# ctu-vras/depth_correction

Hardware: AMD Instinct MI355X
Metric: points/sec through min_eigval_loss fwd+bwd (200k pts, k=10); HBM GB/s vs peak (higher is better)
Workload: dtype f64

## Files before the change

### depth_correction_amd/_native.py

```python
from __future__ import annotations

import ctypes
import functools
import os

import torch

__all__ = ['lib', 'lib_path', 'on_device', 'DC_F32', 'DC_F64', 'DC_Q32', 'LOSS_KINDS', 'MODEL_KINDS']

DC_F32, DC_F64, DC_Q32 = 0, 1, 2
DC_TABLE_SLOTS, DC_TABLE_RUNS = 0, 1
LOSS_KINDS = {'min_eigval_loss': 0, 'trace_loss': 1}
DC_LOSS_RAW_POINTWISE, DC_LOSS_SKIP_NANS, DC_LOSS_ONLY_FINITE = 0x100, 0x200, 0x400
LOSS_RAW_POINTWISE = 0x100
DC_ERR_ARG, DC_ERR_DTYPE, DC_ERR_WORKSPACE, DC_ERR_UNSUPPORTED = -1, -2, -3, -4
DC_ERR_BACKWARD_TABLES = -5
MODEL_KINDS = {None: 0, 'BaseModel': 0, 'Polynomial': 1, 'ScaledPolynomial': 2, 'Linear': 3, 'InvCos': 4, 'ScaledInvCos': 5}
MAX_MODEL_TERMS = 8
DC_ICP_STATE_COUNT, DC_ICP_STATE_POSE, DC_ICP_STATE_PRIOR, DC_ICP_STATE_PAIRS, DC_ICP_STATE_SSE, DC_ICP_STATE_OVERLAP = 64, 0, 16, 48, 49, 50
DC_ICP_MAX_SMOOTH, DC_ICP_PARTIALS = 8, 30
DC_ICP_CT_STATE_COUNT, DC_ICP_CT_STATE_TWIST, DC_ICP_CT_STATE_PRIOR_TWIST, DC_ICP_CT_PARTIALS = 16, 0, 6, 93
DC_BIAS_MAX_BINS, DC_BIAS_MAX_TERMS, DC_BIAS_TOTALS, DC_BIAS_BIN_COLS = 256, 4, 5, 9
DC_BEAM_MAX_SAMPLES = 64
BEAM_DETECTIONS = {'mean': 0, 'quantile': 1}
BEAM_WEIGHTS = {'uniform': 0, 'lambert': 1}
DC_ALIGN_STATE_COUNT, DC_ALIGN_STATE_POSE, DC_ALIGN_STATE_PRIOR, DC_ALIGN_STATE_THRESHOLD = 64, 0, 16, 32
DC_ALIGN_STATE_PAIRS, DC_ALIGN_STATE_RMS, DC_ALIGN_STATE_D_ROT, DC_ALIGN_STATE_D_TRANS = 33, 34, 35, 36
DC_ALIGN_PARTIALS, DC_ALIGN_HISTORY_COLS = 17, 5
DC_GREG_BINS, DC_GREG_FEAT = 11, 33
DC_PLANEREG_MIN_PLANES, DC_PLANEREG_MAX_PLANES = 3, 64
ALIGN_STATUS = {0: 'running', 1: 'converged', 2: 'max_iterations', -1: 'too_few_pairs', -2: 'degenerate', -3: 'not_finite'}
ICP_STATUS = {0: 'running', 1: 'converged', 2: 'max_iterations', -1: 'too_few_pairs', -2: 'singular', -3: 'not_finite', -4: 'bound'}

_LIB = None
_vp, _i32, _i64, _f64, _sz = ctypes.c_void_p, ctypes.c_int, ctypes.c_int64, ctypes.c_double, ctypes.c_size_t

_SIGNATURES = {
    'dc_version': (ctypes.c_int, []),
    'dc_knn_workspace_bytes': (_sz, [_i64, _i64]),
    'dc_knn_set_shell_budget': (_i32, [_i32]),
    'dc_knn_set_fine_cell_count': (_i32, [_i32]),
    'dc_knn_build': (_i32, [_vp, _i32, _i32, _i64, _vp, _i32, _i64, _i32, _f64, _f64, _vp, _vp, _vp, _sz, _vp]),
    'dc_knn_build_i64': (_i32, [_vp, _i32, _i32, _i64, _vp, _i32, _i64, _i32, _f64, _f64, _vp, _vp, _vp, _vp, _sz, _vp]),
    'dc_radius_count': (_i32, [_vp, _i32, _i32, _i64, _f64, _vp, _vp, _vp, _sz, _vp]),
    'dc_radius_fill': (_i32, [_i64, _f64, _i32, _vp, _vp, _sz, _vp]),
    'dc_radius_count_query': (_i32, [_vp, _i32, _i32, _i64, _vp, _i32, _i64, _f64, _vp, _vp, _vp, _sz, _vp]),
    'dc_radius_fill_query': (_i32, [_i64, _i64, _f64, _i32, _vp, _vp, _sz, _vp]),
    'dc_knn_transpose_workspace_bytes': (_sz, [_i64, _i32]),
    'dc_knn_transpose': (_i32, [_vp, _i64, _i32, _i64, _vp, _vp, _vp, _sz, _vp]),
    'dc_spatial_order_workspace_bytes': (_sz, [_i64]),
    'dc_spatial_order': (_i32, [_vp, _i32, _i32, _i64, _vp, _vp, _sz, _vp]),
    'dc_points_fwd': (_i32, [_vp, _vp, _vp, _vp, _vp, _vp, _vp, _i32, _i32, _i32, _vp, _vp, _i64, _i32, _i32, _vp, _i32,
                             _vp, _vp, _vp, _vp, _vp, _vp]),
    'dc_consistency_gate': (_i32, [_vp, _i32, _i32, _vp, _i64, _vp, _i32, _vp, _vp, _vp, _vp]),
    'dc_points_basis': (_i32, [_vp, _vp, _vp, _vp, _vp, _vp, _vp, _i32, _i32, _i32, _vp, _i64, _i32, _vp, _vp, _vp, _vp]),
    'dc_partial_rows': (_i64, [_i64]),
    'dc_param_grad_count': (_i32, [_i32, _i32]),
    'dc_sequence_partials_count': (_i64, [_i64, _i32, _i32]),
    'dc_points_bwd': (_i32, [_vp, _vp, _i32, _i32, _i64, _vp, _vp, _vp, _vp, _vp, _vp, _vp, _i32, _i32, _i32, _vp, _vp, _i32,
                             _i32, _vp, _vp, _vp]),
    'dc_features_fwd': (_i32, [_vp, _i32, _i32, _vp, _i64, _i32, _vp, _f64, _vp, _vp, _vp, _vp, _vp, _vp, _vp, _vp, _vp,
                               _vp, _vp, _vp]),
    'dc_features_set_tiled': (_i32, [_i32]),
    'dc_features_bwd': (_i32, [_vp, _i32, _i32, _vp, _vp, _i64, _vp, _vp, _vp, _vp, _vp, _vp, _vp, _vp, _vp, _vp]),
    'dc_block_table_slots': (_i32, [_vp, _i64, _i32, _vp, _vp, _vp]),
    'dc_block_table_workspace_bytes': (_sz, [_i64]),
    'dc_block_table_build': (_i32, [_vp, _vp, _i64, _i32, _i64, _vp, _i64, _vp, _vp, _vp, _vp, _vp, _sz, _vp]),
    'dc_step_header_build': (_i32, [_vp, _i64, _vp, _vp, _vp, _vp]),
    'dc_step_rows_build': (_i32, [_vp, _i64, _vp, _i32, _vp, _vp]),
    'dc_block_group': (_i32, [_vp, _vp, _vp, _i64, _i32, _vp, _vp, _vp, _vp, _vp]),
    'dc_pose_table_build': (_i32, [_vp, _vp, _i64, _i32, _i32, _vp, _vp, _vp, _vp, _vp, _vp, _vp]),
    'dc_points_local_basis': (_i32, [_vp, _vp, _vp, _vp, _vp, _i32, _i32, _vp, _i64, _i32, _vp, _vp, _vp]),
    'dc_pose_train_finish': (_i32, [_vp, _i32, _i32, _i32, _vp, _vp, _vp, _vp, _vp, _vp, _vp, _i32, _i32, _vp, _f64, _f64, _f64, _f64, _f64,
                                    _vp, _vp, _i32, _vp, _vp, _vp, _vp, _i32, _vp]),
    'dc_pose_train_combine': (_i32, [_vp, _i32, _i32, _i32, _vp, _vp]),
    'dc_pose_train_combine2': (_i32, [_vp, _i32, _vp, _i32, _i32, _i32, _vp, _vp]),
    'dc_table_permute': (_i32, [_vp, _i64, _i32, _vp, _vp, _vp, _vp]),
    'dc_gather_rows': (_i32, [_vp, _i32, _vp, _i64, _vp, _vp]),
    'dc_points_extent_workspace_bytes': (_sz, []),
    'dc_points_extent': (_i32, [_vp, _i32, _i32, _i64, _vp, _vp, _sz, _vp]),
    'dc_scan_ids': (_i32, [_vp, _i32, _i64, _vp, _vp]),
    'dc_scan_lattice_workspace_bytes': (_sz, [_i32]),
    'dc_scan_lattice_shift': (_i32, [_vp, _i32, _i64, _vp, _i32, _vp, _vp, _vp, _sz, _vp]),
    'dc_scan_lattice_localize': (_i32, [_vp, _i64, _i32, _vp, _i32, _vp, _vp]),
    'dc_block_table_set_lds_build': (_i32, [_i32]),
    'dc_block_table_slots_workspace_bytes': (_sz, [_i64, _i32]),
    'dc_block_table_own_base': (_i32, [_vp, _vp, _i64, _vp, _vp]),
    'dc_block_table_run_capacity': (_i64, [_i64, _i64]),
    'dc_block_table_build_runs': (_i32, [_vp, _vp, _i64, _i64, _vp, _vp, _vp, _vp, _vp, _vp, _sz, _vp]),
    'dc_consistency_fwd': (_i32, [_vp, _i32, _i32, _i32, _vp, _vp, _vp, _vp, _i64, _i32, _vp, _vp, _i32, _i32, _i32, _vp, _vp,
                                  _vp, _vp, _vp, _vp]),
    'dc_consistency_bwd': (_i32, [_vp, _i32, _i32, _i32, _vp, _vp, _vp, _vp, _vp, _vp, _i64, _vp, _vp, _vp, _vp, _vp, _vp, _vp,
                                  _i32, _i32, _i32, _vp, _vp, _i32, _i32, _vp, _vp, _vp, _vp]),
    'dc_mask_bounds': (_i32, [_vp, _i32, _i32, _vp, _i32, _i32, _i32, _i64, _f64, _f64, _vp, _vp]),
    'dc_valid_count': (_i32, [_vp, _i64, _i32, _vp, _vp]),
    'dc_mask_bounds_multi': (_i32, [_vp, _i32, _i32, _i64, _i32, _vp, _vp, _vp, _vp, _i32, _vp, _vp]),
    'dc_compact_rows_workspace_bytes': (_sz, [_i64]),
    'dc_compact_rows': (_i32, [_vp, _i64, _i32, _vp, _vp, _vp, _vp, _vp, _vp, _sz, _vp]),
    'dc_to_points': (_i32, [_vp, _i32, _vp, _vp, _i32, _i64, _vp, _vp]),
    'dc_valid_weights': (_i32, [_vp, _i64, _vp, _vp]),
    'dc_scan_prefilter_workspace_bytes': (_sz, [_i64]),
    'dc_scan_prefilter': (_i32, [_vp, _i32, _i32, _vp, _i64, _i32, _f64, _f64, _f64, _vp, _vp, _vp, _vp, _vp, _vp, _sz, _vp]),
    'dc_nn1_corr_workspace_bytes': (_sz, [_i64]),
    'dc_nn1_corr': (_i32, [_vp, _vp, _i64, _f64, _vp, _vp, _vp, _vp, _vp, _sz, _vp]),
    'dc_dispersion': (_i32, [_vp, _i32, _vp, _vp, _i64, _i32, _vp, _vp]),
    'dc_sequence_eval': (_i32, [_vp, _vp, _vp, _vp, _i32, _i32, _i32, _vp, _vp]),
    'dc_sequence_step': (_i32, [_vp, _vp, _vp, _vp, _vp, _vp, _i64, _f64, _f64, _f64, _f64, _f64, _f64, _vp, _vp]),
    'dc_sequence_step_chained': (_i32, [_vp, _vp, _vp, _vp, _vp, _vp, _i64, _i32, _f64, _f64, _f64, _f64, _f64, _f64, _vp, _vp, _vp]),
    'dc_sequence_step_chained_rec': (_i32, [_vp, _vp, _vp, _vp, _vp, _vp, _i64, _i32, _f64, _f64, _f64, _f64, _f64, _f64, _vp, _vp, _vp, _vp]),
    'dc_sequence_eval_after_update': (_i32, [_vp, _vp, _vp, _vp, _vp, _vp, _i64, _vp, _f64, _f64, _f64, _f64, _f64, _f64, _vp, _vp, _vp, _vp]),
    'dc_sequence_step_linked': (_i32, [_vp, _vp, _i32, _i32, _vp, _vp, _vp, _vp, _vp, _vp, _i64, _i64, _f64, _f64, _f64, _f64, _f64, _f64, _vp, _vp,
                                       _vp, _vp]),
    'dc_sequence_chain_flush_linked': (_i32, [_vp, _i32, _vp, _vp, _vp, _vp, _i64, _i64, _f64, _f64, _f64, _f64, _f64, _f64, _vp, _vp, _vp]),
    'dc_sequence_chain_flush': (_i32, [_vp, _vp, _vp, _vp, _i64, _f64, _f64, _f64, _f64, _f64, _f64, _vp, _vp]),
    'dc_adam_step': (_i32, [_vp, _vp, _vp, _vp, _i64, _i64, _f64, _f64, _f64, _f64, _f64, _f64, _vp]),
    'dc_adam_step_device': (_i32, [_vp, _vp, _vp, _vp, _i64, _vp, _f64, _f64, _f64, _f64, _f64, _f64, _vp]),
    'dc_voxel_filter_workspace_bytes': (_sz, [_i64]),
    'dc_voxel_filter': (_i32, [_vp, _i32, _i32, _i64, _f64, _vp, _i32, _vp, _vp, _vp, _vp, _sz, _vp]),
    'dc_cloud_from_points_workspace_bytes': (_sz, [_i64]),
    'dc_cloud_from_points': (_i32, [_vp, _i32, _i32, _vp, _i64, _f64, _f64, _f64, _i32, _vp, _vp, _vp, _vp, _vp, _vp, _sz, _vp]),
    'dc_set_option': (_i32, [_i32, _i32]),
    'dc_profiler_enable': (_i32, [_i32]),
    'dc_profiler_reset': (_i32, []),
    'dc_profiler_read': (_i32, [_i32, _vp, _vp]),
    'dc_profiler_kernel': (_i32, [_i32, _vp, _i32]),
    'dc_p2plane_partial_count': (_i64, [_i64]),
    'dc_p2plane_pair': (_i32, [_vp, _vp, _vp, _vp, _vp, _vp, _vp, _vp, _vp, _vp, _vp, _vp, _i32, _vp, _vp, _i32, _i32,
                               _vp, _vp, _vp, _vp, _i64, _i32, _i32, _vp, _vp, _vp]),
    'dc_p2plane_sequence_partial_count': (_i64, [_vp, _i32]),
    'dc_p2plane_sequence': (_i32, [_vp, _i32, _vp, _i32, _i32, _vp, _i32, _i32, _vp, _vp, _vp, _vp, _vp]),
    'dc_p2point_pair': (_i32, [_vp, _vp, _vp, _vp, _vp, _vp, _vp, _vp, _vp, _vp, _i32, _vp, _vp, _i32, _i32, _vp, _vp, _vp, _vp,
                               _i64, _vp, _vp, _vp]),
    'dc_p2point_sequence': (_i32, [_vp, _i32, _vp, _i32, _i32, _vp, _i32, _i32, _vp, _vp, _vp, _vp, _vp]),
    'dc_icp_sequence_step': (_i32, [_i32, _vp, _i32, _vp, _i32, _i32, _vp, _i32, _i32, _vp, _vp, _vp, _vp, _vp, _vp, _vp]),
    'dc_pose_correct_fwd': (_i32, [_vp, _vp, _i32, _i32, _vp, _vp]),
    'dc_pose_correct_bwd': (_i32, [_vp, _vp, _i32, _i32, _vp, _vp, _vp]),
    'dc_shadow_mask': (_i32, [_vp, _vp, _i32, _i32, _vp, _i64, _i32, _f64, _f64, _f64, _vp, _vp]),
    'dc_correct_depth': (_i32, [_vp, _vp, _vp, _vp, _vp, _i32, _i32, _i32, _i64, _vp, _vp]),
    'dc_shadow_filter': (_i32, [_vp, _vp, _i32, _vp, _i32, _i64, _f64, _f64, _f64, _vp, _vp, _sz, _vp]),
    'dc_ransac_score': (_i32, [_vp, _i32, _vp, _i64, _i64, _i64, _i32, _f64, _vp, _vp, _vp, _vp, _vp, _vp]),
    'dc_ransac_refit_partial_count': (_i32, [_i64]),
    'dc_ransac_refit': (_i32, [_vp, _i32, _vp, _i64, _vp, _vp, _vp, _f64, _vp, _i32, _vp, _vp, _vp]),
    'dc_dbscan': (_i32, [_vp, _i64, _i32, _i32, _vp, _vp, _vp, _vp, _vp, _vp, _vp]),
    'dc_plane_moments_fwd': (_i32, [_vp, _vp, _vp, _i32, _vp, _vp, _vp, _i32, _vp, _vp, _vp, _i32, _i32, _i32, _i32, _vp, _vp, _vp,
                                    _vp, _vp, _vp]),
    'dc_plane_moments_bwd': (_i32, [_vp, _vp, _vp, _i32, _vp, _vp, _vp, _i32, _vp, _vp, _i32, _i32, _i32, _i32, _vp, _vp, _vp, _vp,
                                    _vp, _vp, _vp, _vp, _vp, _vp]),
    'dc_sequence_landscape_workspace_count': (_i64, [_i64]),
    'dc_sequence_landscape': (_i32, [_vp, _i32, _f64, _i32, _vp, _i64, _i32, _vp, _vp, _i64, _i32, _i32, _i32, _i32, _vp, _vp, _i64,
                                     _vp, _vp]),
    'dc_plane_landscape_partials_count': (_i32, [_i32, _i32]),
    'dc_plane_landscape': (_i32, [_vp, _vp, _vp, _i32, _vp, _vp, _vp, _i32, _vp, _vp, _vp, _i32, _i32, _i32, _i32, _vp, _vp, _vp,
# ... 47 lines not shown
    'dc_image_features_fwd': (_i32, [_vp, _vp, _i32, _vp, _vp, _i64, _vp, _i32, _i32, _i32, _i32, _i32, _f64, _vp, _vp, _vp, _vp, _vp, _vp, _vp,
                                     _vp, _vp]),
    'dc_image_shadow_mask': (_i32, [_vp, _vp, _i32, _vp, _i32, _vp, _vp, _i64, _vp, _i32, _i32, _i32, _i32, _i32, _f64, _f64, _f64, _vp, _vp]),
    'dc_align_blocks': (_i32, [_i64]),
    'dc_align_init': (_i32, [_vp, _vp, _vp, _vp, _i32, _vp]),
    'dc_align_accumulate': (_i32, [_vp, _i64, _vp, _i64, _vp, _vp, _vp, _vp, _vp, _vp, _i32, _vp, _vp]),
    'dc_align_finish': (_i32, [_vp, _i32, _vp, _f64, _f64, _i32, _i32, _vp, _vp, _vp, _i32, _vp]),
    'dc_survey_align_workspace_bytes': (_sz, [_i64]),
    'dc_survey_align': (_i32, [_vp, _sz, _i64, _vp, _i64, _vp, _i64, _vp, _f64, _f64, _i32, _f64, _f64, _i32, _vp, _vp, _vp, _vp, _vp, _sz,
                               _vp]),
    'dc_pair_spfh': (_i32, [_vp, _vp, _i64, _vp, _i32, _vp, _vp, _vp]),
    'dc_pair_fpfh': (_i32, [_vp, _vp, _i64, _vp, _i32, _vp, _vp, _vp, _vp]),
    'dc_feature_nn': (_i32, [_vp, _vp, _i64, _vp, _vp, _i64, _vp, _vp, _vp]),
    'dc_feature_nn_tile': (_i32, []),
    'dc_greg_fit': (_i32, [_vp, _vp, _i64, _i64, _i64, _f64, _f64, _vp, _vp, _vp, _vp]),
    'dc_greg_score': (_i32, [_vp, _i64, _vp, _i64, _vp, _vp, _i64, _f64, _vp, _vp]),
    'dc_planereg_blocks': (_i64, [_i64]),
    'dc_planereg_count': (_i32, [_vp, _vp, _i32, _vp, _i32, _vp, _i64, _i64, _i64, _f64, _f64, _f64, _f64, _vp, _vp]),
    'dc_planereg_fill': (_i32, [_vp, _vp, _i32, _vp, _i32, _vp, _i64, _i64, _i64, _f64, _f64, _f64, _f64, _vp, _i64, _vp, _vp, _vp, _vp]),
    'dc_tsdf_integrate': (_i32, [_vp, _vp, _vp, _i32, _i64, _vp, _vp, _f64, _f64, _f64, _f64, _i32, _i32, _i32, _f64, _i32, _f64, _f64, _f64,
                                 _vp, _vp, _vp, _vp]),
    'dc_tsdf_extract_workspace_bytes': (_sz, [_i32, _i32, _i32]),
    'dc_tsdf_extract_count': (_i32, [_vp, _vp, _i32, _i32, _i32, _i32, _vp, _vp, _sz, _vp]),
    'dc_tsdf_extract_fill': (_i32, [_vp, _vp, _f64, _f64, _f64, _f64, _i32, _i32, _i32, _i32, _vp, _sz, _i64, _i64, _vp, _vp, _vp]),
    'dc_tsdf_sparse_workspace_bytes': (_sz, [_i64, _i32, _i64]),
    'dc_tsdf_sparse_allocate': (_i32, [_vp, _vp, _vp, _i32, _i64, _vp, _vp, _f64, _f64, _f64, _f64, _f64, _i32, _f64, _f64, _i64, _vp, _vp, _vp,
                                       _vp, _vp, _sz, _vp]),
    'dc_tsdf_sparse_integrate': (_i32, [_vp, _vp, _vp, _i32, _i64, _vp, _vp, _f64, _f64, _f64, _f64, _f64, _i32, _f64, _f64, _i64, _vp, _vp, _vp,
                                        _vp, _vp, _vp, _vp]),
    'dc_tsdf_sparse_extract_workspace_bytes': (_sz, [_i64]),
    'dc_tsdf_sparse_extract_count': (_i32, [_vp, _vp, _i64, _vp, _vp, _i32, _vp, _vp, _sz, _vp]),
    'dc_tsdf_sparse_extract_fill': (_i32, [_vp, _vp, _i64, _vp, _vp, _f64, _f64, _f64, _f64, _i32, _vp, _sz, _i64, _i64, _vp, _vp, _vp]),
    'dc_tsdf_sparse_sample': (_i32, [_vp, _vp, _vp, _i64, _vp, _vp, _f64, _f64, _f64, _f64, _f64, _i32, _vp, _i64, _vp, _vp, _vp, _vp, _vp, _vp,
                                     _vp, _vp]),
    'dc_tsdf_icp_accumulate': (_i32, [_vp, _vp, _vp, _vp, _vp, _i64, _vp, _f64, _vp, _vp, _vp, _i32, _vp, _vp]),
    'dc_tsdf_loss_workspace_bytes': (_sz, [_i64, _i32, _i32]),
    'dc_tsdf_loss': (_i32, [_vp, _vp, _vp, _i64, _vp, _vp, _vp, _vp, _vp, _i64, _i64, _vp, _vp, _f64, _f64, _f64, _f64, _f64, _i32, _vp, _vp,
                            _vp, _vp, _vp, _vp, _i32, _i64, _vp, _vp, _i32, _i32, _i32, _vp, _vp, _i32, _i32, _f64, _vp, _vp, _vp, _vp, _vp,
                            _sz, _vp]),
    'dc_tsdf_sparse_cast_rays': (_i32, [_vp, _vp, _vp, _i64, _vp, _vp, _vp, _vp, _vp, _i64, _i64, _vp, _vp, _f64, _f64, _f64, _f64, _f64, _i32,
                                        _vp, _vp, _vp, _i32, _i64, _vp, _vp, _i32, _f64, _f64, _f64, _i32, _i32, _vp, _vp, _vp, _vp, _vp, _vp,
                                        _vp, _vp]),
}


class BlockTableDesc(ctypes.Structure):
    _fields_ = [('blk_ptr', _vp), ('blk_ids', _vp), ('slot_ptr', _vp), ('loc', _vp), ('max_rows', ctypes.c_int32),
                ('layout', ctypes.c_int32), ('run_ptr', _vp), ('own_base', _vp), ('packed', ctypes.c_int32),
                ('reserved', ctypes.c_int32), ('row_ptr', _vp)]


class PoseTableDesc(ctypes.Structure):
    _fields_ = [('blk_ptr', _vp), ('ids', _vp), ('loc', _vp), ('own_pos', _vp), ('row_seg', _vp), ('row_scan', _vp)]


class IcpScan(ctypes.Structure):
    _fields_ = [('vps', _vp), ('dirs', _vp), ('depth', _vp), ('inc', _vp), ('lmask', _vp), ('normals', _vp)]


class IcpPair(ctypes.Structure):
    _fields_ = [('scan_a', ctypes.c_int32), ('scan_b', ctypes.c_int32), ('idx_a', _vp), ('idx_b', _vp),
                ('m', ctypes.c_int64), ('weight', ctypes.c_double)]


class PoseTrainStepDesc(ctypes.Structure):
    _fields_ = [('w', _vp), ('w_m', _vp), ('w_v', _vp), ('poses0', _vp), ('deltas', _vp), ('d_m', _vp), ('d_v', _vp),
                ('n_deltas', ctypes.c_int32), ('zero_first', ctypes.c_int32), ('step', _vp), ('lr_w', _f64), ('lr_d', _f64),
                ('beta1', _f64), ('beta2', _f64), ('eps', _f64), ('poses_used', _vp), ('record', _vp), ('ring_rows', ctypes.c_int32),
                ('n_record_extra', ctypes.c_int32), ('record_extra', _vp), ('poses_next', _vp), ('poses12_next', _vp)]


class SequenceDesc(ctypes.Structure):
    _fields_ = [('n', ctypes.c_int64), ('k', ctypes.c_int32), ('n_scans', ctypes.c_int32), ('dtype', ctypes.c_int32),
                ('point_fmt', ctypes.c_int32), ('qparams', ctypes.c_double * 4),
                ('vps', _vp), ('dirs', _vp), ('depth', _vp), ('inc', _vp), ('lmask', _vp), ('scan_id', _vp),
                ('nbr', _vp), ('csr_ptr', _vp), ('csr_src', _vp), ('mask', _vp), ('lane_perm', _vp), ('centre_idx', _vp),
                ('n_centres', ctypes.c_int64), ('x', _vp), ('rec', _vp),
                ('partials', _vp), ('model_kind', ctypes.c_int32), ('n_terms', ctypes.c_int32),
                ('loss_kind', ctypes.c_int32), ('normalization', ctypes.c_int32), ('sqrt_', ctypes.c_int32),
                ('reserved', ctypes.c_int32), ('fwd_table', _vp), ('bwd_table', _vp), ('status', _vp), ('basis', _vp),
                ('partials_count', ctypes.c_int64), ('scan_seg', _vp), ('blk_skip', _vp), ('fwd_rows_active', ctypes.c_int32),
                ('reserved2', ctypes.c_int32), ('pose_table', _vp), ('local_basis', _vp), ('fwd_table_loss', _vp),
                ('fwd_rows_active_loss', ctypes.c_int32), ('reserved3', ctypes.c_int32), ('step_hdr', _vp),
                ('step_rows', _vp)]


def lib_path():
    return os.path.join(os.path.dirname(os.path.abspath(__file__)), 'lib', 'libdc_hip.so')


def lib():
    global _LIB
    if _LIB is None:
        path = lib_path()
        if not os.path.exists(path):
            raise RuntimeError('depth_correction_amd: %s is missing -- build it with `python -c "import '
                               '__graft_entry__ as g; g.build()"` (hipcc, gfx950). There is no CPU fallback.' % path)
        handle = ctypes.CDLL(path)
        for name, (res, args) in _SIGNATURES.items():
            fn = getattr(handle, name)
            fn.restype, fn.argtypes = res, args
        _LIB = handle
    return _LIB


def check(status, what):
    if status != 0:
        kind = {-1: 'invalid argument', -2: 'unsupported dtype', -3: 'workspace too small',
                -4: 'unsupported size', -5: 'backward tables missing'}.get(status, 'HIP error %d' % status)
        raise RuntimeError('%s failed: %s' % (what, kind))


def stream_ptr():
    raw = getattr(torch._C, '_cuda_getCurrentRawStream', None)
    if raw is not None:
        return ctypes.c_void_p(raw(torch.cuda.current_device()))
    return ctypes.c_void_p(torch.cuda.current_stream().cuda_stream)


def _device_of(args, kwargs):
    for a in tuple(args) + tuple(kwargs.values()):
        dev = a.device if isinstance(a, torch.Tensor) else getattr(a, 'device', None)
        if callable(dev):
            dev = dev()
        if isinstance(dev, torch.device) and dev.type == 'cuda':
            return dev
        if isinstance(a, dict):
            a = list(a.values())
        if isinstance(a, (list, tuple)) and a and not isinstance(a[0], (int, float, str)):
            dev = _device_of(a[:1], {})
            if dev is not None:
                return dev
    return None


def on_device(fn):
    @functools.wraps(fn)
    def guarded(*args, **kwargs):
        dev = _device_of(args, kwargs)
        if dev is None or dev.index is None or dev.index == torch.cuda.current_device():
            return fn(*args, **kwargs)
        with torch.cuda.device(dev):
            return fn(*args, **kwargs)
    return guarded


def dtype_code(t):
    if t.dtype == torch.float32:
        return DC_F32
    if t.dtype == torch.float64:
        return DC_F64
    raise TypeError('depth_correction_amd kernels take float32 or float64 tensors, got %s' % t.dtype)


def ptr(t):
    return None if t is None else ctypes.c_void_p(t.data_ptr())


def need(t, shape=None, dtype=None, name='tensor', device=None):
    if not isinstance(t, torch.Tensor):
        raise TypeError('%s must be a torch.Tensor' % name)
    if not t.is_cuda:
        raise RuntimeError('%s must live on the GPU (depth_correction_amd has no CPU path)' % name)
    if device is not None and t.device != device:
        raise RuntimeError('%s is on %s, expected %s' % (name, t.device, device))
    if not t.is_contiguous():
        raise RuntimeError('%s must be contiguous' % name)
# ... 7 lines not shown
```

### depth_correction_amd/csrc/dc_cons_basis.h

```cpp
#pragma once

namespace dc {

struct PointBasis {
  const void* __restrict__ rows;
  const double* __restrict__ w;
  int n_terms;
  double w_scale;
};

__host__ __device__ constexpr int step_rows_piece_words(int row_words, int piece) {
  return row_words - 4 * piece < 4 ? row_words - 4 * piece : 4;
}

__device__ __forceinline__ void stage_weights(const PointBasis& pb, double* s_w, bool coherent = false) {
  if ((int)threadIdx.x < pb.n_terms) {
    const double w = coherent ? __hip_atomic_load(pb.w + threadIdx.x, __ATOMIC_RELAXED, __HIP_MEMORY_SCOPE_AGENT) : pb.w[threadIdx.x];
    s_w[threadIdx.x] = w * pb.w_scale;
  }
}

template <typename PT> struct Basis;
template <> struct Basis<q32> {
  using T = float;
// ... 67 lines not shown
  static __device__ __forceinline__ void stage(int4* tile, int cap, int t, const Pt<double>::Raw& r) {
    tile[t] = make_int4(__double2loint(r.v[0]), __double2hiint(r.v[0]), __double2loint(r.v[1]), __double2hiint(r.v[1]));
    tile[cap + t] = make_int4(__double2loint(r.v[2]), __double2hiint(r.v[2]), 0, 0);
  }
  template <int NP>
  static __device__ __forceinline__ void chain(const PointBasis& pb, int np, int64_t j, const double* g, double* gw) {
    const double* r = static_cast<const double*>(pb.rows) + j * (6 + np);
    const double gu = g[0] * r[3] + g[1] * r[4] + g[2] * r[5];
#pragma unroll
    for (int k = 0; k < NP; ++k)
      if (k < np) gw[k] = gu * r[6 + k];
  }
  static __device__ __forceinline__ void write(void* rows, int64_t i, int nt, const double* x0, const double* u, const QParams&) {
    double* r = static_cast<double*>(rows) + i * (6 + nt);
#pragma unroll
    for (int a = 0; a < 3; ++a) { r[a] = x0[a]; r[3 + a] = u[a]; }
  }
  static __device__ __forceinline__ void write_term(void* rows, int64_t i, int nt, int k, double c) {
    static_cast<double*>(rows)[i * (6 + nt) + 6 + k] = c;
  }
};

template <typename PT>
__device__ __forceinline__ typename Pt<PT>::Raw staged_point(const int4* tile, int cap, int t) {
  int4 piece[Pt<PT>::kRow16];
  read_row<Pt<PT>::kRow16>(tile, cap, (uint32_t)t * 16u, piece);
  return Pt<PT>::from_row(piece);
}

template <typename PT>
__global__ __launch_bounds__(kBlock) void points_basis_kernel(PointInputs in, int64_t n, QParams qp, void* __restrict__ rows) {
  using T = typename Basis<PT>::T;
  __shared__ double s_pose[kLdsScans * 12];
  const PoseTile poses = stage_poses(in, s_pose);
  __syncthreads();
  const int64_t i = (int64_t)blockIdx.x * kBlock + threadIdx.x;
  if (i >= n) return;
  ModelParams mp;
  load_model(in, mp);
  double vp[3], dr[3], T12[12];
  if (in.vps) Row3<T, 3>::load((const T*)in.vps, i, vp, qp);
  else { vp[0] = vp[1] = vp[2] = 0.0; }
  Row3<T, 3>::load((const T*)in.dirs, i, dr, qp);
  const double d = (double)((const T*)in.depth)[i];
  const bool lm = in.lmask ? in.lmask[i] != 0 : true;
  const double inc = (mp.kind != DC_MODEL_NONE && lm) ? (double)((const T*)in.inc)[i] : 0.0;
  load_pose(in, poses, in.scan_id ? in.scan_id[i] : 0, T12);
  double vr[3], drr[3], x0[3];
  rot3(T12, vp, vr);
  vr[0] += T12[3]; vr[1] += T12[7]; vr[2] += T12[11];
  rot3(T12, dr, drr);
  const bool on = mp.kind != DC_MODEL_NONE && lm;
  const double d0 = (on && mp.kind == DC_MODEL_LINEAR) ? 0.0 : d;
#pragma unroll
  for (int a = 0; a < 3; ++a) x0[a] = vr[a] + d0 * drr[a];
  Basis<PT>::write(rows, i, mp.n_terms, x0, drr, qp);
#pragma unroll
  for (int k = 0; k < DC_MAX_MODEL_TERMS; ++k) {
    if (k < mp.n_terms) {
      double dk = 0.0;
      if (on) {
        if (mp.kind > DC_MODEL_SCALED_POLYNOMIAL) dk = model_dw_other(mp, k, d, inc);
        else dk = (mp.kind == DC_MODEL_SCALED_POLYNOMIAL ? -d : -1.0) * pow_term(inc, mp.e[k]);
      }
      Basis<PT>::write_term(rows, i, mp.n_terms, k, dk);
    }
  }
}

__global__ __launch_bounds__(kBlock) void step_rows_kernel(const int32_t* __restrict__ blk_ptr, const int32_t* __restrict__ blk_ids,
                                                           const int32_t* __restrict__ basis, int W, int32_t* __restrict__ out) {
  const int32_t base = blk_ptr[blockIdx.x], nd = blk_ptr[blockIdx.x + 1] - base;
  const int32_t* ids = blk_ids + base;
  int32_t* stretch = out + (int64_t)base * W;
  const int full = (W / 4) * 4 * nd;
  for (int j = threadIdx.x; j < W * nd; j += kBlock) {
    const int g = j < full ? j / (4 * nd) : W / 4;
    const int gw = step_rows_piece_words(W, g);
    const int r = j - 4 * g * nd, t = r / gw, c = r - t * gw;
    stretch[j] = basis[(int64_t)ids[t] * W + 4 * g + c];
  }
}

template <typename PT, bool FULL_EIG, int NS, int P>
__global__ __launch_bounds__(kBlock) void consistency_fwd_basis_kernel(
    PointBasis pb, BlockTab tab, const int32_t* __restrict__ own_base, int cap, const int32_t* __restrict__ centre_idx, int64_t n,
    const uint8_t* __restrict__ mask, const typename Basis<PT>::T* __restrict__ offset, LossParams lp, QParams qp, PT* __restrict__ rec,
    typename Basis<PT>::T* __restrict__ pointwise, typename Basis<PT>::T* __restrict__ eigvals, double* __restrict__ partials) {
  using T = typename Basis<PT>::T;
  extern __shared__ int4 tile[];
  __shared__ double s_w[DC_MAX_MODEL_TERMS];
  const int64_t nblocks = (n + kBlock - 1) / kBlock;
  const int64_t blk = xcd_block(nblocks);
  double acc2[2] = {0.0, 0.0};
  const int32_t s0 = blk >= 0 ? tab.slot_ptr[blk] : 0;
  const bool bad = blk >= 0 && tab.slot_ptr[blk + 1] - s0 != NS;
  if (blk >= 0 && !bad) {
    const int64_t i = blk * kBlock + threadIdx.x;
    const bool live = i < n;
    const uint16_t* lrow = tab.loc + (int64_t)s0 * kBlock + threadIdx.x;
    uint32_t pre[NS];
#pragma unroll
    for (int q = 0; q < NS; ++q) pre[q] = (uint32_t)lrow[q * kBlock];
    stage_weights(pb, s_w);
    const int32_t base = tab.blk_ptr[blk], nd = tab.blk_ptr[blk + 1] - base;
    const int32_t own = (own_base && !centre_idx) ? own_base[blk] : -1;
    __syncthreads();
    double wq[P > 0 ? P : DC_MAX_MODEL_TERMS];
#pragma unroll
    for (int k = 0; k < (P > 0 ? P : DC_MAX_MODEL_TERMS); ++k) wq[k] = (P > 0 || k < pb.n_terms) ? s_w[k] : 0.0;
    for (int t = threadIdx.x; t < nd; t += kBlock)
      Basis<PT>::stage(tile, cap, t, Basis<PT>::template point<P>(pb, wq, tab.blk_ids[base + t]));
    typename Pt<PT>::Raw ci;
    if (own < 0) ci = Basis<PT>::template point<P>(pb, wq, live ? (centre_idx ? (int64_t)centre_idx[i] : i) : 0);
    __syncthreads();
    if (own >= 0) ci = staged_point<PT>(tile, cap, own + (live ? (int)threadIdx.x : 0));
    if (live) {
      CovAcc acc;
      cov_init(acc);
      uint32_t mx = pre[0];
#pragma unroll
      for (int q = 1; q < NS; ++q) mx = max(mx, pre[q]);
      int n_have;
      if (__any((int)(mx == kNoLoc))) n_have = gather_fixed<PT, NS, true>(tile, cap, ci, pre, acc);
      else n_have = gather_fixed<PT, NS, false>(tile, cap, ci, pre, acc);
      acc.W = (double)n_have;
      consistency_point<T, PT, FULL_EIG>(acc, ci, i, mask, offset, lp, qp, rec, pointwise, eigvals, acc2);
    }
  } else {
    __syncthreads();
    __syncthreads();
  }
  if (bad) acc2[0] = acc2[1] = __longlong_as_double(0x7ff8000000000000ll);
  wave_partials<2>(acc2, partials);
}

template <typename PT, bool FULL_EIG, int P>
__global__ __launch_bounds__(kBlock) void consistency_fwd_basis_slots_kernel(
    PointBasis pb, BlockTab tab, const int32_t* __restrict__ own_base, int cap, const int32_t* __restrict__ centre_idx, int64_t n,
    const uint8_t* __restrict__ mask, const typename Basis<PT>::T* __restrict__ offset, LossParams lp, QParams qp, PT* __restrict__ rec,
    typename Basis<PT>::T* __restrict__ pointwise, typename Basis<PT>::T* __restrict__ eigvals, double* __restrict__ partials) {
  using T = typename Basis<PT>::T;
  extern __shared__ int4 tile[];
  __shared__ double s_w[DC_MAX_MODEL_TERMS];
  const int64_t nblocks = (n + kBlock - 1) / kBlock;
  const int64_t blk = xcd_block(nblocks);
  double acc2[2] = {0.0, 0.0};
  const int64_t i = blk * kBlock + threadIdx.x;
  const bool live = blk >= 0 && i < n;
  int32_t nslots = 0, own = -1;
  const uint16_t* lrow = tab.loc;
  uint32_t pre[kPreSlots];
  stage_weights(pb, s_w);
  if (blk >= 0) {
    const int32_t s0 = tab.slot_ptr[blk];
    nslots = tab.slot_ptr[blk + 1] - s0;
    lrow = tab.loc + (int64_t)s0 * kBlock + threadIdx.x;
#pragma unroll
    for (int q = 0; q < kPreSlots; ++q) pre[q] = (live && q < nslots) ? (uint32_t)lrow[q * kBlock] : kNoLoc;
    own = (own_base && !centre_idx) ? own_base[blk] : -1;
  }
  __syncthreads();
  double wq[P > 0 ? P : DC_MAX_MODEL_TERMS];
#pragma unroll
  for (int k = 0; k < (P > 0 ? P : DC_MAX_MODEL_TERMS); ++k) wq[k] = (P > 0 || k < pb.n_terms) ? s_w[k] : 0.0;
  typename Pt<PT>::Raw ci;
// ... 94 lines not shown
```

### depth_correction_amd/csrc/dc_cons_pose.h

```cpp
#pragma once

namespace dc {

struct PoseTab {
  const int32_t* __restrict__ blk_ptr;
  const int32_t* __restrict__ ids;
  const uint16_t* __restrict__ loc;
  const uint16_t* __restrict__ own_pos;
  const uint16_t* __restrict__ row_seg;
  const uint8_t* __restrict__ row_scan;
};
constexpr int kPoseCap = 512;

template <int K>
__global__ __launch_bounds__(kBlock) void pose_table_kernel(BlockTab tab, const int32_t* __restrict__ own_base,
                                                            const int32_t* __restrict__ scan_id, int64_t n, int n_scans,
                                                            int32_t* __restrict__ ids_out, uint16_t* __restrict__ loc_out,
                                                            uint16_t* __restrict__ own_pos, uint16_t* __restrict__ row_seg,
                                                            uint8_t* __restrict__ row_scan, int32_t* __restrict__ info) {
  __shared__ int32_t s_id[kPoseCap];
  __shared__ uint8_t s_scan[kPoseCap];
  __shared__ uint16_t s_new[kPoseCap];
  __shared__ int s_start[kMaxBlockScans + 1];
  const int64_t b = blockIdx.x;
// ... 99 lines not shown
  }
}

template <int NS, int P>
__global__ __launch_bounds__(kBlock, 4) void consistency_step_pose_kernel(
    const int32_t* __restrict__ lrows, PoseTab tab, const double* __restrict__ poses, int n_scans, const double* __restrict__ w,
    int64_t n, const uint8_t* __restrict__ mask, LossParams lp, QParams qp, double* __restrict__ p_fwd, double* __restrict__ p_bwd) {
  constexpr int CAP = kPoseCap;
  __shared__ int4 tile[2 * CAP];
  __shared__ unsigned long long s_g[3 * CAP];
  __shared__ double s_pose[kLdsScans * 12];
  __shared__ float s_bound[kWavesPerBlock];
  const int tid = threadIdx.x;
  const int64_t nblocks = (n + kBlock - 1) / kBlock;
  const int64_t blk = xcd_block(nblocks);
  const int64_t rs = (int64_t)gridDim.x;
  double* pcol = p_bwd + 2 * P * rs + (int64_t)(blockIdx.x & 7) * (gridDim.x >> 3) + (blockIdx.x >> 3);
  double acc2[2] = {0.0, 0.0}, gw[P];
#pragma unroll
  for (int k = 0; k < P; ++k) gw[k] = 0.0;
  if (blk < 0) {
    for (int item = tid; item < 12 * n_scans; item += kBlock) pcol[item * rs] = 0.0;
  } else {
    for (int t = tid; t < n_scans * 12; t += kBlock) s_pose[t] = poses[t];
    double wq[P];
#pragma unroll
    for (int k = 0; k < P; ++k) wq[k] = w[k];
    const int64_t i = blk * kBlock + tid;
    const bool live = i < n;
    const bool in_mask = live && (mask ? mask[i] != 0 : true);
    const uint16_t* lrow = tab.loc + (blk * NS) * kBlock + tid;
    uint32_t pre[NS];
#pragma unroll
    for (int q = 0; q < NS; ++q) pre[q] = live ? (uint32_t)lrow[q * kBlock] : kNoLoc;
    const uint32_t own = live ? (uint32_t)tab.own_pos[i] : 0u;
    const int32_t base = tab.blk_ptr[blk], nd = tab.blk_ptr[blk + 1] - base;
    static_assert(CAP == 2 * kBlock, "two staged rows per thread");
    int2 rw[2][3];
    int rsc[2];
#pragma unroll
    for (int j = 0; j < 2; ++j) {
      const int t = tid + j * kBlock < nd ? tid + j * kBlock : 0;
      const int2* src = reinterpret_cast<const int2*>(lrows) + 3 * (int64_t)(base + t);
      rw[j][0] = src[0]; rw[j][1] = src[1]; rw[j][2] = src[2];
      rsc[j] = tab.row_scan[base + t];
    }
    for (int t = tid; t < 3 * CAP; t += kBlock) s_g[t] = 0ull;
    __syncthreads();
#pragma unroll
    for (int j = 0; j < 2; ++j) {
      const int t = tid + j * kBlock;
      if (t >= nd) continue;
      const float c0 = __int_as_float(rw[j][2].x), c1f = __int_as_float(rw[j][2].y);
      const int sc = rsc[j];
      double dp = (double)__int_as_float(rw[j][0].x) + wq[0] * (double)c0;
      if constexpr (P > 1) dp += wq[1] * (double)c1f;
      const double dl[3] = {(double)__int_as_float(rw[j][0].y), (double)__int_as_float(rw[j][1].x), (double)__int_as_float(rw[j][1].y)};
      const double* Tp = s_pose + sc * 12;
      double u[3], x[3];
#pragma unroll
      for (int a = 0; a < 3; ++a) {
        u[a] = Tp[4 * a] * dl[0] + Tp[4 * a + 1] * dl[1] + Tp[4 * a + 2] * dl[2];
        x[a] = Tp[4 * a + 3] + dp * u[a];
      }
      tile[t] = make_int4(quantize(x[0], qp.origin[0], qp.inv_scale, qp.flag), quantize(x[1], qp.origin[1], qp.inv_scale, qp.flag),
                          quantize(x[2], qp.origin[2], qp.inv_scale, qp.flag), __float_as_int((float)u[0]));
      tile[CAP + t] = make_int4(__float_as_int((float)u[1]), __float_as_int((float)u[2]), rw[j][2].x, rw[j][2].y);
    }
    __syncthreads();
    const bool work = live && (!mask || __any((int)in_mask));
    Pt<q32>::Raw ci;
    double cm[3] = {0.0, 0.0, 0.0}, v0[3] = {0.0, 0.0, 0.0}, c1 = 0.0, c2 = 0.0;
    float bound = 0.0f;
    if (work) {
      const char* tb = reinterpret_cast<const char*>(tile);
      ci = Pt<q32>::from_row(reinterpret_cast<const int4*>(tb + own));
      CovAcc acc;
      cov_init(acc);
      uint32_t mo = pre[0];
#pragma unroll
      for (int q = 1; q < NS; ++q) mo |= pre[q];
      const bool any_miss = __any((int)(mo & 1u)) != 0;
      int n_have;
      if (any_miss) n_have = gather_fixed<q32, NS, true>(tile, CAP, ci, pre, acc);
      else n_have = gather_fixed<q32, NS, false>(tile, CAP, ci, pre, acc);
      acc.W = (double)n_have;
      double se2;
      step_point2<q32, NS>(acc, n_have, !any_miss, in_mask, lp, qp, acc2, cm, v0, &c1, &c2, &se2);
      const float r = sqrtf((float)se2);
      bound = (float)(fabs(c1) + fabs(c2)) * (r > 1.0f ? r : 1.0f);
    }
    bound = bound == bound ? bound : INFINITY;
#pragma unroll
    for (int o = kWave / 2; o > 0; o >>= 1) bound = fmaxf(bound, __shfl_xor(bound, o, kWave));
    if ((tid & (kWave - 1)) == 0) s_bound[tid / kWave] = bound;
    __syncthreads();
    bound = s_bound[0];
#pragma unroll
    for (int q = 1; q < kWavesPerBlock; ++q) bound = fmaxf(bound, s_bound[q]);
    const bool poisoned = !(bound < INFINITY);
    int sh = 0;
    if (bound > 0.0f && !poisoned) {
      int ex;
      (void)frexpf(bound, &ex);
      sh = 50 - ex;
      sh = sh > 100 ? 100 : sh;
    }
    const double S = ldexp(1.0, sh), invS = ldexp(1.0, -sh);
    if (work && !poisoned) {
      float cmf[3], vs[3], vu[3], gwf[P];
      const double c1s = c1 * S;
#pragma unroll
      for (int a = 0; a < 3; ++a) { cmf[a] = (float)cm[a]; vs[a] = (float)(c1s * v0[a]); vu[a] = (float)v0[a]; }
      const float c2f = (float)(c2 * S);
#pragma unroll
      for (int k = 0; k < P; ++k) gwf[k] = 0.0f;
      if (__any((int)(c1 != 0.0 || c2 != 0.0))) {
#pragma unroll
        for (int q = 0; q < NS; ++q) {
          if (q % 4 == 0 && q > 0) __builtin_amdgcn_sched_barrier(0);
          chain_term_pose<P, CAP>(tile, s_g, pre[q], pre[q] != kNoLoc && (c1 != 0.0 || c2 != 0.0), ci, cmf, vs, vu, c2f, gwf);
        }
      }
#pragma unroll
      for (int k = 0; k < P; ++k) gw[k] = (double)gwf[k] * (qp.scale * invS);
    }
    __syncthreads();
    {
      const uint16_t* seg = tab.row_seg + blk * (n_scans + 1);
      const int sc = tid >> 3, part = tid & 7;
      const bool mine = sc < n_scans;
      const int end = mine ? (int)seg[sc + 1] : 0;
      double sacc[12];
#pragma unroll
      for (int q = 0; q < 12; ++q) sacc[q] = 0.0;
      for (int p = mine ? (int)seg[sc] + part : 0; p < end; p += 8) {
        const int4 xr = tile[p];
        const double qd[3] = {(double)xr.x, (double)xr.y, (double)xr.z};
#pragma unroll
        for (int a = 0; a < 3; ++a) {
          const unsigned long long bits = s_g[a * CAP + p];
          const double g = fma((double)(int)(uint32_t)(bits >> 32), 4294967296.0, (double)(uint32_t)bits);
#pragma unroll
          for (int c = 0; c < 3; ++c) sacc[(a & 1) * 6 + (a >> 1) * 3 + c] = fma(g, qd[c], sacc[(a & 1) * 6 + (a >> 1) * 3 + c]);
          sacc[9 + a] += g;
        }
      }
      const bool up1 = (part & 1) != 0, up2 = (part & 2) != 0;
      double h[6], r3[3], gs[3];
#pragma unroll
      for (int q = 0; q < 6; ++q) h[q] = (up1 ? sacc[6 + q] : sacc[q]) + dpp_f64<kDppXor1>(up1 ? sacc[q] : sacc[6 + q]);
#pragma unroll
      for (int q = 0; q < 3; ++q) {
        r3[q] = (up2 ? h[3 + q] : h[q]) + dpp_f64<kDppXor2>(up2 ? h[q] : h[3 + q]);
        r3[q] += dpp_f64<kDppShl4>(r3[q]);
        gs[q] = dpp_f64<kDppQuad3>(r3[q]);
      }
      if (mine && part < 3) {
        const double unscale = qp.scale * invS;
        const double* Tp = s_pose + sc * 12;
        const double ga = (part == 0 ? gs[0] : (part == 1 ? gs[1] : gs[2])) * unscale;
        double m[3];
#pragma unroll
        for (int c = 0; c < 3; ++c) m[c] = fma(r3[c] * unscale, qp.scale, ga * (qp.origin[c] - Tp[4 * c + 3]));
        double* dst = pcol + (sc * 12 + part * 4) * rs;
#pragma unroll
        for (int b2 = 0; b2 < 3; ++b2) {
          const double v = fma(m[2], Tp[8 + b2], fma(m[1], Tp[4 + b2], m[0] * Tp[b2]));
// ... 12 lines not shown
```

### depth_correction_amd/csrc/dc_cons_step.h

```cpp
#pragma once

namespace dc {

template <typename PT, int P> struct StepRow;
template <int P> struct StepRow<q32, P> {
  static constexpr int kPieces = (6 + P + 3) / 4;
  struct Raw { int32_t q[6 + P]; };
  static __device__ __forceinline__ Raw fetch(const PointBasis& pb, int64_t row) {
    const int32_t* r = static_cast<const int32_t*>(pb.rows) + row * (6 + P);
    Raw o;
#pragma unroll
    for (int c = 0; c < 6 + P; ++c) o.q[c] = r[c];
    return o;
  }
  static __device__ __forceinline__ void stage(const PointBasis& pb, const double* wq, int64_t row, int4* tile, int cap, int t) {
    place(fetch(pb, row), wq, tile, cap, t);
  }
  static __device__ __forceinline__ Raw fetch_copy(const int32_t* crow, int nd, int t) {
    constexpr int W = 6 + P;
    Raw o;
#pragma unroll
    for (int g = 0; g < kPieces; ++g) {
      const int gw = step_rows_piece_words(W, g);
      const int32_t* r = crow + (uint32_t)(4 * g * nd + gw * t);
// ... 368 lines not shown
  {
    const double* h = hand + lane;
    v[0] = (v[0] + h[0]) + (h[kWave] + h[2 * kWave]);
#pragma unroll
    for (int k = 0; k < P; ++k) {
      const double* hk = h + (1 + k) * kOthers * kWave;
      v[2 + k] = (v[2 + k] + hk[0]) + (hk[kWave] + hk[2 * kWave]);
    }
    const double* hc = hand + NL * kOthers * kWave;
    cnt = (cnt + hc[1]) + (hc[2] + hc[3]);
  }
  double tot;
  if constexpr (NP2 == 4) tot = DPP ? wave_sum4_dpp<true>(v) : wave_sum_packed<4>(v);
  else tot = DPP ? wave_sum8_regs(v) : wave_sum_packed<8>(v);
  if (q == 1) tot = cnt;
  if (lane < NP2) {
    if (q < 2) *reinterpret_cast<double*>(fwd + off_f) = tot;
    else if (q < NV) *reinterpret_cast<double*>(bwd + off_b) = tot;
  }
}

template <typename PT, int NS, int P, int VAR = 0>
__global__ __launch_bounds__(kBlock) void consistency_step_basis_kernel(
    PointBasis pb, BlockTab tab, const int32_t* __restrict__ own_base, int cap, const int32_t* __restrict__ centre_idx, int64_t n,
    const uint8_t* __restrict__ mask, LossParams lp, QParams qp, double* __restrict__ p_fwd, double* __restrict__ p_bwd,
    StepChain ch) {
  extern __shared__ int4 tile[];
  __shared__ double s_w[DC_MAX_MODEL_TERMS];
  __shared__ int s_ok;
  __shared__ double s_front[kBlock / kWave];
  const bool chained = ch.ready != nullptr;
  if (chained && (int)blockIdx.x < ch.n_front) { chain_front_block<P>(ch, s_front); return; }
  const int64_t nblocks = (n + kBlock - 1) / kBlock;
  int64_t blk = chain_block_of(ch, chained, nblocks);
  if (blk >= 0 && ch.blk_skip && ch.blk_skip[blk]) blk = -1;
  double acc2[2] = {0.0, 0.0}, gw[P];
#pragma unroll
  for (int k = 0; k < P; ++k) gw[k] = 0.0;
  const int32_t s0 = blk >= 0 ? tab.slot_ptr[blk] : 0;
  bool bad = blk >= 0 && tab.slot_ptr[blk + 1] - s0 != NS;
  if (blk >= 0 && !bad) {
    const int64_t i = blk * kBlock + threadIdx.x;
    const bool live = i < n;
    const bool in_mask = live && (mask ? mask[i] != 0 : true);
    const uint16_t* lrow = tab.loc + (int64_t)s0 * kBlock + threadIdx.x;
    uint32_t pre[NS];
#pragma unroll
    for (int q = 0; q < NS; ++q) pre[q] = (uint32_t)lrow[q * kBlock];
    const int32_t base = tab.blk_ptr[blk], nd = tab.blk_ptr[blk + 1] - base;
    const int32_t own = (own_base && !centre_idx) ? own_base[blk] : -1;
    double wq[P];
    if (chained) {
      typename StepRow<PT, P>::Raw r0, r1;
      const int t0 = threadIdx.x, t1 = threadIdx.x + kBlock;
      if (t0 < nd) r0 = StepRow<PT, P>::fetch(pb, tab.blk_ids[base + t0]);
      if (t1 < nd) r1 = StepRow<PT, P>::fetch(pb, tab.blk_ids[base + t1]);
      chain_weights<P>(ch, pb.w_scale, s_w, &s_ok);
      __syncthreads();
      if (!s_ok) bad = true;
#pragma unroll
      for (int k = 0; k < P; ++k) wq[k] = s_w[k];
      if (t0 < nd) StepRow<PT, P>::place(r0, wq, tile, cap, t0);
      if (t1 < nd) StepRow<PT, P>::place(r1, wq, tile, cap, t1);
      for (int t = threadIdx.x + 2 * kBlock; t < nd; t += kBlock) StepRow<PT, P>::stage(pb, wq, tab.blk_ids[base + t], tile, cap, t);
    } else {
      stage_weights(pb, s_w);
      __syncthreads();
#pragma unroll
      for (int k = 0; k < P; ++k) wq[k] = s_w[k];
      for (int t = threadIdx.x; t < nd; t += kBlock) StepRow<PT, P>::stage(pb, wq, tab.blk_ids[base + t], tile, cap, t);
    }
    typename Pt<PT>::Raw ci;
    if (own < 0) ci = Basis<PT>::template point<P>(pb, wq, live ? (centre_idx ? (int64_t)centre_idx[i] : i) : 0);
    __syncthreads();
    if (own >= 0) ci = staged_point<PT>(tile, cap, own + (live ? (int)threadIdx.x : 0));
    if (live && (!mask || __any((int)in_mask))) {
      CovAcc acc;
      cov_init(acc);
      uint32_t mx = pre[0];
#pragma unroll
      for (int q = 1; q < NS; ++q) mx = max(mx, pre[q]);
      const bool any_miss = __any((int)(mx == kNoLoc)) != 0;
      int n_have;
      if (any_miss) n_have = gather_fixed<PT, NS, true>(tile, cap, ci, pre, acc);
      else n_have = gather_fixed<PT, NS, false>(tile, cap, ci, pre, acc);
      acc.W = (double)n_have;
      double cm[3], v0[3], c1, c2;
      if constexpr ((VAR & kVarSlimTail) != 0) step_point2<PT, NS>(acc, n_have, !any_miss, in_mask, lp, qp, acc2, cm, v0, &c1, &c2);
      else step_point<PT>(acc, in_mask, lp, qp, acc2, cm, v0, &c1, &c2);
      const double u = Pt<PT>::unit(qp);
      if constexpr ((VAR & kVarF32Sweep) != 0 && std::is_same<PT, q32>::value) {
        float cmf[3], vs[3], vu[3], gwf[P];
#pragma unroll
        for (int a = 0; a < 3; ++a) { cmf[a] = (float)cm[a]; vs[a] = (float)(c1 * v0[a]); vu[a] = (float)v0[a]; }
        const float c2f = (float)c2;
#pragma unroll
        for (int k = 0; k < P; ++k) gwf[k] = 0.0f;
        if (any_miss) {
#pragma unroll
          for (int q = 0; q < NS; ++q) {
            if (q % 4 == 0 && q > 0) __builtin_amdgcn_sched_barrier(0);
            chain_term_f32<P>(tile, cap, pre[q], pre[q] != kNoLoc, ci, cmf, vs, vu, c2f, gwf);
          }
        } else {
#pragma unroll
          for (int q = 0; q < NS; ++q) {
            if (q % 4 == 0 && q > 0) __builtin_amdgcn_sched_barrier(0);
            chain_term_f32<P>(tile, cap, pre[q], true, ci, cmf, vs, vu, c2f, gwf);
          }
        }
#pragma unroll
        for (int k = 0; k < P; ++k) gw[k] = (double)gwf[k] * u;
      } else {
        double mean[3];
        StepRow<PT, P>::mean_of(ci, cm, mean);
        if (any_miss) {
#pragma unroll
          for (int q = 0; q < NS; ++q) chain_term<PT, P>(tile, cap, pre[q], pre[q] != kNoLoc, mean, v0, c1, c2, gw);
        } else {
#pragma unroll
          for (int q = 0; q < NS; ++q) chain_term<PT, P>(tile, cap, pre[q], true, mean, v0, c1, c2, gw);
        }
#pragma unroll
        for (int k = 0; k < P; ++k) gw[k] *= u;
      }
    }
  }
  if (chained) {
    step_block_row<P, (VAR & kVarDppSums) != 0>(acc2[0], acc2[1] != 0.0, gw, bad, blk < 0, reinterpret_cast<double*>(tile), p_fwd, p_bwd, ch.n_front);
    return;
  }
  if (bad) acc2[0] = acc2[1] = __longlong_as_double(0x7ff8000000000000ll);
  step_partials<P, (VAR & kVarDppSums) != 0>(acc2, gw, p_fwd, p_bwd);
}

constexpr int kStepQ32Cap = 512;

typedef float float2v __attribute__((ext_vector_type(2)));
template <int P, int CAP>
__device__ __forceinline__ void chain_term_q32(const int4* tile, uint32_t off, bool have, const Pt<q32>::Raw& ci, const float* cmf, const float* vs,
                                               const float* vu, float c2f, float* gw) {
  const char* row = reinterpret_cast<const char*>(tile) + (have ? off : 0u);
  const int4 p0 = *reinterpret_cast<const int4*>(row);
  const int4 p1 = *reinterpret_cast<const int4*>(row + (size_t)CAP * 16);
  const float2v e01 = float2v{(float)(p0.x - ci.v[0]), (float)(p0.y - ci.v[1])} - float2v{cmf[0], cmf[1]};
  const float e0 = e01.x, e1 = e01.y, e2 = (float)(p0.z - ci.v[2]) - cmf[2];
  const float u0 = __int_as_float(p0.w), u1 = __int_as_float(p1.x), u2 = __int_as_float(p1.y);
  const float al = fmaf(vs[2], e2, fmaf(vs[1], e1, vs[0] * e0));
  const float be = fmaf(vu[2], u2, fmaf(vu[1], u1, vu[0] * u0));
  const float ga = fmaf(e2, u2, fmaf(e1, u1, e0 * u0));
  float tj = fmaf(al, be, -(c2f * ga));
  if (!have) tj = 0.0f;
  if constexpr (P == 2) {
    float2v g = float2v{gw[0], gw[1]};
    g = __builtin_elementwise_fma(float2v{tj, tj}, float2v{__int_as_float(p1.z), __int_as_float(p1.w)}, g);
    gw[0] = g.x; gw[1] = g.y;
  } else {
    gw[0] = fmaf(tj, __int_as_float(p1.z), gw[0]);
    if constexpr (P > 1) gw[1] = fmaf(tj, __int_as_float(p1.w), gw[1]);
    if constexpr (P > 2) gw[2] = fmaf(tj, __int_as_float(reinterpret_cast<const int4*>(row + (size_t)CAP * 32)->x), gw[2]);
  }
}

template <int P, int CAP> constexpr int step_q32_blocks() {
  constexpr int lds = StepRow<q32, P>::kPieces * CAP * 16 + 512;
  return 7 * lds <= 160 * 1024 ? 7 : 6 * lds <= 160 * 1024 ? 6 : 4;
}
template <int Q> __device__ __forceinline__ uint32_t pre_at(const uint32_t* pk) { return (Q & 1) ? pk[Q >> 1] >> 16 : pk[Q >> 1] & 0xFFFFu; }
template <int NS, bool MISS, int Q0 = 0>
__device__ __forceinline__ int gather_fixed_pk(const int4* tile, const Pt<q32>::Raw& ci, const uint32_t* pk, CovAcc& acc) {
  if constexpr (Q0 >= NS) return 0;
  else {
    constexpr int NQ = NS - Q0 < 4 ? NS - Q0 : 4;
    uint32_t off[NQ];
    off[0] = pre_at<Q0>(pk);
    if constexpr (NQ > 1) off[1] = pre_at<Q0 + (NQ > 1 ? 1 : 0)>(pk);
    if constexpr (NQ > 2) off[2] = pre_at<Q0 + (NQ > 2 ? 2 : 0)>(pk);
    if constexpr (NQ > 3) off[3] = pre_at<Q0 + (NQ > 3 ? 3 : 0)>(pk);
    Pt<q32>::Raw cj[NQ];
    bool have[NQ];
    int n_have = 0;
#pragma unroll
    for (int u_ = 0; u_ < NQ; ++u_) {
      have[u_] = !MISS || off[u_] != kNoLoc;
      int4 piece[1];
      read_row<1>(tile, 0, have[u_] ? off[u_] : 0u, piece);
      cj[u_] = Pt<q32>::from_row(piece);
    }
#pragma unroll
    for (int u_ = 0; u_ < NQ; ++u_) {
      double d[3];
      Pt<q32>::delta(have[u_] ? cj[u_] : ci, ci, d);
      cov_add_d(acc, d[0], d[1], d[2]);
      n_have += have[u_] ? 1 : 0;
    }
    return n_have + gather_fixed_pk<NS, MISS, Q0 + 4>(tile, ci, pk, acc);
  }
}
template <int NS, int P, int CAP, bool MISS, int Q = 0>
__device__ __forceinline__ void chain_sweep_pk(const int4* tile, const uint32_t* pk, const Pt<q32>::Raw& ci, const float* cmf, const float* vs,
                                               const float* vu, float c2f, float* gwf) {
  if constexpr (Q < NS) {
    if constexpr (Q % 4 == 0 && Q > 0) __builtin_amdgcn_sched_barrier(0);
    const uint32_t off = pre_at<Q>(pk);
    chain_term_q32<P, CAP>(tile, off, !MISS || off != kNoLoc, ci, cmf, vs, vu, c2f, gwf);
    chain_sweep_pk<NS, P, CAP, MISS, Q + 1>(tile, pk, ci, cmf, vs, vu, c2f, gwf);
  }
}
#ifdef DC_BLOCK_TRACE
__device__ unsigned long long* g_block_trace = nullptr;
#define DC_TRACE_BEGIN() const unsigned long long trace_t0 = __builtin_amdgcn_s_memrealtime()
#define DC_TRACE_END() do { if (threadIdx.x == 0 && g_block_trace) { \
    unsigned long long* tr_ = g_block_trace + 4 * (size_t)blockIdx.x; \
    tr_[0] = ((unsigned long long)__builtin_amdgcn_s_getreg((31 << 11) | 20) << 32) | (unsigned)__builtin_amdgcn_s_getreg((31 << 11) | 4); \
    tr_[1] = trace_t0; tr_[2] = __builtin_amdgcn_s_memrealtime(); tr_[3] = 1; } } while (0)
#else
#define DC_TRACE_BEGIN() do {} while (0)
#define DC_TRACE_END() do {} while (0)
#endif

template <int NS, int P, int CAP, int BLOCKS = step_q32_blocks<P, CAP>()>
__global__ __launch_bounds__(kBlock, BLOCKS) void consistency_step_q32_kernel(
    PointBasis pb, BlockTab tab, const StepHdr* __restrict__ hdr, const int32_t* __restrict__ step_rows, const int32_t* __restrict__ centre_idx,
    int64_t n, LossParams lp, QParams qp, double* __restrict__ p_fwd, double* __restrict__ p_bwd, StepChain ch) {
  constexpr int NV = 2 + P, NP2 = NV <= 4 ? 4 : 8;
  constexpr int cap = CAP;
  __shared__ int4 tile[StepRow<q32, P>::kPieces * CAP];
  __shared__ double s_w[DC_MAX_MODEL_TERMS];
  __shared__ double s_front[kWavesPerBlock];
  __shared__ int s_ok[2];
  DC_TRACE_BEGIN();
  const bool chained = ch.ready != nullptr;
  if (chained && (int)blockIdx.x < ch.n_front) { chain_front_block<P>(ch, s_front); return; }
  const int64_t nblocks = (n + kBlock - 1) / kBlock;
  const int64_t blk = chain_block_of(ch, chained, nblocks);
  double loss = 0.0, gw[P];
  bool cnt_lane = false;
#pragma unroll
  for (int k = 0; k < P; ++k) gw[k] = 0.0;
  typedef int32_t int16v __attribute__((ext_vector_type(16)));
  int16v hw = {0, 0, 0, 0, 0, kStepHdrSkip, 0, 0, 0, 0, 0, 0, 0, 0, 0, 0};
  if (blk >= 0) hw = *reinterpret_cast<const int16v*>(hdr + blk);
  const int wave_s = __builtin_amdgcn_readfirstlane((int)(threadIdx.x / kWave));
  const uint32_t in_lo = (uint32_t)(wave_s == 0 ? hw[8] : wave_s == 1 ? hw[10] : wave_s == 2 ? hw[12] : hw[14]);
  const uint32_t in_hi = (uint32_t)(wave_s == 0 ? hw[9] : wave_s == 1 ? hw[11] : wave_s == 2 ? hw[13] : hw[15]);
  const uint64_t in_word = ((uint64_t)in_hi << 32) | in_lo;
  const int32_t s0 = hw[0], base = hw[2], nd = hw[3], own = hw[4];
  const bool skip = (hw[5] & kStepHdrSkip) != 0;
  bool bad = !skip && hw[1] != NS;
  if (!skip && !bad) {
    const uint32_t tid = threadIdx.x;
    const int64_t i0 = blk * kBlock;
    const bool live = tid < (uint32_t)hw[6];
    const bool in_mask = ((in_word >> (tid & (kWave - 1))) & 1ull) != 0;
    const uint16_t* lrow = tab.loc + (int64_t)s0 * kBlock;
    constexpr int NW = (NS + 1) / 2;
    uint32_t pk[NW];
#pragma unroll
    for (int j = 0; j < NW; ++j)
      pk[j] = (uint32_t)lrow[(uint32_t)(2 * j * kBlock) + tid] |
              (2 * j + 1 < NS ? (uint32_t)lrow[(uint32_t)((2 * j + 1 < NS ? 2 * j + 1 : 0) * kBlock) + tid] << 16 : 0u);
    const int32_t* ids = tab.blk_ids + base;
    const int32_t* crow = step_rows ? step_rows + (int64_t)base * (6 + P) : nullptr;
    double wq[P];
    if (chained) {
      typename StepRow<q32, P>::Raw r0, r1;
      const int t0 = (int)tid, t1 = (int)tid + kBlock;
      if (crow) {
        if (t0 < nd) r0 = StepRow<q32, P>::fetch_copy(crow, nd, t0);
        if (t1 < nd) r1 = StepRow<q32, P>::fetch_copy(crow, nd, t1);
      } else {
        if (t0 < nd) r0 = StepRow<q32, P>::fetch(pb, ids[t0]);
        if (t1 < nd) r1 = StepRow<q32, P>::fetch(pb, ids[t1]);
      }
      chain_weights<P>(ch, pb.w_scale, s_w, s_ok);
      __syncthreads();
      if (!s_ok[0]) bad = true;
#pragma unroll
      for (int k = 0; k < P; ++k) wq[k] = s_w[k];
      if (t0 < nd) StepRow<q32, P>::place(r0, wq, tile, cap, t0);
      if (t1 < nd) StepRow<q32, P>::place(r1, wq, tile, cap, t1);
      if (crow) for (int t = (int)tid + 2 * kBlock; t < nd; t += kBlock) StepRow<q32, P>::place(StepRow<q32, P>::fetch_copy(crow, nd, t), wq, tile, cap, t);
      else for (int t = (int)tid + 2 * kBlock; t < nd; t += kBlock) StepRow<q32, P>::stage(pb, wq, ids[t], tile, cap, t);
    } else {
      stage_weights(pb, s_w);
      __syncthreads();
#pragma unroll
      for (int k = 0; k < P; ++k) wq[k] = s_w[k];
      if (crow) for (int t = (int)tid; t < nd; t += kBlock) StepRow<q32, P>::place(StepRow<q32, P>::fetch_copy(crow, nd, t), wq, tile, cap, t);
      else for (int t = (int)tid; t < nd; t += kBlock) StepRow<q32, P>::stage(pb, wq, ids[t], tile, cap, t);
    }
    Pt<q32>::Raw ci;
    if (own < 0) ci = Basis<q32>::template point<P>(pb, wq, live ? (centre_idx ? (int64_t)(centre_idx + i0)[tid] : i0 + tid) : 0);
    __syncthreads();
    if (own >= 0) ci = staged_point<q32>(tile, cap, own + (live ? (int)tid : 0));
    if (live && in_word != 0) {
      CovAcc acc;
      cov_init(acc);
      uint32_t mo = pk[0];
#pragma unroll
      for (int j = 1; j < NW; ++j) mo |= pk[j];
      const bool any_miss = __any((int)(mo & 0x00010001u)) != 0;
      int n_have;
      if (any_miss) n_have = gather_fixed_pk<NS, true>(tile, ci, pk, acc);
      else n_have = gather_fixed_pk<NS, false>(tile, ci, pk, acc);
      acc.W = (double)n_have;
      double cm[3], v0[3], c1, c2, acc2[2] = {0.0, 0.0};
      step_point2<q32, NS>(acc, n_have, !any_miss, in_mask, lp, qp, acc2, cm, v0, &c1, &c2);
      loss = acc2[0];
      cnt_lane = acc2[1] != 0.0;
      float cmf[3], vs[3], vu[3], gwf[P];
#pragma unroll
      for (int a = 0; a < 3; ++a) { cmf[a] = (float)cm[a]; vs[a] = (float)(c1 * v0[a]); vu[a] = (float)v0[a]; }
      const float c2f = (float)c2;
#pragma unroll
      for (int k = 0; k < P; ++k) gwf[k] = 0.0f;
      asm volatile("" ::: "memory");
      Pt<q32>::Raw cs;
      if (own >= 0) {
        cs = staged_point<q32>(tile, cap, own + (int)tid);
      } else {
        double w2[P];
#pragma unroll
        for (int k = 0; k < P; ++k) w2[k] = s_w[k];
        cs = Basis<q32>::template point<P>(pb, w2, centre_idx ? (int64_t)(centre_idx + i0)[tid] : i0 + tid);
      }
      if (any_miss) chain_sweep_pk<NS, P, CAP, true>(tile, pk, cs, cmf, vs, vu, c2f, gwf);
      else chain_sweep_pk<NS, P, CAP, false>(tile, pk, cs, cmf, vs, vu, c2f, gwf);
      const double u = qp.scale;
#pragma unroll
      for (int k = 0; k < P; ++k) gw[k] = (double)gwf[k] * u;
    }
  }
  if (chained) {
    static_assert(sizeof(tile) >= step_hand_bytes<P>(), "the hand-over of step_block_row lives in the tile");
    step_block_row<P>(loss, cnt_lane, gw, bad, skip, reinterpret_cast<double*>(tile), p_fwd, p_bwd, ch.n_front);
    DC_TRACE_END();
    return;
  }
  const double nan_ = __longlong_as_double(0x7ff8000000000000ll);
  if (bad) loss = nan_;
  const double cnt = bad ? nan_ : (double)__popcll(__ballot((int)cnt_lane));
  double v[NP2];
  v[0] = loss; v[1] = 0.0;
#pragma unroll
  for (int k = 0; k < NP2 - 2; ++k) v[2 + k] = k < P ? gw[k] : 0.0;
  double tot;
  if constexpr (NP2 == 4) tot = wave_sum4_dpp(v);
  else tot = wave_sum8_regs(v);
  const int lane = threadIdx.x & (kWave - 1), wave = threadIdx.x / kWave;
  if (packed_value_of_lane<NP2>(lane & (NP2 - 1)) == 1) tot = cnt;
  const int64_t rs = (int64_t)gridDim.x * kWavesPerBlock, row = (int64_t)blockIdx.x * kWavesPerBlock + wave;
  if (lane < NP2) {
    const int q = packed_value_of_lane<NP2>(lane);
    if (q < 2) p_fwd[q * rs + row] = tot;
    else if (q < NV) p_bwd[(q - 2) * rs + row] = tot;
  }
  DC_TRACE_END();
}

template <typename PT, int P>
__global__ __launch_bounds__(kBlock) void consistency_step_basis_slots_kernel(
    PointBasis pb, BlockTab tab, const int32_t* __restrict__ own_base, int cap, const int32_t* __restrict__ centre_idx, int64_t n,
    const uint8_t* __restrict__ mask, LossParams lp, QParams qp, double* __restrict__ p_fwd, double* __restrict__ p_bwd,
    StepChain ch, int packed) {
  extern __shared__ int4 tile[];
  __shared__ double s_w[DC_MAX_MODEL_TERMS];
  __shared__ int s_ok;
  __shared__ double s_front[kBlock / kWave];
  const bool chained = ch.ready != nullptr;
  if (chained && (int)blockIdx.x < ch.n_front) { chain_front_block<P>(ch, s_front); return; }
  const int64_t nblocks = (n + kBlock - 1) / kBlock;
  int64_t blk = xcd_block_of((int64_t)blockIdx.x - (chained ? ch.n_front : 0), nblocks);
  if (blk >= 0 && ch.blk_skip && ch.blk_skip[blk]) blk = -1;
  double acc2[2] = {0.0, 0.0}, gw[P];
#pragma unroll
  for (int k = 0; k < P; ++k) gw[k] = 0.0;
  const int64_t i = blk * kBlock + threadIdx.x;
  const bool live = blk >= 0 && i < n;
  int32_t nslots = 0, own = -1, base = 0, nd = 0;
  const uint16_t* lrow = tab.loc;
  uint32_t pre[kPreSlots];
  if (blk >= 0) {
    const int32_t s0 = tab.slot_ptr[blk];
    nslots = tab.slot_ptr[blk + 1] - s0;
    lrow = tab.loc + (int64_t)s0 * kBlock + threadIdx.x;
#pragma unroll
    for (int q = 0; q < kPreSlots; ++q) pre[q] = (live && q < nslots) ? (uint32_t)lrow[q * kBlock] : kNoLoc;
    own = (own_base && !centre_idx) ? own_base[blk] : -1;
    base = tab.blk_ptr[blk];
    nd = tab.blk_ptr[blk + 1] - base;
  }
  double wq[P];
  bool timed_out = false;
  typename Pt<PT>::Raw ci;
  if (chained) {
    typename StepRow<PT, P>::Raw r0, r1;
    const int t0 = threadIdx.x, t1 = threadIdx.x + kBlock;
    if (t0 < nd) r0 = StepRow<PT, P>::fetch(pb, tab.blk_ids[base + t0]);
    if (t1 < nd) r1 = StepRow<PT, P>::fetch(pb, tab.blk_ids[base + t1]);
    chain_weights<P>(ch, pb.w_scale, s_w, &s_ok);
    __syncthreads();
    timed_out = !s_ok;
#pragma unroll
    for (int k = 0; k < P; ++k) wq[k] = s_w[k];
    if (t0 < nd) StepRow<PT, P>::place(r0, wq, tile, cap, t0);
    if (t1 < nd) StepRow<PT, P>::place(r1, wq, tile, cap, t1);
    for (int t = threadIdx.x + 2 * kBlock; t < nd; t += kBlock) StepRow<PT, P>::stage(pb, wq, tab.blk_ids[base + t], tile, cap, t);
  } else {
    stage_weights(pb, s_w);
    __syncthreads();
#pragma unroll
    for (int k = 0; k < P; ++k) wq[k] = s_w[k];
    for (int t = threadIdx.x; t < nd; t += kBlock) StepRow<PT, P>::stage(pb, wq, tab.blk_ids[base + t], tile, cap, t);
  }
  if (blk >= 0 && own < 0) ci = Basis<PT>::template point<P>(pb, wq, live ? (centre_idx ? (int64_t)centre_idx[i] : i) : 0);
  __syncthreads();
  if (live) {
    if (own >= 0) ci = staged_point<PT>(tile, cap, own + (int)threadIdx.x);
    CovAcc acc;
    cov_init(acc);
    bool miss = false;
#pragma unroll
    for (int q = 0; q < kPreSlots; ++q) miss |= (q < nslots) && pre[q] == kNoLoc;
    int n_have = 0;
    if (__any((int)miss)) n_have = gather_slots<PT, true>(tile, cap, ci, pre, nslots, acc);
    else n_have = gather_slots<PT, false>(tile, cap, ci, pre, nslots, acc);
    if (nslots > kPreSlots) n_have += gather_tail<PT>(tile, cap, ci, lrow, nslots, packed != 0, acc);
    acc.W = (double)n_have;
    double cm[3], v0[3], c1, c2;
    const bool full = nslots >= 2 && !__any((int)(n_have != nslots));
    step_point2<PT, 2>(acc, n_have, full, mask ? mask[i] != 0 : true, lp, qp, acc2, cm, v0, &c1, &c2, nullptr, nslots);
    const double u = Pt<PT>::unit(qp);
    if constexpr (std::is_same<PT, q32>::value) {
      float cmf[3], vs[3], vu[3], gwf[P];
#pragma unroll
      for (int a = 0; a < 3; ++a) { cmf[a] = (float)cm[a]; vs[a] = (float)(c1 * v0[a]); vu[a] = (float)v0[a]; }
      const float c2f = (float)c2;
#pragma unroll
      for (int k = 0; k < P; ++k) gwf[k] = 0.0f;
#pragma unroll
      for (int q = 0; q < kPreSlots; ++q)
        if (q < nslots) chain_term_f32<P>(tile, cap, pre[q], pre[q] != kNoLoc, ci, cmf, vs, vu, c2f, gwf);
#pragma unroll
      for (int k = 0; k < P; ++k) gw[k] = (double)gwf[k];
      if (nslots > kPreSlots) chain_tail_f32<P>(tile, cap, lrow, nslots, packed != 0, ci, cmf, vs, vu, c2f, gw);
#pragma unroll
      for (int k = 0; k < P; ++k) gw[k] *= u;
    } else {
      double mean[3];
      StepRow<PT, P>::mean_of(ci, cm, mean);
#pragma unroll
      for (int q = 0; q < kPreSlots; ++q)
        if (q < nslots) chain_term<PT, P>(tile, cap, pre[q], pre[q] != kNoLoc, mean, v0, c1, c2, gw);
      if (nslots > kPreSlots) chain_tail<PT, P>(tile, cap, lrow, nslots, packed != 0, mean, v0, c1, c2, gw);
#pragma unroll
      for (int k = 0; k < P; ++k) gw[k] *= u;
    }
  }
  if (chained) {
    step_block_row<P>(acc2[0], acc2[1] != 0.0, gw, timed_out, blk < 0, reinterpret_cast<double*>(tile), p_fwd, p_bwd, ch.n_front);
    return;
  }
  step_partials<P, true>(acc2, gw, p_fwd, p_bwd);
}

template <int P, int CAP>
__global__ __launch_bounds__(kBlock, (CAP <= 1024 ? 5 : 4)) void consistency_step_ragged_q32_kernel(
    PointBasis pb, BlockTab tab, const int32_t* __restrict__ own_base, const int32_t* __restrict__ row_ptr, int64_t n,
    const uint8_t* __restrict__ mask, LossParams lp, QParams qp, double* __restrict__ p_fwd, double* __restrict__ p_bwd,
    StepChain ch) {
  using Row = StepRow<q32, P>;
  extern __shared__ int4 tile[];
  __shared__ double s_w[DC_MAX_MODEL_TERMS];
  __shared__ int s_ok;
  __shared__ double s_front[kBlock / kWave];
  DC_TRACE_BEGIN();
  const bool chained = ch.ready != nullptr;
  if (chained && (int)blockIdx.x < ch.n_front) { chain_front_block<P>(ch, s_front); return; }
  const int64_t nblocks = (n + kBlock - 1) / kBlock;
  int64_t blk = xcd_block_of((int64_t)blockIdx.x - (chained ? ch.n_front : 0), nblocks);
  if (blk >= 0 && ch.blk_skip && ch.blk_skip[blk]) blk = -1;
  double acc2[2] = {0.0, 0.0}, gw[P];
#pragma unroll
  for (int k = 0; k < P; ++k) gw[k] = 0.0;
  const int64_t i = blk * kBlock + threadIdx.x;
  const bool live = blk >= 0 && i < n;
  int32_t nslots = 0, own = 0, base = 0, nd = 0, deg = 0;
  const uint16_t* lrow = tab.loc;
  uint32_t first[kTrip];
  if (blk >= 0) {
    const int32_t s0 = tab.slot_ptr[blk];
    nslots = tab.slot_ptr[blk + 1] - s0;
    lrow = tab.loc + (int64_t)s0 * kBlock + threadIdx.x;
    if (live) deg = row_ptr[i + 1] - row_ptr[i];
    own = own_base[blk];
    base = tab.blk_ptr[blk];
    nd = tab.blk_ptr[blk + 1] - base;
  }
  const uint32_t own_off = (uint32_t)(own + (int)threadIdx.x) * 16u;
#pragma unroll
  for (int u_ = 0; u_ < kTrip; ++u_) first[u_] = (live && nslots > 0) ? (uint32_t)lrow[u_ * kBlock] : kNoLoc;
  double wq[P];
  bool timed_out = false;
  if (chained) {
    typename Row::Raw r0, r1;
    const int t0 = threadIdx.x, t1 = threadIdx.x + kBlock;
    if (t0 < nd) r0 = Row::fetch(pb, tab.blk_ids[base + t0]);
    if (t1 < nd) r1 = Row::fetch(pb, tab.blk_ids[base + t1]);
    chain_weights<P>(ch, pb.w_scale, s_w, &s_ok);
    __syncthreads();
    timed_out = !s_ok;
#pragma unroll
    for (int k = 0; k < P; ++k) wq[k] = s_w[k];
    if (t0 < nd) Row::place(r0, wq, tile, CAP, t0);
    if (t1 < nd) Row::place(r1, wq, tile, CAP, t1);
    for (int t = threadIdx.x + 2 * kBlock; t < nd; t += kBlock) Row::stage(pb, wq, tab.blk_ids[base + t], tile, CAP, t);
  } else {
    stage_weights(pb, s_w);
    __syncthreads();
#pragma unroll
    for (int k = 0; k < P; ++k) wq[k] = s_w[k];
    for (int t = threadIdx.x; t < nd; t += kBlock) Row::stage(pb, wq, tab.blk_ids[base + t], tile, CAP, t);
  }
  __syncthreads();
  const bool in_mask = live && (mask ? mask[i] != 0 : true);
  if (live && (!mask || __any((int)in_mask))) {
    const char* tb = reinterpret_cast<const char*>(tile);
    const Pt<q32>::Raw ci = Pt<q32>::from_row(reinterpret_cast<const int4*>(tb + own_off));
    int wmax = deg;
#pragma unroll
    for (int off = kWave / 2; off > 0; off >>= 1) wmax = max(wmax, __shfl_xor(wmax, off, kWave));
    wmax = __builtin_amdgcn_readfirstlane(min(wmax, nslots));
    CovAcc acc;
    cov_init(acc);
    auto sweep1 = [&](const uint32_t* l, uint32_t* nx, const uint16_t* pn) {
#pragma unroll
      for (int u_ = 0; u_ < kTrip; ++u_) nx[u_] = (uint32_t)pn[u_ * kBlock];
      int4 r[kTrip];
#pragma unroll
      for (int u_ = 0; u_ < kTrip; ++u_) r[u_] = *reinterpret_cast<const int4*>(tb + (l[u_] == kNoLoc ? own_off : l[u_]));
#pragma unroll
      for (int u_ = 0; u_ < kTrip; ++u_)
        cov_add_d(acc, (double)(r[u_].x - ci.v[0]), (double)(r[u_].y - ci.v[1]), (double)(r[u_].z - ci.v[2]));
    };
    {
      uint32_t la[kTrip], lb[kTrip];
#pragma unroll
      for (int u_ = 0; u_ < kTrip; ++u_) la[u_] = first[u_];
      const uint16_t* pn = lrow + kTrip * kBlock;
      for (int q0 = 0; q0 < wmax; q0 += 2 * kTrip) {
        sweep1(la, lb, pn);
        pn += kTrip * kBlock;
        if (q0 + kTrip >= wmax) break;
        sweep1(lb, la, pn);
        pn += kTrip * kBlock;
      }
    }
    acc.W = (double)deg;
    double cm[3], v0[3], c1, c2;
    step_point2<q32, 2>(acc, deg, false, in_mask, lp, qp, acc2, cm, v0, &c1, &c2);
    const double u = Pt<q32>::unit(qp);
    float cmf[3], vs[3], vu[3];
#pragma unroll
    for (int a = 0; a < 3; ++a) { cmf[a] = (float)cm[a]; vs[a] = (float)(c1 * v0[a]); vu[a] = (float)v0[a]; }
    const float c2f = (float)c2;
    auto sweep2 = [&](const uint32_t* l, uint32_t* nx, const uint16_t* pn) {
#pragma unroll
      for (int u_ = 0; u_ < kTrip; ++u_) nx[u_] = (uint32_t)pn[u_ * kBlock];
      float2v g[P];
#pragma unroll
      for (int k = 0; k < P; ++k) g[k] = float2v{0.0f, 0.0f};
#pragma unroll
      for (int u_ = 0; u_ < kTrip; u_ += 2) {
        const bool ha = l[u_] != kNoLoc, hb = l[u_ + 1] != kNoLoc;
        const char* ra = tb + (ha ? l[u_] : own_off);
        const char* rb = tb + (hb ? l[u_ + 1] : own_off);
        const int4 a0 = *reinterpret_cast<const int4*>(ra), a1 = *reinterpret_cast<const int4*>(ra + CAP * 16);
        const int4 b0 = *reinterpret_cast<const int4*>(rb), b1 = *reinterpret_cast<const int4*>(rb + CAP * 16);
        const float2v e0 = float2v{(float)(a0.x - ci.v[0]), (float)(b0.x - ci.v[0])} - float2v{cmf[0], cmf[0]};
        const float2v e1 = float2v{(float)(a0.y - ci.v[1]), (float)(b0.y - ci.v[1])} - float2v{cmf[1], cmf[1]};
        const float2v e2 = float2v{(float)(a0.z - ci.v[2]), (float)(b0.z - ci.v[2])} - float2v{cmf[2], cmf[2]};
        const float2v u0 = float2v{__int_as_float(a0.w), __int_as_float(b0.w)};
        const float2v u1 = float2v{__int_as_float(a1.x), __int_as_float(b1.x)};
        const float2v u2 = float2v{__int_as_float(a1.y), __int_as_float(b1.y)};
        const float2v al = __builtin_elementwise_fma(float2v{vs[2], vs[2]}, e2, __builtin_elementwise_fma(float2v{vs[1], vs[1]}, e1, float2v{vs[0], vs[0]} * e0));
        const float2v be = __builtin_elementwise_fma(float2v{vu[2], vu[2]}, u2, __builtin_elementwise_fma(float2v{vu[1], vu[1]}, u1, float2v{vu[0], vu[0]} * u0));
        const float2v ga = __builtin_elementwise_fma(e2, u2, __builtin_elementwise_fma(e1, u1, e0 * u0));
        float2v tj = __builtin_elementwise_fma(al, be, -(float2v{c2f, c2f} * ga));
        tj = float2v{ha ? tj.x : 0.0f, hb ? tj.y : 0.0f};
        g[0] = __builtin_elementwise_fma(tj, float2v{__int_as_float(a1.z), __int_as_float(b1.z)}, g[0]);
        if constexpr (P > 1) g[1] = __builtin_elementwise_fma(tj, float2v{__int_as_float(a1.w), __int_as_float(b1.w)}, g[1]);
        if constexpr (P > 2)
          g[2] = __builtin_elementwise_fma(tj, float2v{__int_as_float(reinterpret_cast<const int4*>(ra + CAP * 32)->x),
                                                       __int_as_float(reinterpret_cast<const int4*>(rb + CAP * 32)->x)}, g[2]);
      }
#pragma unroll
      for (int k = 0; k < P; ++k) gw[k] += (double)(g[k].x + g[k].y);
    };
    {
      uint32_t la[kTrip], lb[kTrip];
#pragma unroll
      for (int u_ = 0; u_ < kTrip; ++u_) la[u_] = first[u_];
      const uint16_t* pn = lrow + kTrip * kBlock;
      for (int q0 = 0; q0 < wmax; q0 += 2 * kTrip) {
        sweep2(la, lb, pn);
        pn += kTrip * kBlock;
        if (q0 + kTrip >= wmax) break;
        sweep2(lb, la, pn);
        pn += kTrip * kBlock;
      }
    }
#pragma unroll
    for (int k = 0; k < P; ++k) gw[k] *= u;
  }
  if (chained) step_block_row<P>(acc2[0], acc2[1] != 0.0, gw, timed_out, blk < 0, reinterpret_cast<double*>(tile), p_fwd, p_bwd, ch.n_front);
  else step_partials<P, true>(acc2, gw, p_fwd, p_bwd);
  DC_TRACE_END();
}

}
```

### depth_correction_amd/csrc/dc_consistency.hip

```cpp
#include <type_traits>
#include <atomic>
#include <mutex>
#include <cstdio>
#include <hip/hip_ext.h>
#include "dc_common.h"
#include "dc_device.h"
#include "dc_pointmath.h"
#include "dc_prof.h"
#include "dc_points_dev.h"
#include "dc_cons_route.h"
#include "../../include/dc_hip.h"

namespace dc {

template <typename T, typename PT, int STRIDE>
__global__ __launch_bounds__(kBlock) void points_fwd_kernel(PointInputs in, int64_t n, QParams qp, PT* __restrict__ x_out,
                                                            T* __restrict__ vps_out, T* __restrict__ dirs_out,
                                                            T* __restrict__ depth_out) {
  __shared__ double s_pose[kLdsScans * 12];
  const int64_t i = (int64_t)blockIdx.x * kBlock + threadIdx.x;
  const int64_t ic = i < n ? i : n - 1;
  ModelParams mp;
  load_model(in, mp);
  T vp_r[3] = {T(0), T(0), T(0)}, dr_r[3];
// ... 356 lines not shown
    const PT* __restrict__ x, const PT* __restrict__ rec, const int32_t* __restrict__ csr_ptr,
    const int32_t* __restrict__ csr_src, const uint8_t* __restrict__ lane_perm, int64_t n, PointInputs in, QParams qp,
    T* __restrict__ grad_points, double* __restrict__ partials, int n_acc, uint32_t rec_bytes) {
#pragma clang fp contract(off)
  constexpr int want_e = WANT_E, want_pose = WANT_POSE;
  __shared__ double lds[(kBlock / kWave) * 2 * DC_MAX_MODEL_TERMS];
  __shared__ double s_pose[kLdsScans * 12];
  const PoseTile poses = in.dirs ? stage_poses(in, s_pose) : PoseTile{nullptr};
  if (WANT_POSE) pose_ticket_init();
  __syncthreads();
  const int64_t nblocks = (n + kBlock - 1) / kBlock;
  const int64_t blk = xcd_block(nblocks);
  ModelParams mp;
  load_model(in, mp);
  double gw[DC_MAX_MODEL_TERMS], ge[DC_MAX_MODEL_TERMS], gT[6];
#pragma unroll
  for (int k = 0; k < DC_MAX_MODEL_TERMS; ++k) gw[k] = ge[k] = 0.0;
#pragma unroll
  for (int k = 0; k < 6; ++k) gT[k] = 0.0;
  int scan = -1;
  bool active = false;
  if (blk >= 0) {
    const int64_t base = blk * kBlock;
    const int64_t j = base + (lane_perm ? (int64_t)lane_perm[base + threadIdx.x] : (int64_t)threadIdx.x);
    if (j < n) {
      active = true;
      double g[3] = {0.0, 0.0, 0.0};
      const typename Pt<PT>::Raw cj = Pt<PT>::template load<STRIDE>(x, j, qp);
      const double u = Pt<PT>::unit(qp);
      const int32_t beg = csr_ptr[j], end = csr_ptr[j + 1];
      const BufRsrc rrec = make_rsrc(rec, rec_bytes);
      int32_t nxt[4];
#pragma unroll
      for (int u_ = 0; u_ < 4; ++u_) nxt[u_] = (beg + u_ < end) ? csr_src[beg + u_] : -1;
      for (int32_t e0 = beg; e0 < end; e0 += 4) {
        int32_t src[4];
        int4 q[4][RecRaw<PT>::kRow16];
#pragma unroll
        for (int u_ = 0; u_ < 4; ++u_) src[u_] = nxt[u_];
#pragma unroll
        for (int u_ = 0; u_ < 4; ++u_) {
#pragma unroll
          for (int a = 0; a < RecRaw<PT>::kRow16; ++a) q[u_][a] = buf_load16(rrec, (uint32_t)src[u_] * RowBytes<PT>::rec + 16u * a);
        }
#pragma unroll
        for (int u_ = 0; u_ < 4; ++u_) nxt[u_] = (e0 + 4 + u_ < end) ? csr_src[e0 + 4 + u_] : -1;
        edge_terms4<PT>(cj, q, g);
      }
      g[0] *= u; g[1] *= u; g[2] *= u;
      if (grad_points) Row3<T, STRIDE>::store(grad_points, j, g, QParams{});
      if (in.dirs) points_bwd_point<T>(in, poses, mp, j, g, gw, ge, gT, want_e != 0, want_pose != 0, &scan);
    }
  }
  if (in.dirs) reduce_param_grads<T>(in, active, want_e, want_pose, gw, ge, gT, scan, lds, partials, lane_perm ? -2 : blk);
}

struct BlockTab {
  const int32_t* __restrict__ blk_ptr;
  const int32_t* __restrict__ blk_ids;
  const int32_t* __restrict__ slot_ptr;
  const uint16_t* __restrict__ loc;
};
constexpr uint32_t kNoLoc = 0xFFFFu;

template <int ROW16>
__device__ __forceinline__ int stage_rows(const int32_t* __restrict__ blk_ptr, const int32_t* __restrict__ blk_ids, int64_t blk,
                                          const int4* __restrict__ src, int4* tile, int cap) {
  const int32_t base = blk_ptr[blk], nd = blk_ptr[blk + 1] - base;
  for (int t = threadIdx.x; t < nd; t += kBlock) {
    const int64_t id = blk_ids[base + t];
#pragma unroll
    for (int a = 0; a < ROW16; ++a) tile[a * cap + t] = src[id * ROW16 + a];
  }
  return nd;
}

template <int ROW16>
__device__ __forceinline__ void read_row(const int4* tile, int cap, uint32_t off, int4* q) {
  const char* p = reinterpret_cast<const char*>(tile) + off;
#pragma unroll
  for (int a = 0; a < ROW16; ++a) q[a] = *reinterpret_cast<const int4*>(p + (size_t)a * cap * 16);
}

constexpr int kPreSlots = 16;

template <typename PT, bool MISS>
__device__ __forceinline__ int slot_add(const int4* tile, int cap, const typename Pt<PT>::Raw& ci, uint32_t l, CovAcc& acc) {
  constexpr int XR = Pt<PT>::kRow16;
  const bool have = !MISS || l != kNoLoc;
  int4 piece[XR];
  read_row<XR>(tile, cap, have ? l : 0u, piece);
  const typename Pt<PT>::Raw cj = Pt<PT>::from_row(piece);
  double d[3];
  Pt<PT>::delta(have ? cj : ci, ci, d);
  cov_add_d(acc, d[0], d[1], d[2]);
  return have ? 1 : 0;
}

template <typename PT, bool MISS>
__device__ __forceinline__ int gather_slots(const int4* tile, int cap, const typename Pt<PT>::Raw& ci, const uint32_t* pre,
                                            int nslots, CovAcc& acc) {
  constexpr int XR = Pt<PT>::kRow16;
  int n_have = 0;
#pragma unroll
  for (int t = 0; t < kPreSlots / 4; ++t) {
    if (4 * t + 4 <= nslots) {
      typename Pt<PT>::Raw cj[4];
      bool have[4];
#pragma unroll
      for (int u_ = 0; u_ < 4; ++u_) {
        have[u_] = !MISS || pre[4 * t + u_] != kNoLoc;
        int4 piece[XR];
        read_row<XR>(tile, cap, have[u_] ? pre[4 * t + u_] : 0u, piece);
        cj[u_] = Pt<PT>::from_row(piece);
      }
#pragma unroll
      for (int u_ = 0; u_ < 4; ++u_) {
        double d[3];
        Pt<PT>::delta(have[u_] ? cj[u_] : ci, ci, d);
        cov_add_d(acc, d[0], d[1], d[2]);
        n_have += have[u_] ? 1 : 0;
      }
    } else {
#pragma unroll
      for (int u_ = 0; u_ < 4; ++u_)
        if (4 * t + u_ < nslots) n_have += slot_add<PT, MISS>(tile, cap, ci, pre[4 * t + u_], acc);
    }
  }
  return n_have;
}

constexpr int kTrip = 8;
template <typename PT>
__device__ __forceinline__ int gather_tail(const int4* tile, int cap, const typename Pt<PT>::Raw& ci, const uint16_t* lrow,
                                           int nslots, bool packed, CovAcc& acc) {
  constexpr int XR = Pt<PT>::kRow16;
  int n_have = 0;
  uint32_t nxt[kTrip];
#pragma unroll
  for (int u_ = 0; u_ < kTrip; ++u_) nxt[u_] = (kPreSlots + u_ < nslots) ? (uint32_t)lrow[(kPreSlots + u_) * kBlock] : kNoLoc;
  for (int q0 = kPreSlots; q0 < nslots; q0 += kTrip) {
    uint32_t l[kTrip];
#pragma unroll
    for (int u_ = 0; u_ < kTrip; ++u_) l[u_] = nxt[u_];
    if (packed && __all((int)(l[0] == kNoLoc))) break;
#pragma unroll
    for (int u_ = 0; u_ < kTrip; ++u_) nxt[u_] = (q0 + kTrip + u_ < nslots) ? (uint32_t)lrow[(q0 + kTrip + u_) * kBlock] : kNoLoc;
    typename Pt<PT>::Raw cj[kTrip];
#pragma unroll
    for (int u_ = 0; u_ < kTrip; ++u_) {
      int4 piece[XR];
      read_row<XR>(tile, cap, l[u_] != kNoLoc ? l[u_] : 0u, piece);
      cj[u_] = Pt<PT>::from_row(piece);
    }
#pragma unroll
    for (int u_ = 0; u_ < kTrip; ++u_) {
      const bool have = l[u_] != kNoLoc;
      double d[3];
      Pt<PT>::delta(have ? cj[u_] : ci, ci, d);
      cov_add_d(acc, d[0], d[1], d[2]);
      n_have += have ? 1 : 0;
    }
  }
  return n_have;
}

template <typename T, typename PT, bool FULL_EIG>
__global__ __launch_bounds__(kBlock) void consistency_fwd_staged_kernel(
    const PT* __restrict__ x, BlockTab tab, int cap, const int32_t* __restrict__ centre_idx, int64_t n,
    const uint8_t* __restrict__ mask, const T* __restrict__ offset, LossParams lp, QParams qp, PT* __restrict__ rec,
    T* __restrict__ pointwise, T* __restrict__ eigvals, double* __restrict__ partials) {
  constexpr int XR = Pt<PT>::kRow16;
  extern __shared__ int4 tile[];
  const int64_t nblocks = (n + kBlock - 1) / kBlock;
  const int64_t blk = xcd_block(nblocks);
  double acc2[2] = {0.0, 0.0};
  const int4* xg = reinterpret_cast<const int4*>(x);
  const int64_t i = blk * kBlock + threadIdx.x;
  const bool live = blk >= 0 && i < n;
  typename Pt<PT>::Raw ci;
  int32_t nslots = 0;
  const uint16_t* lrow = tab.loc;
  uint32_t pre[kPreSlots];
  if (blk >= 0) {
    const int32_t s0 = tab.slot_ptr[blk];
    nslots = tab.slot_ptr[blk + 1] - s0;
    lrow = tab.loc + (int64_t)s0 * kBlock + threadIdx.x;
    if (live) ci = Pt<PT>::from_row(xg + (centre_idx ? (int64_t)centre_idx[i] : i) * XR);
#pragma unroll
    for (int q = 0; q < kPreSlots; ++q) pre[q] = (live && q < nslots) ? (uint32_t)lrow[q * kBlock] : kNoLoc;
    stage_rows<XR>(tab.blk_ptr, tab.blk_ids, blk, xg, tile, cap);
  }
  __syncthreads();
  if (live) {
    CovAcc acc;
    cov_init(acc);
    bool miss = false;
#pragma unroll
    for (int q = 0; q < kPreSlots; ++q) miss |= (q < nslots) && pre[q] == kNoLoc;
    int n_have = 0;
    if (__any((int)miss)) n_have = gather_slots<PT, true>(tile, cap, ci, pre, nslots, acc);
    else n_have = gather_slots<PT, false>(tile, cap, ci, pre, nslots, acc);
    for (int q = kPreSlots; q < nslots; ++q) {
      const uint32_t l = lrow[q * kBlock];
      n_have += slot_add<PT, true>(tile, cap, ci, l, acc);
    }
    acc.W = (double)n_have;
    consistency_point<T, PT, FULL_EIG>(acc, ci, i, mask, offset, lp, qp, rec, pointwise, eigvals, acc2);
  }
  wave_partials<2>(acc2, partials);
}

template <typename PT, int NS, bool MISS>
__device__ __forceinline__ int gather_fixed(const int4* tile, int cap, const typename Pt<PT>::Raw& ci, const uint32_t* pre,
                                            CovAcc& acc) {
  constexpr int XR = Pt<PT>::kRow16;
  int n_have = 0;
#pragma unroll
  for (int q0 = 0; q0 < NS; q0 += 4) {
    typename Pt<PT>::Raw cj[4];
    bool have[4];
#pragma unroll
    for (int u_ = 0; u_ < 4; ++u_) {
      if (q0 + u_ < NS) {
        have[u_] = !MISS || pre[q0 + u_] != kNoLoc;
        int4 piece[XR];
        read_row<XR>(tile, cap, have[u_] ? pre[q0 + u_] : 0u, piece);
        cj[u_] = Pt<PT>::from_row(piece);
      }
    }
#pragma unroll
    for (int u_ = 0; u_ < 4; ++u_) {
      if (q0 + u_ < NS) {
        double d[3];
        Pt<PT>::delta(have[u_] ? cj[u_] : ci, ci, d);
        cov_add_d(acc, d[0], d[1], d[2]);
        n_have += have[u_] ? 1 : 0;
      }
    }
  }
  return n_have;
}

template <typename T, typename PT, bool FULL_EIG, int NS>
__global__ __launch_bounds__(kBlock) void consistency_fwd_fixed_kernel(
    const PT* __restrict__ x, BlockTab tab, int cap, const int32_t* __restrict__ centre_idx, int64_t n,
    const uint8_t* __restrict__ mask, const T* __restrict__ offset, LossParams lp, QParams qp, PT* __restrict__ rec,
    T* __restrict__ pointwise, T* __restrict__ eigvals, double* __restrict__ partials) {
  constexpr int XR = Pt<PT>::kRow16;
  extern __shared__ int4 tile[];
  const int64_t nblocks = (n + kBlock - 1) / kBlock;
  const int64_t blk = xcd_block(nblocks);
  double acc2[2] = {0.0, 0.0};
  const int32_t s0 = blk >= 0 ? tab.slot_ptr[blk] : 0;
  const bool bad = blk >= 0 && tab.slot_ptr[blk + 1] - s0 != NS;
  if (blk >= 0 && !bad) {
    const int4* xg = reinterpret_cast<const int4*>(x);
    const int64_t i = blk * kBlock + threadIdx.x;
    const bool live = i < n;
    const uint16_t* lrow = tab.loc + (int64_t)s0 * kBlock + threadIdx.x;
    uint32_t pre[NS];
#pragma unroll
    for (int q = 0; q < NS; ++q) pre[q] = (uint32_t)lrow[q * kBlock];
    typename Pt<PT>::Raw ci = Pt<PT>::from_row(xg + (live ? (centre_idx ? (int64_t)centre_idx[i] : i) : 0) * XR);
    stage_rows<XR>(tab.blk_ptr, tab.blk_ids, blk, xg, tile, cap);
    __syncthreads();
    if (live) {
      CovAcc acc;
      cov_init(acc);
      uint32_t mx = pre[0];
#pragma unroll
      for (int q = 1; q < NS; ++q) mx = max(mx, pre[q]);
      int n_have;
      if (__any((int)(mx == kNoLoc))) n_have = gather_fixed<PT, NS, true>(tile, cap, ci, pre, acc);
      else n_have = gather_fixed<PT, NS, false>(tile, cap, ci, pre, acc);
      acc.W = (double)n_have;
      consistency_point<T, PT, FULL_EIG>(acc, ci, i, mask, offset, lp, qp, rec, pointwise, eigvals, acc2);
    }
  } else {
    __syncthreads();
  }
  if (bad) acc2[0] = acc2[1] = __longlong_as_double(0x7ff8000000000000ll);
  wave_partials<2>(acc2, partials);
}

template <typename T, typename PT, bool WANT_E, bool WANT_POSE>
__global__ __launch_bounds__(kBlock) void consistency_bwd_staged_kernel(
    const PT* __restrict__ x, const PT* __restrict__ rec, BlockTab tab, int cap, int64_t n, PointInputs in, QParams qp,
    T* __restrict__ grad_points, double* __restrict__ partials, int n_acc) {
  constexpr int want_e = WANT_E, want_pose = WANT_POSE;
  constexpr int RR = RecRaw<PT>::kRow16, XR = Pt<PT>::kRow16;
  extern __shared__ int4 tile[];
  __shared__ double lds[(kBlock / kWave) * 2 * DC_MAX_MODEL_TERMS];
  __shared__ double s_pose[kLdsScans * 12];
  const PoseTile poses = in.dirs ? stage_poses(in, s_pose) : PoseTile{nullptr};
  const int64_t nblocks = (n + kBlock - 1) / kBlock;
  const int64_t blk = xcd_block(nblocks);
  ModelParams mp;
  load_model(in, mp);
  double gw[DC_MAX_MODEL_TERMS], ge[DC_MAX_MODEL_TERMS], gT[6];
#pragma unroll
  for (int k = 0; k < DC_MAX_MODEL_TERMS; ++k) gw[k] = ge[k] = 0.0;
#pragma unroll
  for (int k = 0; k < 6; ++k) gT[k] = 0.0;
  int scan = -1;
  const int64_t j = blk * kBlock + threadIdx.x;
  const bool active = blk >= 0 && j < n;
  typename Pt<PT>::Raw cj;
  PointRaw<T> raw;
  uint32_t pre[kPreSlots];
  int32_t nslots = 0;
  uint32_t nd = 0;
  const uint16_t* lrow = tab.loc;
  if (blk >= 0) {
    const int32_t s0 = tab.slot_ptr[blk];
    nslots = tab.slot_ptr[blk + 1] - s0;
// ... 244 lines not shown
                                                                int64_t rows_fwd, int64_t rows_bwd, int n_red, int n_out,
                                                                double* __restrict__ out, AdamArgs adam,
                                                                const int32_t* __restrict__ status, int pose_first = -1,
                                                                int pose_cols = 0) {
  __shared__ double lds[kRedBlock / kWave * kPoseRedCols];
  const int a = blockIdx.x;
  if (a == 0)
    for (int z = 2 + n_red + threadIdx.x; z < n_out; z += kRedBlock) out[z] = 0.0;
  const int lane = threadIdx.x & (kWave - 1), wave = threadIdx.x / kWave;
  if (pose_first >= 0 && a >= 2 + pose_first) {
    const int col = (a - 2 - pose_first) * kPoseRedCols + (threadIdx.x & (kPoseRedCols - 1));
    const bool have = col < pose_cols;
    const double* p = p_bwd + (int64_t)pose_first * rows_bwd + (have ? col : 0);
    double s = strided_sum(p, have ? rows_bwd / kWavesPerBlock : 0, pose_cols, threadIdx.x / kPoseRedCols, kRedBlock / kPoseRedCols);
#pragma unroll
    for (int o = kPoseRedCols; o < kWave; o <<= 1) s += __shfl_xor(s, o, kWave);
    if (lane < kPoseRedCols) lds[wave * kPoseRedCols + lane] = s;
    __syncthreads();
    if (threadIdx.x < kPoseRedCols && have) {
      double t = 0.0;
      for (int wv = 0; wv < kRedBlock / kWave; ++wv) t += lds[wv * kPoseRedCols + threadIdx.x];
      out[2 + pose_first + col] = t;
    }
    return;
  }
  const bool flagged = a == 0 && threadIdx.x == 0 && status && *status != 0;
  const int64_t n_rows = a < 2 ? rows_fwd : rows_bwd;
  const double* p = a < 2 ? p_fwd + (int64_t)a * rows_fwd : p_bwd + (int64_t)(a - 2) * rows_bwd;
  const bool step = adam.p && a >= 2 && a - 2 < adam.n && threadIdx.x == 0;
  double p0 = 0.0, m0 = 0.0, v0 = 0.0;
  if (step) { p0 = adam.p[a - 2]; m0 = adam.m[a - 2]; v0 = adam.v[a - 2]; }
  const double s = wave_sum(strided_sum(p, n_rows));
  if (lane == 0) lds[wave] = s;
  __syncthreads();
  if (threadIdx.x == 0) {
    double t = 0.0;
    for (int wv = 0; wv < kRedBlock / kWave; ++wv) t += lds[wv];
    if (flagged) t = __longlong_as_double(0x7ff8000000000000ll);
    out[a] = t;
    if (step) adam_apply(adam, a - 2, t, p0, m0, v0);
  }
}

static inline unsigned red_grid(int n_red, int pose_first, int pose_cols) {
  if (pose_first < 0 || n_red <= pose_first) return 2u + (unsigned)n_red;
  return 2u + (unsigned)pose_first + (unsigned)((pose_cols + kPoseRedCols - 1) / kPoseRedCols);
}

__global__ void adam_kernel(const double* __restrict__ grad, AdamArgs adam) {
  const int i = (int)(blockIdx.x * blockDim.x + threadIdx.x);
  if (i < adam.n) adam_update(adam, i, grad[i]);
}

__global__ __launch_bounds__(256) void adam_device_step_kernel(const double* __restrict__ grad, AdamArgs adam, int64_t* __restrict__ step) {
  const double t = (double)(*step + 1);
  adam.bias1 = 1.0 - pow(adam.b1, t);
  adam.bias2_sqrt = sqrt(1.0 - pow(adam.b2, t));
  for (int i = threadIdx.x; i < adam.n; i += blockDim.x) adam_update(adam, i, grad[i]);
  __syncthreads();
  if (threadIdx.x == 0) *step = (int64_t)t;
}

}

using namespace dc;

#define DC_CHECK_LAUNCH()                                  \
  do {                                                     \
    hipError_t err__ = hipGetLastError();                  \
    if (err__ != hipSuccess) return (int)err__;            \
  } while (0)

static inline int64_t n_blocks(int64_t n) { return (n + kBlock - 1) / kBlock; }
static std::atomic<bool> g_no_tab{false};
static std::atomic<int> g_fwd_generic{0};
static std::atomic<bool> g_no_basis{false};
static std::atomic<bool> g_two_pass{false};
static std::atomic<int> g_chain_spin{1 << 22};
static std::atomic<int> g_step_var{1};
static std::atomic<bool> g_pose_three_pass{false};
static std::atomic<bool> g_no_reverse{false};
static std::atomic<bool> g_step_six{false};
static std::atomic<bool> g_no_step_rows{false};

template <int P, int CAP>
static int ragged_launch(dim3 grid, hipStream_t stream, hipEvent_t ev0, hipEvent_t ev1, const PointBasis& pb, const BlockTab& tab,
                         const dcBlockTable* t, int64_t n_rows, const uint8_t* mask, const LossParams& lp, const QParams& qp, double* p_fwd,
                         double* p_bwd, const StepChain& ch) {
  constexpr size_t bytes = (size_t)StepRow<q32, P>::kPieces * CAP * 16;
  static_assert(bytes >= step_hand_bytes<P>(), "the hand-over of step_block_row lives in the tile");
  static std::atomic<uint64_t> attr_set{0};
  if (bytes > 60 * 1024) {
    int dev = 0;
    if (hipGetDevice(&dev) != hipSuccess) dev = 0;
    const uint64_t bit = 1ull << (dev & 63);
    if (!(attr_set.fetch_or(bit) & bit)) {
      hipError_t err = hipFuncSetAttribute((const void*)consistency_step_ragged_q32_kernel<P, CAP>, hipFuncAttributeMaxDynamicSharedMemorySize, (int)bytes);
      if (err != hipSuccess) { attr_set.fetch_and(~bit); return (int)err; }
    }
  }
  hipExtLaunchKernelGGL((consistency_step_ragged_q32_kernel<P, CAP>), grid, dim3(kBlock), bytes, stream, ev0, ev1, 0, pb, tab, t->own_base, t->row_ptr, n_rows,
                        mask, lp, qp, p_fwd, p_bwd, ch);
  return DC_OK;
}

static_assert(kRouteBlock == kBlock && kRouteXcds == kXcds && kRouteWavesPerBlock == kWavesPerBlock && kRouteLdsScans == kLdsScans &&
              kRouteMaxBlockScans == kMaxBlockScans && kRouteStepQ32Cap == kStepQ32Cap && kRouteChainFront == kChainFront, "dc_cons_route.h");
static_assert(route_xcd_grid(1) == xcd_grid(1) && route_xcd_grid(8) == xcd_grid(8) && route_xcd_grid(7813) == xcd_grid(7813), "dc_cons_route.h");
static_assert(route_step_row_bytes(false, 1) == StepRow<q32, 1>::kPieces * 16 && route_step_row_bytes(false, 2) == StepRow<q32, 2>::kPieces * 16 &&
              route_step_row_bytes(false, 3) == StepRow<q32, 3>::kPieces * 16 && route_step_row_bytes(true, 1) == StepRow<double, 1>::kPieces * 16 &&
              route_step_row_bytes(true, 2) == StepRow<double, 2>::kPieces * 16 && route_step_row_bytes(true, 3) == StepRow<double, 3>::kPieces * 16, "dc_cons_route.h");
static_assert(route_x_row_bytes(false) == RowBytes<q32>::x && route_x_row_bytes(true) == RowBytes<double>::x &&
              route_rec_row_bytes(false) == RowBytes<q32>::rec && route_rec_row_bytes(true) == RowBytes<double>::rec, "dc_cons_route.h");

static inline RouteOptions route_options() {
  RouteOptions o;
  o.no_tab = g_no_tab.load(); o.fwd_generic = g_fwd_generic.load(); o.no_basis = g_no_basis.load(); o.two_pass = g_two_pass.load();
  o.step_var = g_step_var.load(); o.pose_three_pass = g_pose_three_pass.load(); o.step_six = g_step_six.load();
  return o;
}

#define DC_SWITCH_K(k, OTHER, M, ...) \
  do { switch (k) { case 10: M(10, __VA_ARGS__); break; case 4: M(4, __VA_ARGS__); break; case 8: M(8, __VA_ARGS__); break; \
                    case 16: M(16, __VA_ARGS__); break; default: { OTHER; } } } while (0)
#define DC_SWITCH_P(p, OTHER, M, ...) \
  do { if ((p) == 2) M(2, __VA_ARGS__); else if ((p) == 1) M(1, __VA_ARGS__); else { OTHER; } } while (0)

extern "C" {

int dc_version(void) { return 100; }

int64_t dc_partial_rows(int64_t n) { return route_xcd_grid(route_blocks(n)) * kRouteWavesPerBlock; }

int dc_param_grad_count(int n_terms, int n_scans) { return 2 * n_terms + 12 * n_scans; }

int64_t dc_sequence_partials_count(int64_t n, int n_terms, int n_scans) { return route_partials_count(n, n_terms, n_scans); }

static PointInputs make_inputs(const void* vps, const void* dirs, const void* depth, const void* inc,
                               const uint8_t* lmask, const int32_t* scan_id, const double* poses, int n_scans,
                               int model_kind, int n_terms, const double* w, const double* e) {
  PointInputs in;
  in.vps = vps; in.dirs = dirs; in.depth = depth; in.inc = inc; in.lmask = lmask; in.scan_id = scan_id;
  in.poses = poses; in.w = w; in.e = e; in.model_kind = model_kind; in.n_terms = n_terms; in.n_scans = n_scans;
  return in;
}

static int check_model(int model_kind, int n_terms, const void* inc, const double* w, const double* e) {
  if (model_kind < DC_MODEL_NONE || model_kind > DC_MODEL_LAST) return DC_ERR_ARG;
  if (model_kind != DC_MODEL_NONE) {
    if (n_terms < 1 || n_terms > DC_MAX_MODEL_TERMS || !inc || !w || !e) return DC_ERR_ARG;
    if (model_kind == DC_MODEL_LINEAR && n_terms != 3) return DC_ERR_ARG;
    if ((model_kind == DC_MODEL_INVCOS || model_kind == DC_MODEL_SCALED_INVCOS) && n_terms != 1) return DC_ERR_ARG;
  }
  return DC_OK;
}

static int make_qparams(int point_fmt, int dtype, int stride, const double* qparams, QParams* qp, int32_t* flag = nullptr) {
  *qp = QParams{};
  qp->flag = flag;
  if (point_fmt == DC_Q32) {
    if (!qparams || stride != 4 || dtype != DC_F32 || !(qparams[3] > 0.0)) return DC_ERR_ARG;
    qp->origin[0] = qparams[0]; qp->origin[1] = qparams[1]; qp->origin[2] = qparams[2];
    qp->scale = qparams[3];
    qp->inv_scale = 1.0 / qparams[3];
    return DC_OK;
  }
  return point_fmt == dtype ? DC_OK : DC_ERR_DTYPE;
}

#define DC_DISPATCH_FMT(dtype, fmt, stride, LAUNCH)                       \
  do {                                                                    \
    if ((fmt) == DC_Q32) { LAUNCH(float, q32, 4); }                       \
    else if ((dtype) == DC_F32) { if ((stride) == 3) { LAUNCH(float, float, 3); } else { LAUNCH(float, float, 4); } } \
    else if ((dtype) == DC_F64) { if ((stride) == 3) { LAUNCH(double, double, 3); } else { LAUNCH(double, double, 4); } } \
    else return DC_ERR_DTYPE;                                             \
  } while (0)

int dc_points_fwd(const void* vps, const void* dirs, const void* depth, const void* inc, const uint8_t* lmask,
                  const int32_t* scan_id, const double* poses, int n_scans, int model_kind, int n_terms,
                  const double* w, const double* e, int64_t n, int dtype, int point_fmt, const double* qparams,
                  int out_stride, void* points_out, void* vps_out, void* dirs_out, void* depth_out, int32_t* status,
                  hipStream_t stream) {
  if (n == 0) return DC_OK;
  if (n < 0 || !dirs || !depth || !points_out || (out_stride != 3 && out_stride != 4)) return DC_ERR_ARG;
  if (scan_id && (!poses || n_scans < 1)) return DC_ERR_ARG;
  int rc = check_model(model_kind, n_terms, inc, w, e);
  if (rc) return rc;
  QParams qp;
  rc = make_qparams(point_fmt, dtype, out_stride, qparams, &qp, status);
  if (rc) return rc;
  if (n == 0) return DC_OK;
  if (model_kind == DC_MODEL_NONE) n_terms = 0;
  PointInputs in = make_inputs(vps, dirs, depth, inc, lmask, scan_id, poses, n_scans, model_kind, n_terms, w, e);
  dim3 grid((unsigned)n_blocks(n)), block(kBlock);
#define LAUNCH(T, PT, S) \
  DC_TIMED_LAUNCH((points_fwd_kernel<T, PT, S>), grid, block, 0, stream, in, n, qp, (PT*)points_out, (T*)vps_out, (T*)dirs_out, (T*)depth_out)
  { ProfScope prof(0); DC_DISPATCH_FMT(dtype, point_fmt, out_stride, LAUNCH); }
#undef LAUNCH
  DC_CHECK_LAUNCH();
  return DC_OK;
}

int dc_points_basis(const void* vps, const void* dirs, const void* depth, const void* inc, const uint8_t* lmask,
                    const int32_t* scan_id, const double* poses, int n_scans, int model_kind, int n_terms, const double* e,
                    int64_t n, int dtype, const double* qparams, void* rows_out, int32_t* status, hipStream_t stream) {
  if (n == 0) return DC_OK;
  if (n < 0 || !dirs || !depth || !rows_out) return DC_ERR_ARG;
  if (scan_id && (!poses || n_scans < 1)) return DC_ERR_ARG;
  if (dtype != DC_F32 && dtype != DC_F64) return DC_ERR_DTYPE;
  if (dtype == DC_F32 && !qparams) return DC_ERR_ARG;
  int rc = check_model(model_kind, n_terms, inc, e, e);
  if (rc || model_kind == DC_MODEL_NONE) return rc ? rc : DC_ERR_ARG;
  QParams qp;
  rc = make_qparams(dtype == DC_F32 ? DC_Q32 : DC_F64, dtype, 4, qparams, &qp, status);
  if (rc) return rc;
  PointInputs in = make_inputs(vps, dirs, depth, inc, lmask, scan_id, poses, n_scans, model_kind, n_terms, e, e);
  if (dtype == DC_F32)
    hipLaunchKernelGGL((points_basis_kernel<q32>), dim3((unsigned)n_blocks(n)), dim3(kBlock), 0, stream, in, n, qp, rows_out);
  else
    hipLaunchKernelGGL((points_basis_kernel<double>), dim3((unsigned)n_blocks(n)), dim3(kBlock), 0, stream, in, n, qp, rows_out);
  DC_CHECK_LAUNCH();
  return DC_OK;
}

int dc_step_rows_build(const dcBlockTable* table, int64_t n_rows, const void* basis, int row_words, void* rows_out, hipStream_t stream) {
  if (!table || n_rows < 0 || table->layout != DC_TABLE_SLOTS || !table->blk_ptr || row_words < 7 || row_words > 6 + 3) return DC_ERR_ARG;
  if (n_rows == 0) return DC_OK;
  if (!table->blk_ids || !basis || !rows_out || ((uintptr_t)rows_out & 15)) return DC_ERR_ARG;
  hipLaunchKernelGGL(step_rows_kernel, dim3((unsigned)n_blocks(n_rows)), dim3(kBlock), 0, stream, table->blk_ptr, table->blk_ids,
                     static_cast<const int32_t*>(basis), row_words, static_cast<int32_t*>(rows_out));
  DC_CHECK_LAUNCH();
  return DC_OK;
}

int dc_points_local_basis(const void* dirs, const void* depth, const void* inc, const uint8_t* lmask, const int32_t* scan_id,
                          int model_kind, int n_terms, const double* e, int64_t n, int dtype, const dcPoseTable* table, void* rows_out,
                          hipStream_t stream) {
  if (n == 0) return DC_OK;
  if (n < 0 || !dirs || !depth || !rows_out || n_terms < 1 || n_terms > 2 || !table || !table->blk_ptr || !table->ids) return DC_ERR_ARG;
  if (dtype != DC_F32) return DC_ERR_DTYPE;
  int rc = check_model(model_kind, n_terms, inc, e, e);
  if (rc || model_kind == DC_MODEL_NONE) return rc ? rc : DC_ERR_ARG;
  PointInputs in = make_inputs(nullptr, dirs, depth, inc, lmask, scan_id, nullptr, 1, model_kind, n_terms, e, e);
  PoseTab tab{table->blk_ptr, table->ids, table->loc, table->own_pos, table->row_seg, table->row_scan};
  hipLaunchKernelGGL((points_local_basis_kernel<float>), dim3((unsigned)n_blocks(n)), dim3(kBlock), 0, stream, in, tab, (int32_t*)rows_out);
  DC_CHECK_LAUNCH();
  return DC_OK;
}

int dc_pose_table_build(const dcBlockTable* fwd, const int32_t* scan_id, int64_t n, int n_scans, int k, int32_t* ids_out,
                        uint16_t* loc_out, uint16_t* own_pos, uint16_t* row_seg, uint8_t* row_scan, int32_t* info, hipStream_t stream) {
  if (!fwd || fwd->layout != DC_TABLE_SLOTS || !fwd->blk_ptr || !fwd->blk_ids || !fwd->slot_ptr || !fwd->loc || !fwd->own_base) return DC_ERR_ARG;
  if (n < 1 || n_scans < 1 || n_scans > kMaxBlockScans || !ids_out || !loc_out || !own_pos || !row_seg || !row_scan || !info) return DC_ERR_ARG;
  if (k != 4 && k != 8 && k != 10 && k != 16) return DC_ERR_UNSUPPORTED;
  hipError_t err = hipMemsetAsync(info, 0, sizeof(int32_t), stream);
  if (err != hipSuccess) return (int)err;
  BlockTab tab{fwd->blk_ptr, fwd->blk_ids, fwd->slot_ptr, fwd->loc};
  const dim3 grid((unsigned)n_blocks(n)), block(kBlock);
#define PT_K(KK) hipLaunchKernelGGL((pose_table_kernel<KK>), grid, block, 0, stream, tab, fwd->own_base, scan_id, n, n_scans, ids_out, loc_out, own_pos, \
                                    row_seg, row_scan, info)
  if (k == 10) PT_K(10); else if (k == 4) PT_K(4); else if (k == 8) PT_K(8); else PT_K(16);
#undef PT_K
  DC_CHECK_LAUNCH();
  return DC_OK;
}

static int consistency_fwd_impl(const void* points, int stride, int dtype, int point_fmt, const double* qparams,
                                const int32_t* nbr, const int32_t* centre_idx, const dcBlockTable* table, int64_t n, int k,
                                const uint8_t* mask,
                                const void* offset, int loss_kind,
                                int normalization, int sqrt_, void* rec, void* pointwise, void* eigvals, double* partials_ws,
                                double* sums_out, hipStream_t stream, bool reduce) {
  if (n == 0 && sums_out) return (int)hipMemsetAsync(sums_out, 0, 2 * sizeof(double), stream);
  if (n < 0 || k < 1 || !points || !partials_ws || !sums_out || (stride != 3 && stride != 4)) return DC_ERR_ARG;
  if ((loss_kind & 0xFF) != DC_LOSS_MIN_EIGVAL && (loss_kind & 0xFF) != DC_LOSS_TRACE) return DC_ERR_ARG;
  if (loss_kind & ~(0xFF | DC_LOSS_RAW_POINTWISE | DC_LOSS_SKIP_NANS | DC_LOSS_ONLY_FINITE)) return DC_ERR_ARG;
  BlockTab tab{};
  size_t lds_bytes = 0;
  int lds_rows = 0;
  const bool staged = use_table(table, g_no_tab.load(), DC_TABLE_SLOTS, stride, point_fmt == DC_F64 ? 32u : 16u, 0, 60 * 1024, &lds_bytes, &lds_rows);
  if (staged) tab = BlockTab{table->blk_ptr, table->blk_ids, table->slot_ptr, table->loc};
  const int fixed_k = g_fwd_generic.load() ? 0 : k;
  if (!staged && !nbr) return table ? DC_ERR_UNSUPPORTED : DC_ERR_ARG;
  QParams qp;
  int rc = make_qparams(point_fmt, dtype, stride, qparams, &qp);
  if (rc) return rc;
  if (n == 0) return (int)hipMemsetAsync(sums_out, 0, 2 * sizeof(double), stream);
  const LossParams lp = make_loss_params(loss_kind, normalization, sqrt_);
  const int64_t rows = xcd_grid(n_blocks(n));
  dim3 grid((unsigned)rows), block(kBlock);
#define FWD_ARGS(T, PT) (const PT*)points, nbr, centre_idx, n, k, mask, (const T*)offset, lp, qp, (PT*)rec, (T*)pointwise, (T*)eigvals, partials_ws
#define FWD_STAGED_ARGS(T, PT) (const PT*)points, tab, lds_rows, centre_idx, n, mask, (const T*)offset, lp, qp, (PT*)rec, (T*)pointwise, (T*)eigvals, partials_ws
#define DC_SWITCH_EIG(M, ...) do { if (eigvals) M(true, __VA_ARGS__); else M(false, __VA_ARGS__); } while (0)
#define FWD_FIXED(EIG, T, PT, NS) DC_TIMED_LAUNCH((consistency_fwd_fixed_kernel<T, PT, EIG, NS>), grid, block, lds_bytes, stream, FWD_STAGED_ARGS(T, PT))
#define FWD_STAGED(EIG, T, PT) DC_TIMED_LAUNCH((consistency_fwd_staged_kernel<T, PT, EIG>), grid, block, lds_bytes, stream, FWD_STAGED_ARGS(T, PT))
#define FWD_GATHER(EIG, T, PT, S) DC_TIMED_LAUNCH((consistency_fwd_kernel<T, PT, S, EIG>), grid, block, 0, stream, FWD_ARGS(T, PT))
#define FWD_FIXED_K(NS, T, PT) DC_SWITCH_EIG(FWD_FIXED, T, PT, NS)
#define LAUNCH(T, PT, S) \
  do { \
    if (S == 4 && staged) DC_SWITCH_K(fixed_k, DC_SWITCH_EIG(FWD_STAGED, T, PT), FWD_FIXED_K, T, PT);    \
    else DC_SWITCH_EIG(FWD_GATHER, T, PT, S); \
  } while (0)
  { ProfScope prof(1); DC_DISPATCH_FMT(dtype, point_fmt, stride, LAUNCH); }
#undef LAUNCH
#undef FWD_FIXED_K
#undef FWD_GATHER
#undef FWD_STAGED
#undef FWD_FIXED
#undef DC_SWITCH_EIG
  DC_CHECK_LAUNCH();
  if (!reduce) return DC_OK;
  hipLaunchKernelGGL(reduce_partials_kernel, dim3(2), dim3(kRedBlock), 0, stream, partials_ws, rows * kWavesPerBlock, sums_out);
  DC_CHECK_LAUNCH();
// ... 97 lines not shown
#undef BWD_GATHER
#undef BWD_STAGED
#undef BWD_RUNS
#undef DC_SWITCH_EP
  DC_CHECK_LAUNCH();
  if (params && n_red > 0 && reduce) {
    hipLaunchKernelGGL(reduce_partials_kernel, dim3(n_red), dim3(kRedBlock), 0, stream, partials_ws, prows, grads_out);
    DC_CHECK_LAUNCH();
  }
  return DC_OK;
}

int dc_consistency_bwd(const void* points, int stride, int dtype, int point_fmt, const double* qparams, const void* rec,
                       const int32_t* csr_ptr, const int32_t* csr_src, const uint8_t* lane_perm, const dcBlockTable* table,
                       int64_t n, const void* vps, const void* dirs, const void* depth, const void* inc, const uint8_t* lmask,
                       const int32_t* scan_id, const double* poses, int n_scans, int model_kind, int n_terms, const double* w,
                       const double* e, int want_exponent_grad, int want_pose_grad, void* grad_points, double* partials_ws,
                       double* grads_out, hipStream_t stream) {
  return consistency_bwd_impl(points, stride, dtype, point_fmt, qparams, rec, csr_ptr, csr_src, lane_perm, table, n, vps, dirs, depth,
                              inc, lmask, scan_id, poses, n_scans, model_kind, n_terms, w, e, want_exponent_grad,
                              want_pose_grad, grad_points, partials_ws, grads_out, stream, true, 0);
}

int dc_points_bwd(const void* grad_points, const int32_t* perm, int stride, int dtype, int64_t n, const void* vps,
                  const void* dirs, const void* depth, const void* inc, const uint8_t* lmask, const int32_t* scan_id,
                  const double* poses, int n_scans, int model_kind, int n_terms, const double* w, const double* e,
                  int want_exponent_grad, int want_pose_grad, double* partials_ws, double* grads_out,
                  hipStream_t stream) {
  if (n < 0 || !grad_points || !dirs || !depth || !partials_ws || !grads_out || (stride != 3 && stride != 4))
    return DC_ERR_ARG;
  if (scan_id && (!poses || n_scans < 1)) return DC_ERR_ARG;
  int rc = check_model(model_kind, n_terms, inc, w, e);
  if (rc) return rc;
  if (model_kind == DC_MODEL_NONE) n_terms = 0;
  const int n_acc = 2 * n_terms + 12 * n_scans;
  if (n_acc == 0) return DC_OK;
  if (n == 0) return (int)hipMemsetAsync(grads_out, 0, n_acc * sizeof(double), stream);
  PointInputs in = make_inputs(vps, dirs, depth, inc, lmask, scan_id, poses, n_scans, model_kind, n_terms, w, e);
  const int64_t rows = n_blocks(n);
  const int64_t prows = rows * kWavesPerBlock;
  dim3 grid((unsigned)rows), block(kBlock);
  const int n_red = want_pose_grad ? n_acc : 2 * n_terms;
  if (n_red < n_acc) {
    hipError_t err = hipMemsetAsync(grads_out + n_red, 0, (size_t)(n_acc - n_red) * sizeof(double), stream);
    if (err != hipSuccess) return (int)err;
  }
  if (n_red == 0) return DC_OK;
  if (want_pose_grad) {
    hipError_t err = hipMemsetAsync(partials_ws + (size_t)prows * 2 * n_terms, 0, (size_t)prows * 12 * n_scans * sizeof(double), stream);
    if (err != hipSuccess) return (int)err;
  }
#define LAUNCH(T, S) \
  hipLaunchKernelGGL((points_bwd_kernel<T, S>), grid, block, 0, stream, (const T*)grad_points, perm, n, in, \
                     want_exponent_grad, want_pose_grad, partials_ws, n_acc)
  if (dtype == DC_F32) { if (stride == 3) LAUNCH(float, 3); else LAUNCH(float, 4); }
  else if (dtype == DC_F64) { if (stride == 3) LAUNCH(double, 3); else LAUNCH(double, 4); }
  else return DC_ERR_DTYPE;
#undef LAUNCH
  DC_CHECK_LAUNCH();
  hipLaunchKernelGGL(reduce_partials_kernel, dim3(n_red), dim3(kRedBlock), 0, stream, partials_ws, prows, grads_out);
  DC_CHECK_LAUNCH();
  return DC_OK;
}

#ifdef DC_BLOCK_TRACE
int dc_debug_block_trace(void* buf) {
  unsigned long long* p = (unsigned long long*)buf;
  return (int)hipMemcpyToSymbol(HIP_SYMBOL(dc::g_block_trace), &p, sizeof(p));
}
#endif
int dc_set_option(int option, int value) {
  static const bool enabled = [] { const char* e = getenv("DC_ENABLE_ABLATIONS"); return e && atoi(e) != 0; }();
  if (!enabled) return DC_ERR_UNSUPPORTED;
  if (option == 0) { g_no_tab.store(value != 0); return DC_OK; }
  if (option == 1) { g_fwd_generic.store(value); return DC_OK; }
  if (option == 3) { g_no_basis.store(value != 0); return DC_OK; }
  if (option == 4) { g_two_pass.store(value != 0); return DC_OK; }
  if (option == 5) { g_chain_spin.store(value < 0 ? (1 << 22) : value); return DC_OK; }
  if (option == 6) { g_step_var.store(value); return DC_OK; }
  if (option == 7) { g_pose_three_pass.store(value != 0); return DC_OK; }
  if (option == 8) { g_no_reverse.store(value != 0); return DC_OK; }
  if (option == 9) { g_step_six.store(value != 0); return DC_OK; }
  if (option == 10) { g_no_step_rows.store(value != 0); return DC_OK; }
  return DC_ERR_ARG;
}

int dc_profiler_enable(int every) {
  std::lock_guard<std::mutex> lock(g_prof.mu);
  g_prof.every = every < 0 ? 0 : every;
  return DC_OK;
}
int dc_profiler_reset(void) {
  std::lock_guard<std::mutex> lock(g_prof.mu);
  for (int k = 0; k < kProfKinds; ++k) { g_prof.count[k] = 0; g_prof.seen[k] = 0; }
  return DC_OK;
}
int dc_profiler_kernel(int kind, char* buf, int len) {
  if (kind < 0 || kind >= kProfKinds || !buf || len < 1) return DC_ERR_ARG;
  const char* nm = g_prof.last_kernel[kind];
  snprintf(buf, (size_t)len, "%s", nm ? nm : "");
  return DC_OK;
}
int dc_profiler_read(int kind, double* total_ms, int64_t* launches) {
  if (kind < 0 || kind >= kProfKinds || !total_ms || !launches) return DC_ERR_ARG;
  double tot = 0.0;
  int n;
  { std::lock_guard<std::mutex> lock(g_prof.mu); n = g_prof.count[kind]; }
  for (int i = 0; i < n; ++i) {
    hipError_t err = hipEventSynchronize(g_prof.stop[kind][i]);
    if (err != hipSuccess) return (int)err;
    float ms = 0.f;
    err = hipEventElapsedTime(&ms, g_prof.start[kind][i], g_prof.stop[kind][i]);
    if (err != hipSuccess) return (int)err;
    tot += ms;
  }
  *total_ms = tot;
  *launches = n;
  return DC_OK;
}

static int make_adam(double* param, double* exp_avg, double* exp_avg_sq, int64_t n, int64_t step, double grad_scale, double lr,
                     double beta1, double beta2, double eps, double weight_decay, AdamArgs* a) {
  if (!param || !exp_avg || !exp_avg_sq || n < 0 || n > 0x7fffffff || step < 1) return DC_ERR_ARG;
  *a = AdamArgs{param, exp_avg, exp_avg_sq, (int)n, grad_scale, lr, beta1, beta2, eps, weight_decay,
                1.0 - pow(beta1, (double)step), sqrt(1.0 - pow(beta2, (double)step))};
  return DC_OK;
}

int dc_adam_step(double* param, const double* grad, double* exp_avg, double* exp_avg_sq, int64_t n, int64_t step,
                 double grad_scale, double lr, double beta1, double beta2, double eps, double weight_decay,
                 hipStream_t stream) {
  AdamArgs a;
  int rc = make_adam(param, exp_avg, exp_avg_sq, n, step, grad_scale, lr, beta1, beta2, eps, weight_decay, &a);
  if (rc || !grad) return rc ? rc : DC_ERR_ARG;
  if (n == 0) return DC_OK;
  hipLaunchKernelGGL(adam_kernel, dim3((unsigned)((n + 63) / 64)), dim3(64), 0, stream, grad, a);
  DC_CHECK_LAUNCH();
  return DC_OK;
}

int dc_adam_step_device(double* param, const double* grad, double* exp_avg, double* exp_avg_sq, int64_t n, int64_t* step,
                        double grad_scale, double lr, double beta1, double beta2, double eps, double weight_decay,
                        hipStream_t stream) {
  AdamArgs a;
  int rc = make_adam(param, exp_avg, exp_avg_sq, n, 1, grad_scale, lr, beta1, beta2, eps, weight_decay, &a);
  if (rc || !grad || !step) return rc ? rc : DC_ERR_ARG;
  hipLaunchKernelGGL(adam_device_step_kernel, dim3(1), dim3(256), 0, stream, grad, a, step);
  DC_CHECK_LAUNCH();
  return DC_OK;
}

struct ChainCall {
  int32_t* ready;
  int parity, has_prev;
  double* out_prev;
  AdamArgs adam_prev;
  const double* grad_sum;
  bool reduce_now;
  double* w_prev_out = nullptr;
  uint32_t stamp = 0;
  const double* prev_rows = nullptr;
  int64_t prev_count = 0;
  const double* acc_in = nullptr;
  const int32_t* prev_status = nullptr;
};
static inline double* chain_buffer(const dcSequenceDesc* d, int n_terms, int parity) {
  const int64_t rows = route_seq_rows(d).rows;
  const int n_acc = 2 * n_terms + 12 * d->n_scans;
  return d->partials + (int64_t)(2 + n_acc) * rows + (int64_t)parity * (2 + n_terms) * rows;
}
static StepChain make_chain(const ChainCall& c, int n_out, const double* own_prev, int64_t own_rows, int32_t* status, int spin_limit,
                            const double* w_now, int reverse) {
  StepChain ch{};
  ch.ready = c.ready; ch.stamp = c.stamp; ch.parity = c.parity; ch.has_prev = c.has_prev; ch.n_front = kChainFront; ch.n_out = n_out;
  ch.reverse = reverse;
  ch.prev = c.prev_rows ? c.prev_rows : own_prev; ch.prev_rows = c.prev_rows ? c.prev_count : own_rows;
  ch.grad_sum = c.grad_sum; ch.out_prev = c.out_prev; ch.w_prev_out = c.w_prev_out; ch.status = status; ch.spin_limit = spin_limit;
  ch.w_now = w_now; ch.prev_status = c.prev_status; ch.acc_in = c.acc_in; ch.adam = c.adam_prev;
  return ch;
}

struct StepLaunch {
  const dcSequenceDesc* d; hipStream_t stream; dim3 grid; PointBasis pb; BlockTab tab; LossParams lp; QParams qp; double *p_fwd, *p_bwd; StepChain ch;
};

static int launch_step_ragged(const SeqRoute& r, const StepLaunch& a) {
  ProfScope prof(1);
#define RAGGED(P, CAP) (prof.name("(consistency_step_ragged_q32_kernel<" #P ", " #CAP ">)"), \
                        ragged_launch<P, CAP>(a.grid, a.stream, prof.start(), prof.stop(), a.pb, a.tab, r.table, r.n_rows, a.d->mask, a.lp, a.qp, a.p_fwd, a.p_bwd, a.ch))
#define RAGGED_CAPS(P, X) do { switch (r.cap) { case 1024: return RAGGED(P, 1024); case 1280: return RAGGED(P, 1280); case 1600: return RAGGED(P, 1600); \
                                                case 2048: return RAGGED(P, 2048); case 2560: return RAGGED(P, 2560); default: return RAGGED(P, 4096); } } while (0)
  DC_SWITCH_P(r.P, switch (r.cap) { case 1024: return RAGGED(3, 1024); case 1600: return RAGGED(3, 1600); default: return RAGGED(3, 2560); }, RAGGED_CAPS, 0);
#undef RAGGED_CAPS
#undef RAGGED
  return DC_OK;
}

static int launch_step_q32(const SeqRoute& r, const StepLaunch& a) {
  ProfScope prof(1);
  const StepHdr* hdr = static_cast<const StepHdr*>(a.d->step_hdr);
  const int32_t* step_rows = g_no_step_rows.load() ? nullptr : static_cast<const int32_t*>(a.d->step_rows);
  const dim3 block(kBlock);
  static_assert(kStepQ32Cap == 512, "the profiler names the instantiation by its literal arguments");
  static_assert(step_q32_blocks<1, 512>() == 7 && step_q32_blocks<2, 512>() == 7 && step_q32_blocks<3, 512>() == 6 && step_q32_blocks<2, 768>() == 6,
                "which instantiations dc_set_option(9, 1) has a six-block build of");
#define STEPQ_TAIL a.pb, a.tab, hdr, step_rows, a.d->centre_idx, r.n_rows, a.lp, a.qp, a.p_fwd, a.p_bwd, a.ch
#define STEPQ(P, NS, CAP) DC_TIMED_LAUNCH((consistency_step_q32_kernel<NS, P, CAP>), a.grid, block, 0, a.stream, STEPQ_TAIL)
#define STEPQ_SIX(P, NS, X) DC_TIMED_LAUNCH((consistency_step_q32_kernel<NS, P, 512, 6>), a.grid, block, 0, a.stream, STEPQ_TAIL)
#define STEPQ_P(NS, CAP) DC_SWITCH_P(r.P, STEPQ(3, NS, CAP), STEPQ, NS, CAP)
#define STEPQ_SIX_P(NS, X) DC_SWITCH_P(r.P, , STEPQ_SIX, NS, X)
  if (r.six) DC_SWITCH_K(r.k, , STEPQ_SIX_P, 0);
  else if (r.cap == 512) DC_SWITCH_K(r.k, , STEPQ_P, 512);
  else DC_SWITCH_K(r.k, , STEPQ_P, 768);
#undef STEPQ_SIX_P
#undef STEPQ_P
#undef STEPQ_SIX
#undef STEPQ
#undef STEPQ_TAIL
  return DC_OK;
}

#define STEP_TAIL a.pb, a.tab, r.table->own_base, r.rows_fwd, a.d->centre_idx, r.n_rows, a.d->mask, a.lp, a.qp, a.p_fwd, a.p_bwd, a.ch
static size_t step_lds(const SeqRoute& r, const StepLaunch& a, size_t hand_bytes) {
  return a.ch.ready && r.lds_fwd < hand_bytes ? hand_bytes : r.lds_fwd;
}
static int launch_step_basis(const SeqRoute& r, const StepLaunch& a) {
  ProfScope prof(1);
  const dim3 block(kBlock);
#define STEPB(P, NS, PT) DC_TIMED_LAUNCH((consistency_step_basis_kernel<PT, NS, P, kStepVar>), a.grid, block, step_lds(r, a, step_hand_bytes<P>()), a.stream, STEP_TAIL)
#define STEPB_P(NS, PT) DC_SWITCH_P(r.P, STEPB(3, NS, PT), STEPB, NS, PT)
  if (r.round2 && r.f64) DC_TIMED_LAUNCH((consistency_step_basis_kernel<double, 10, 2, 0>), a.grid, block, step_lds(r, a, step_hand_bytes<2>()), a.stream, STEP_TAIL);
  else if (r.round2) DC_TIMED_LAUNCH((consistency_step_basis_kernel<q32, 10, 2, 0>), a.grid, block, step_lds(r, a, step_hand_bytes<2>()), a.stream, STEP_TAIL);
  else if (r.f64) DC_SWITCH_K(r.k, , STEPB_P, double);
  else DC_SWITCH_K(r.k, , STEPB_P, q32);
#undef STEPB_P
#undef STEPB
  return DC_OK;
}

static int launch_step_slots(const SeqRoute& r, const StepLaunch& a) {
  ProfScope prof(1);
  const dim3 block(kBlock);
#define STEPS(P, PT, X) DC_TIMED_LAUNCH((consistency_step_basis_slots_kernel<PT, P>), a.grid, block, step_lds(r, a, step_hand_bytes<P>()), a.stream, STEP_TAIL, r.table->packed)
  if (r.f64) DC_SWITCH_P(r.P, STEPS(3, double, 0), STEPS, double, 0);
  else DC_SWITCH_P(r.P, STEPS(3, q32, 0), STEPS, q32, 0);
#undef STEPS
  return DC_OK;
}
#undef STEP_TAIL

static int run_one_pass(const SeqRoute& r, const dcSequenceDesc* d, const double* w, double* out, hipStream_t stream, const AdamArgs& adam,
                        const ChainCall* chain) {
  StepLaunch a{};
  int rc = make_qparams(d->point_fmt, d->dtype, 4, d->qparams, &a.qp);
  if (rc) return rc;
  a.d = d; a.stream = stream; a.grid = dim3((unsigned)r.grid);
  a.pb = PointBasis{d->basis, w, r.n_terms, r.f64 ? 1.0 : a.qp.inv_scale};
  a.lp = make_loss_params(d->loss_kind & ~DC_LOSS_RAW_POINTWISE, d->normalization, d->sqrt_);
  a.tab = BlockTab{r.table->blk_ptr, r.table->blk_ids, r.table->slot_ptr, r.table->loc};
  a.p_fwd = chain ? chain_buffer(d, r.n_terms, chain->parity) : d->partials;
  a.p_bwd = chain ? a.p_fwd + 2 * r.g_blocks : d->partials + 2 * r.rows;
  if (chain) a.ch = make_chain(*chain, 2 + r.n_acc, chain_buffer(d, r.n_terms, chain->parity ^ 1), r.g_blocks, d->status, g_chain_spin.load(), w,
                               (chain->parity && !g_no_reverse.load()) ? 1 : 0);
  a.ch.blk_skip = (d->mask && !d->centre_idx) ? d->blk_skip : nullptr;
  switch (r.kind) {
    case ROUTE_STEP_RAGGED: rc = launch_step_ragged(r, a); break;
    case ROUTE_STEP_Q32: rc = launch_step_q32(r, a); break;
    case ROUTE_STEP_BASIS: rc = launch_step_basis(r, a); break;
    default: rc = launch_step_slots(r, a); break;
  }
  if (rc) return rc;
  DC_CHECK_LAUNCH();
  if (chain && !chain->reduce_now) return DC_OK;
  const int64_t rows_g = chain ? r.g_blocks : r.grid * kWavesPerBlock;
  hipLaunchKernelGGL(reduce_eval_kernel, dim3(2 + r.n_terms), dim3(kRedBlock), 0, stream, a.p_fwd, a.p_bwd, rows_g, rows_g, r.n_terms, 2 + r.n_acc, out,
                     chain ? AdamArgs{} : adam, (const int32_t*)d->status);
  DC_CHECK_LAUNCH();
  return DC_OK;
}

static int run_two_pass(const SeqRoute& r, const dcSequenceDesc* d, const double* w, int want_grad, double* out, hipStream_t stream,
                        const AdamArgs& adam) {
  QParams qp;
  int rc = make_qparams(d->point_fmt, d->dtype, 4, d->qparams, &qp);
  if (rc) return rc;
  const PointBasis pb{d->basis, w, r.n_terms, r.f64 ? 1.0 : qp.inv_scale};
  const LossParams lp = make_loss_params(d->loss_kind & ~DC_LOSS_RAW_POINTWISE, d->normalization, d->sqrt_);
  const BlockTab tab{r.table->blk_ptr, r.table->blk_ids, r.table->slot_ptr, r.table->loc};
  const dim3 block(kBlock);
// ... 244 lines not shown
```

### depth_correction_amd/plan.py

```python
from __future__ import annotations

import ctypes

import os

import numpy as np

import torch

from . import ops
from . import _native as nv
from ._native import need, lib, check, ptr, stream_ptr, on_device

__all__ = ['SequencePlan', 'SequenceTrainer', 'consistency_loss', 'KernelTimer', 'PlanRegistry']


class SequencePlan:
    kMaskGroup = 2048

    @on_device
    def __init__(self, clouds, poses, neighbors, mask=None, model_kind='ScaledPolynomial', loss='min_eigval_loss',
                 normalization=True, sqrt=False, spatial_sort=True, point_format='auto', degree_sort=False,
                 active_only=False, block_tables=True, bwd_layout='runs', stages=None, basis=True, lazy_backward=True,
                 scan_group=True, mask_first=False, nan_policy=None, pose_kernel=True, degree_group=False, heavy_first=False,
                 wave_pack=None, step_rows=True):
        mark = stages.mark if stages is not None else (lambda name: None)
        get = (lambda c, f: c[f]) if isinstance(clouds[0], dict) else getattr
        vps = ops.cat_rows([get(c, 'vps') for c in clouds])
        dirs = ops.cat_rows([get(c, 'dirs') for c in clouds])
        depth = ops.cat_rows([get(c, 'depth') for c in clouds]).reshape(-1)
        incs = [get(c, 'inc_angles') for c in clouds]
        inc = None if incs[0] is None else ops.cat_rows(incs).reshape(-1)
        lms = [get(c, 'mask') for c in clouds]
        dev = dirs.device
        sizes = [len(get(c, 'dirs')) for c in clouds]
        lmask = None if lms[0] is None else ops.cat_rows(lms)
        scan_id = ops.scan_ids(sizes, dev)
        self.n, self.n_scans, self.device, self.dtype = dirs.shape[0], len(clouds), dev, dirs.dtype
        self._poses_key = self._poses12 = self._poses_ref = None
        self.sizes = sizes
        self.model_kind, self.loss, self.normalization, self.sqrt = model_kind, loss, bool(normalization), bool(sqrt)
        assert nan_policy in (None, 'skip_nans', 'only_finite')
        self.nan_policy = nan_policy
        g = getattr(neighbors, '_dc_graph', None)
        nbr = g.nbr if g is not None and g.version == neighbors._version else ops.as_index32(neighbors)
        need(nbr, (self.n, None), dtype=torch.int32, name='neighbors', device=dev)
        self.k = nbr.shape[1]
        if mask is not None:
            need(mask, (self.n,), dtype=torch.bool, name='mask', device=dev)

        mark('plan_concat')
        ps0 = ops.PointSet(vps if bool(vps.any()) else None, dirs, depth, inc, lmask, scan_id)
        P0 = self.poses12(poses)
        x0 = ops.points_fwd(ps0, P0)
        mark('plan_points0')
        if spatial_sort and self.n > 1:
            order = ops.spatial_order(x0).long()
            mark('plan_morton_order')
            if degree_sort:
                valid = nbr[nbr >= 0].long()
                deg = torch.bincount(valid, minlength=self.n)[order]
                nb = (self.n + 255) // 256
                pad = torch.full((nb * 256,), 2 ** 40, dtype=torch.int64, device=dev)
                pad[:self.n] = deg
                local = torch.argsort(pad.reshape(nb, 256), dim=1, stable=True)
                pos = (local + torch.arange(nb, device=dev)[:, None] * 256).reshape(-1)
                order = order[pos[pos < self.n]]
            self.scan_seg, self.skipped_wavefronts, self.blk_skip = None, 0.0, None
            if wave_pack is None:
                wave_pack = nbr.shape[1] <= 10 and not heavy_first and not degree_group
            if wave_pack and mask is not None and not degree_sort and not active_only and not mask_first and self.n >= 4 * 256:
                m_o = mask[order]
                pos = torch.arange(self.n, device=dev)
                pa, pb = pos[m_o], pos[~m_o]
                na, nb_ = pa.numel(), pb.numel()
                big = torch.iinfo(torch.int64).max
                ka = pa[::64].clone()
                kb = pb[::64].clone()
                if na % 64 and ka.numel():
                    ka[-1] = big - 1
                if nb_ % 64 and kb.numel():
                    kb[-1] = big
                keys = torch.cat([ka, kb])
                runs = torch.argsort(keys, stable=True)
                start = torch.cat([torch.arange(ka.numel(), device=dev) * 64, na + torch.arange(kb.numel(), device=dev) * 64])[runs]
                length = torch.cat([torch.full((ka.numel(),), 64, device=dev), torch.full((kb.numel(),), 64, device=dev)])
                if na % 64 and ka.numel():
                    length[ka.numel() - 1] = na % 64
                if nb_ % 64 and kb.numel():
                    length[-1] = nb_ % 64
                length = length[runs]
                off = torch.cumsum(length, 0) - length
                idx = torch.repeat_interleave(start - off, length) + pos
                order = order[torch.cat([pa, pb])[idx]]
                self._wave_packed = True
                mark('plan_wave_pack')
            if mask_first and mask is not None and not degree_sort and not active_only:
                sb = torch.arange(self.n, device=dev) // self.kMaskGroup
                order = order[torch.argsort(sb * 2 + (~mask[order]).long(), stable=True)]
                mark('plan_mask_first')
            by_degree = bool(degree_group) and scan_group and not degree_sort
            deg = None
            if heavy_first and scan_group and not degree_sort and self.n // 256 > 8:
                deg = (nbr >= 0).sum(1)
                nbf, per = self.n // 256, ((self.n + 255) // 256 + 7) // 8
                b = torch.arange(per * 8, device=dev)
                logical = (b % 8) * per + b // 8
                logical = logical[logical < nbf]
# ... 38 lines not shown
            self.order, self.rank = order, rank
            mark('plan_permute')
        else:
            self.order = self.rank = None
            self.scan_seg, self.skipped_wavefronts, self.blk_skip = None, 0.0, None
        if not bool(vps.any()):
            vps = None
        self.ps = ops.PointSet(vps, dirs, depth, inc, lmask, scan_id)
        self.nbr_full, self.mask_full = nbr, mask
        self.centre_idx = None
        if active_only and mask is not None:
            self.centre_idx = torch.nonzero(mask).reshape(-1).to(torch.int32).contiguous()
            nbr = nbr[self.centre_idx.long()].contiguous()
            mask = None
        self.nbr, self.mask = nbr, mask
        self._csr = self._bwd_table = None
        self._bwd_layout, self._block_tables = bwd_layout, bool(block_tables)
        if not lazy_backward:
            self.ensure_backward_tables()
        mark('plan_transpose')
        self.lane_perm = None
        self.fwd_table = None
        if block_tables:
            ragged = nbr.shape[1] > 16 and nbr.shape[0] > 0 and bool((nbr[:, -1] < 0).any())
            if ragged:
                self.fwd_table = ops.block_table(csr=ops.table_to_csr(nbr), layout='slots', own_rows='csr' if self.centre_idx is None else False)
            else:
                self.fwd_table = ops.block_table(nbr=nbr, own_rows=self.centre_idx is None)
        self.fwd_rows_active = self.fwd_rows_active_loss = 0
        self.fwd_table_loss = None
        if (block_tables and self.fwd_table is not None and mask is not None and self.centre_idx is None and nbr.shape[1] <= 16
                and nbr.shape[0] > 0 and getattr(self, '_wave_packed', False)):
            rows_ = torch.arange(self.n, device=dev, dtype=torch.int32)[:, None]
            nbr_loss = torch.where(mask[:, None] | (nbr == rows_), nbr, torch.full_like(nbr, -1)).contiguous()
            self.fwd_table_loss = ops.block_table(nbr=nbr_loss, own_rows=True)
            del nbr_loss
        if self.fwd_table is not None and getattr(self, 'blk_skip', None) is not None and self.centre_idx is None:
            keep = self.blk_skip.cpu().numpy() == 0
            rows_per_block = np.diff(self.fwd_table.blk_ptr.cpu().numpy())
            self.fwd_rows_active = int(rows_per_block[keep].max()) if keep.any() else 0
            if self.fwd_table_loss is not None:
                rows_per_block = np.diff(self.fwd_table_loss.blk_ptr.cpu().numpy())
                self.fwd_rows_active_loss = int(rows_per_block[keep].max()) if keep.any() else 0
        self.step_hdr = None
        ft = self.fwd_table_loss or self.fwd_table
        if ft is not None and ft.slot_ptr is not None:
            self.step_hdr = torch.empty((max((nbr.shape[0] + 255) // 256, 1), 16), dtype=torch.int32, device=dev)
            m8 = None if mask is None else mask.view(torch.uint8)
            skip = self.blk_skip if (mask is not None and self.centre_idx is None) else None
            check(lib().dc_step_header_build(ft.ref(), nbr.shape[0], ptr(m8), ptr(skip), ptr(self.step_hdr), stream_ptr()),
                  'dc_step_header_build')
        mark('plan_block_tables')
        self.count = float(nbr.shape[0] if mask is None else int(mask.sum().item()))

        self.qfmt = None
        self.status = torch.zeros((1,), dtype=torch.int32, device=dev)
        if point_format in ('auto', 'q32') and self.dtype == torch.float32:
            lo, hi = ops.points_extent(x0)
            qfmt = ops.QFormat.for_extent(lo, hi)
            if point_format == 'q32' or qfmt.scale <= ops.QFormat.MAX_AUTO_SCALE:
                self.qfmt = qfmt
            else:
                point_format = 'f64'
        elif point_format == 'q32':
            raise TypeError('the q32 point format goes with float32 clouds')
        if point_format == 'f64' and self.dtype == torch.float32:
            ps = self.ps
            up = lambda t: None if t is None else t.double()
            self.ps = ops.PointSet(up(ps.vps), up(ps.dirs), up(ps.depth), up(ps.inc), ps.lmask, ps.scan_id)
            self.dtype = torch.float64
        self.point_format = 'q32' if self.qfmt is not None else ('f64' if self.dtype == torch.float64 else 'f32')
        pdt = torch.int32 if self.qfmt is not None else self.dtype
        self.x = torch.empty((self.n, 4), dtype=pdt, device=dev)
        self.rec = torch.empty((nbr.shape[0], 8), dtype=pdt, device=dev)
        self.partials = torch.empty((ops.lib().dc_sequence_partials_count(self.n, ops.nv.MAX_MODEL_TERMS, self.n_scans),),
                                    dtype=torch.float64, device=dev)
        self.version = 0
        self._desc = None
        self.use_basis = bool(basis)
        self.use_pose_kernel = bool(pose_kernel)
        self._pose_table = self._local_basis = None
        self._basis = None
        self.use_step_rows = bool(step_rows)
        self._poses_key = self._poses12 = self._poses_ref = None

    @on_device
    def ensure_backward_tables(self):
        if self._csr is None:
            self._csr = ops.knn_transpose(self.nbr, n_dst=self.n)
            self._bwd_table = ops.block_table(csr=self._csr, layout=self._bwd_layout) if self._block_tables else None
            self._desc = None
        return self._csr

    csr_ptr = property(lambda self: self.ensure_backward_tables()[0])
    csr_src = property(lambda self: self.ensure_backward_tables()[1])

    @property
    def bwd_table(self):
        self.ensure_backward_tables()
        return self._bwd_table

    def desc(self, n_terms):
        if self._desc is None or self._desc.n_terms != n_terms:
            d = nv.SequenceDesc()
            d.n, d.k, d.n_scans = self.n, self.k, self.n_scans
            d.dtype = nv.DC_F32 if self.dtype == torch.float32 else nv.DC_F64
            d.point_fmt = nv.DC_Q32 if self.qfmt is not None else d.dtype
            if self.qfmt is not None:
                for i in range(4):
                    d.qparams[i] = self.qfmt._c[i]
            p = lambda t: None if t is None else t.data_ptr()
            ps = self.ps
            d.vps, d.dirs, d.depth, d.inc, d.lmask, d.scan_id = p(ps.vps), p(ps.dirs), p(ps.depth), p(ps.inc), p(ps.lmask), p(ps.scan_id)
            csr = self._csr or (None, None)
            d.nbr, d.csr_ptr, d.csr_src, d.mask = p(self.nbr), p(csr[0]), p(csr[1]), p(self.mask)
            d.lane_perm = p(self.lane_perm)
            d.fwd_table = None if self.fwd_table is None else self.fwd_table.ref()
            ftl = getattr(self, 'fwd_table_loss', None)
            d.fwd_table_loss = None if ftl is None else ftl.ref()
            d.fwd_rows_active_loss = int(getattr(self, 'fwd_rows_active_loss', 0)) if ftl is not None else 0
            d.bwd_table = None if self._bwd_table is None else self._bwd_table.ref()
            d.centre_idx, d.n_centres = p(self.centre_idx), (0 if self.centre_idx is None else self.centre_idx.shape[0])
            d.x, d.rec, d.partials = p(self.x), p(self.rec), p(self.partials)
            d.partials_count = self.partials.numel()
            d.status = p(self.status)
            d.scan_seg = p(getattr(self, 'scan_seg', None))
            skip = getattr(self, 'blk_skip', None) if (self.mask is not None and self.centre_idx is None) else None
            d.blk_skip, d.fwd_rows_active = p(skip), int(getattr(self, 'fwd_rows_active', 0)) if skip is not None else 0
            d.step_hdr = p(getattr(self, 'step_hdr', None))
            d.model_kind = nv.MODEL_KINDS[self.model_kind] if n_terms > 0 else 0
            d.n_terms = n_terms
            d.loss_kind, d.normalization, d.sqrt_ = nv.LOSS_KINDS[self.loss], int(self.normalization), int(self.sqrt)
            d.loss_kind |= {None: 0, 'skip_nans': nv.DC_LOSS_SKIP_NANS, 'only_finite': nv.DC_LOSS_ONLY_FINITE}[self.nan_policy]
            if d.model_kind != 0 and ps.inc is None:
                raise ValueError('the model needs incidence angles')
            self._desc = d
        return self._desc

    def _set_pose_tables(self, d, w, exponent, want_grad, want_exponent, want_pose):
        ok = (self.use_pose_kernel and want_grad and want_pose and not want_exponent and w is not None and w.numel() in (1, 2)
              and self.qfmt is not None and self.ps.vps is None and self.centre_idx is None and self.fwd_table is not None
              and self.fwd_table.own_base is not None and self.k in (4, 8, 10, 16) and self.n_scans <= 32
              and d.model_kind != 0 and self._block_tables and self.nbr.shape[1] == self.k)
        if ok and self._pose_table is None:
            self._pose_table = self._build_pose_table()
        if not ok or self._pose_table is False:
            d.pose_table = d.local_basis = None
            return
        nt = w.numel()
        key = (exponent.data_ptr(), exponent._version, nt, d.model_kind)
        lb = self._local_basis
        if lb is None or lb[0] != key:
            ps = self.ps
            rows = torch.empty((max(self._pose_table[1]['ids'].numel(), 1), 6), dtype=torch.int32, device=self.device)
            check(lib().dc_points_local_basis(ptr(ps.dirs), ptr(ps.depth), ptr(ps.inc), ptr(ps.lmask), ptr(ps.scan_id), d.model_kind, nt,
                                              ptr(exponent), self.n, nv.DC_F32, ctypes.byref(self._pose_table[0]), ptr(rows),
                                              stream_ptr()), 'dc_points_local_basis')
            self._local_basis = lb = (key, rows, exponent)
        d.pose_table = ctypes.cast(ctypes.pointer(self._pose_table[0]), ctypes.c_void_p)
        d.local_basis = lb[1].data_ptr()

    def _build_pose_table(self):
        ft, dev, nb = (getattr(self, 'fwd_table_loss', None) or self.fwd_table), self.device, (self.n + 255) // 256
        total = int(ft.blk_ptr[-1].item())
        t = dict(ids=torch.empty((max(total, 1),), dtype=torch.int32, device=dev),
                 loc=torch.empty((nb * self.k * 256,), dtype=torch.uint16, device=dev),
                 own_pos=torch.empty((self.n,), dtype=torch.uint16, device=dev),
                 row_seg=torch.empty((nb * (self.n_scans + 1),), dtype=torch.uint16, device=dev),
                 row_scan=torch.empty((max(total, 1),), dtype=torch.uint8, device=dev))
        info = torch.zeros((1,), dtype=torch.int32, device=dev)
        check(lib().dc_pose_table_build(ft.ref(), ptr(self.ps.scan_id), self.n, self.n_scans, self.k, ptr(t['ids']), ptr(t['loc']),
                                        ptr(t['own_pos']), ptr(t['row_seg']), ptr(t['row_scan']), ptr(info), stream_ptr()),
              'dc_pose_table_build')
        if int(info.item()) != 0:
            return False
        desc = nv.PoseTableDesc(ptr(ft.blk_ptr), ptr(t['ids']), ptr(t['loc']), ptr(t['own_pos']), ptr(t['row_seg']),
                                ptr(t['row_scan']))
        return desc, t

    def _set_basis(self, d, w, exponent, poses12, want_exponent, want_pose, stepping=True):
        f64 = self.qfmt is None and self.x.dtype == torch.float64 and self.ps.dirs.dtype == torch.float64
        ok = (self.use_basis and (self.qfmt is not None or f64) and w is not None
              and not want_exponent and not want_pose
              and self.fwd_table is not None and self._block_tables and self._bwd_layout == 'runs'
              and d.model_kind != 0)
        if not ok:
            d.basis = d.step_rows = None
            return
        nt = w.numel()
        b = self._basis
        key = (poses12.data_ptr(), poses12._version, exponent.data_ptr(), exponent._version, nt)
        if b is None or b[0] != key:
            ps = self.ps
            rows = torch.empty((self.n, 6 + nt), dtype=torch.float64 if f64 else torch.int32, device=self.device)
            check(lib().dc_points_basis(ptr(ps.vps), ptr(ps.dirs), ptr(ps.depth), ptr(ps.inc), ptr(ps.lmask), ptr(ps.scan_id),
                                        ptr(poses12), self.n_scans, d.model_kind, nt, ptr(exponent), self.n,
                                        nv.DC_F64 if f64 else nv.DC_F32, None if f64 else self.qfmt._c, ptr(rows),
                                        ptr(self.status), stream_ptr()), 'dc_points_basis')
            self._basis = b = [key, rows, poses12, exponent, None, 0]
        d.basis = b[1].data_ptr()
        if stepping:
            b[5] += 1
        ft = getattr(self, 'fwd_table_loss', None) or self.fwd_table
        if (b[4] is None and b[5] >= 2 and self.use_step_rows and self.qfmt is not None and nt <= 3 and self.n > 0
                and getattr(self, 'step_hdr', None) is not None and ft.blk_ids is not None):
            if getattr(self, '_step_rows_total', None) is None:
                self._step_rows_total = int(ft.blk_ptr[-1].item())
            b[4] = torch.empty((max(self._step_rows_total, 1) * (6 + nt),), dtype=torch.int32, device=self.device)
            check(lib().dc_step_rows_build(ft.ref(), self.nbr.shape[0], ptr(b[1]), 6 + nt, ptr(b[4]), stream_ptr()), 'dc_step_rows_build')
        d.step_rows = None if (b[4] is None or not self.use_step_rows) else b[4].data_ptr()

    @on_device
    def eval_native(self, w, exponent, poses12, out, want_grad=True, want_exponent=False, want_pose=False):
        nt = 0 if w is None else w.numel()
        d = self.desc(nt)
        need(poses12, (self.n_scans, 12), dtype=torch.float64, name='poses12', device=self.device)
        need(out, (2 + 2 * nt + 12 * self.n_scans,), dtype=torch.float64, name='out', device=self.device)
        if nt:
            need(w, (nt,), dtype=torch.float64, name='w', device=self.device)
            need(exponent, (nt,), dtype=torch.float64, name='exponent', device=self.device)
        for attempt in (0, 1):
            self._set_basis(d, w, exponent, poses12, want_exponent, want_pose)
            self._set_pose_tables(d, w, exponent, want_grad, want_exponent, want_pose)
            rc = lib().dc_sequence_eval(ctypes.byref(d), ptr(w), ptr(exponent), ptr(poses12), int(want_grad),
                                        int(want_exponent), int(want_pose), ptr(out), stream_ptr())
            if rc != nv.DC_ERR_BACKWARD_TABLES or attempt:
                break
            self.ensure_backward_tables()
            d = self.desc(nt)
        check(rc, 'dc_sequence_eval')
        self.version += 1
        return out

    @on_device
    def step_native(self, w, exponent, poses12, out, exp_avg, exp_avg_sq, t, grad_scale, lr, betas, eps, weight_decay):
        nt = w.numel()
        d = self.desc(nt)
        need(poses12, (self.n_scans, 12), dtype=torch.float64, name='poses12', device=self.device)
        need(out, (2 + 2 * nt + 12 * self.n_scans,), dtype=torch.float64, name='out', device=self.device)
        for name, v in (('w', w), ('exponent', exponent), ('exp_avg', exp_avg), ('exp_avg_sq', exp_avg_sq)):
            need(v, (nt,), dtype=torch.float64, name=name, device=self.device)
        for attempt in (0, 1):
            self._set_basis(d, w, exponent, poses12, False, False)
            rc = lib().dc_sequence_step(ctypes.byref(d), ptr(w), ptr(exponent), ptr(poses12), ptr(exp_avg), ptr(exp_avg_sq),
                                        int(t), float(grad_scale), float(lr), float(betas[0]), float(betas[1]), float(eps),
                                        float(weight_decay), ptr(out), stream_ptr())
            if rc != nv.DC_ERR_BACKWARD_TABLES or attempt:
                break
            self.ensure_backward_tables()
            d = self.desc(nt)
        check(rc, 'dc_sequence_step')
        self.version += 1
        return out

    @on_device
    def step_chained(self, w, exponent, poses12, out_prev, exp_avg, exp_avg_sq, t, has_prev, ready, grad_scale, lr, betas, eps,
                     weight_decay, w_used_prev=None):
        nt = w.numel()
        d = self.desc(nt)
        need(out_prev, (2 + 2 * nt + 12 * self.n_scans,), dtype=torch.float64, name='out_prev', device=self.device)
        if w_used_prev is not None:
            need(w_used_prev, (nt,), dtype=torch.float64, name='w_used_prev', device=self.device)
            for name, v in (('w', w), ('exponent', exponent), ('exp_avg', exp_avg), ('exp_avg_sq', exp_avg_sq)):
                need(v, (nt,), dtype=torch.float64, name=name, device=self.device)
            need(ready, (16,), dtype=torch.int32, name='ready', device=self.device)
            self._set_basis(d, w, exponent, poses12, False, False)
            rc = lib().dc_sequence_step_chained_rec(ctypes.byref(d), ptr(w), ptr(exponent), ptr(poses12), ptr(exp_avg), ptr(exp_avg_sq),
                                                    int(t), int(bool(has_prev)), float(grad_scale), float(lr), float(betas[0]),
                                                    float(betas[1]), float(eps), float(weight_decay), ptr(ready), ptr(out_prev),
                                                    ptr(w_used_prev), stream_ptr())
            if rc in (-4, nv.DC_ERR_BACKWARD_TABLES):
                return False
            check(rc, 'dc_sequence_step_chained_rec')
            self.version += 1
            return True
        need(ready, (16,), dtype=torch.int32, name='ready', device=self.device)
        for name, v in (('w', w), ('exponent', exponent), ('exp_avg', exp_avg), ('exp_avg_sq', exp_avg_sq)):
            need(v, (nt,), dtype=torch.float64, name=name, device=self.device)
        self._set_basis(d, w, exponent, poses12, False, False)
        rc = lib().dc_sequence_step_chained(ctypes.byref(d), ptr(w), ptr(exponent), ptr(poses12), ptr(exp_avg), ptr(exp_avg_sq),
                                            int(t), int(bool(has_prev)), float(grad_scale), float(lr), float(betas[0]),
                                            float(betas[1]), float(eps), float(weight_decay), ptr(ready), ptr(out_prev), stream_ptr())
        if rc in (-4, nv.DC_ERR_BACKWARD_TABLES):
            return False
        check(rc, 'dc_sequence_step_chained')
        self.version += 1
        return True

    @on_device
    def step_linked(self, prev_plan, prev_parity, finish, acc_in, w, exponent, poses12, exp_avg, exp_avg_sq, step, stamp, ready, out_prev,
                    grad_scale, lr, betas, eps, weight_decay, w_used_prev=None):
        nt = w.numel()
        d = self.desc(nt)
# ... 576 lines not shown
```

### include/dc_hip.h

```cpp
#ifndef DC_HIP_H
#define DC_HIP_H

#include <stddef.h>
#include <stdint.h>

#ifdef __cplusplus
extern "C" {
#endif

#ifndef DC_F32
#define DC_F32 0
#define DC_F64 1
#define DC_Q32 2
#define DC_LOSS_MIN_EIGVAL 0
#define DC_LOSS_TRACE 1
#define DC_LOSS_RAW_POINTWISE 0x100
#define DC_LOSS_SKIP_NANS 0x200
#define DC_LOSS_ONLY_FINITE 0x400
#define DC_MODEL_NONE 0
#define DC_MODEL_POLYNOMIAL 1
#define DC_MODEL_SCALED_POLYNOMIAL 2
#define DC_MODEL_LINEAR 3
#define DC_MODEL_INVCOS 4
#define DC_MODEL_SCALED_INVCOS 5
// ... 16 lines not shown
size_t dc_knn_workspace_bytes(int64_t n, int64_t n_query);
int dc_knn_set_shell_budget(int shells);
int dc_knn_set_fine_cell_count(int points);
int dc_knn_build(const void* points, int stride, int dtype, int64_t n, const void* query, int q_stride,
                 int64_t n_query, int k, double r, double cell_hint, int32_t* idx_out, double* dist_out, void* ws,
                 size_t ws_bytes, dcStream_t stream);
int dc_knn_build_i64(const void* points, int stride, int dtype, int64_t n, const void* query, int q_stride,
                 int64_t n_query, int k, double r, double cell_hint, int32_t* idx_out, int64_t* idx64_out, double* dist_out, void* ws,
                 size_t ws_bytes, dcStream_t stream);

int dc_radius_count(const void* points, int stride, int dtype, int64_t n, double r, int32_t* count_out,
                    int32_t* kmax_out, void* ws, size_t ws_bytes, dcStream_t stream);
int dc_radius_fill(int64_t n, double r, int kmax, int32_t* idx_out, void* ws, size_t ws_bytes, dcStream_t stream);
int dc_radius_count_query(const void* points, int stride, int dtype, int64_t n, const void* query, int q_stride, int64_t n_query,
                          double r, int32_t* count_out, int32_t* kmax_out, void* ws, size_t ws_bytes, dcStream_t stream);
int dc_radius_fill_query(int64_t n, int64_t n_query, double r, int kmax, int32_t* idx_out, void* ws, size_t ws_bytes,
                         dcStream_t stream);

size_t dc_knn_transpose_workspace_bytes(int64_t n, int k);
size_t dc_scan_lattice_workspace_bytes(int n_scans);
int dc_scan_lattice_shift(const void* points, int dtype, int64_t n, const int64_t* scan_ptr, int n_scans, double* shifted, int32_t* info,
                          void* ws, size_t ws_bytes, dcStream_t stream);
int dc_scan_lattice_localize(int32_t* nbr, int64_t n, int k, const int64_t* scan_ptr, int n_scans, int32_t* info, dcStream_t stream);
size_t dc_points_extent_workspace_bytes(void);
int dc_points_extent(const void* points, int stride, int dtype, int64_t n, double* out6, void* ws, size_t ws_bytes, dcStream_t stream);
int dc_scan_ids(const int64_t* scan_ptr, int n_scans, int64_t n, int32_t* out, dcStream_t stream);
int dc_knn_transpose(const int32_t* nbr, int64_t n, int k, int64_t n_dst, int32_t* csr_ptr, int32_t* csr_src, void* ws,
                     size_t ws_bytes, dcStream_t stream);

size_t dc_spatial_order_workspace_bytes(int64_t n);
int dc_spatial_order(const void* points, int stride, int dtype, int64_t n, int32_t* order_out, void* ws,
                     size_t ws_bytes, dcStream_t stream);

int dc_points_fwd(const void* vps, const void* dirs, const void* depth, const void* inc, const uint8_t* lmask,
                  const int32_t* scan_id, const double* poses, int n_scans, int model_kind, int n_terms,
                  const double* w, const double* e, int64_t n, int dtype, int point_fmt, const double* qparams,
                  int out_stride, void* points_out, void* vps_out, void* dirs_out, void* depth_out, int32_t* status,
                  dcStream_t stream);

int dc_points_basis(const void* vps, const void* dirs, const void* depth, const void* inc, const uint8_t* lmask,
                    const int32_t* scan_id, const double* poses, int n_scans, int model_kind, int n_terms, const double* e,
                    int64_t n, int dtype, const double* qparams, void* rows_out, int32_t* status, dcStream_t stream);

int64_t dc_partial_rows(int64_t n);
int dc_param_grad_count(int n_terms, int n_scans);
int dc_points_bwd(const void* grad_points, const int32_t* perm, int stride, int dtype, int64_t n, const void* vps,
                  const void* dirs, const void* depth, const void* inc, const uint8_t* lmask, const int32_t* scan_id,
                  const double* poses, int n_scans, int model_kind, int n_terms, const double* w, const double* e,
                  int want_exponent_grad, int want_pose_grad, double* partials_ws, double* grads_out,
                  dcStream_t stream);

int dc_features_fwd(const void* points, int stride, int dtype, const int32_t* nbr, int64_t n, int k,
                    const void* mean_weights, double scale, const void* dirs, void* mean, void* cov, void* eigvals,
                    void* eigvecs, void* normals, void* inc_angles, int32_t* nvalid, void* weights_out,
                    void* cmean_out, void* invd_out, dcStream_t stream);

int dc_features_set_tiled(int on);

int dc_features_bwd(const void* points, int stride, int dtype, const int32_t* csr_ptr, const int32_t* csr_src,
                    int64_t n, const void* cmean, const void* invd, const int32_t* nvalid, const void* eigvecs,
                    const void* grad_mean, const void* grad_cov, const void* grad_eigvals, void* grec_ws,
                    void* grad_points, dcStream_t stream);

#define DC_TABLE_SLOTS 0
#define DC_TABLE_RUNS 1
typedef struct dcBlockTable {
  const int32_t* blk_ptr;
  const int32_t* blk_ids;
  const int32_t* slot_ptr;
  const uint16_t* loc;
  int32_t max_rows;
  int32_t layout;
  const int32_t* run_ptr;
  const int32_t* own_base;
  int32_t packed;
  int32_t reserved;
  const int32_t* row_ptr;
} dcBlockTable;
int dc_block_table_slots(const int32_t* row_ptr, int64_t n_rows, int k, int32_t* slot_cnt_ws, int32_t* slot_ptr,
                         dcStream_t stream);
int dc_step_header_build(const dcBlockTable* table, int64_t n_rows, const uint8_t* mask, const uint8_t* blk_skip, void* hdr_out,
                         dcStream_t stream);
int dc_step_rows_build(const dcBlockTable* table, int64_t n_rows, const void* basis, int row_words, void* rows_out, dcStream_t stream);
size_t dc_block_table_workspace_bytes(int64_t n_refs);
int dc_block_table_set_lds_build(int on);
size_t dc_block_table_slots_workspace_bytes(int64_t n_rows, int k);
int dc_block_table_build(const int32_t* row_ptr, const int32_t* ids, int64_t n_rows, int k, int64_t n_refs,
                         const int32_t* slot_ptr, int64_t n_slot_rows, int32_t* blk_ptr, int32_t* blk_ids, uint16_t* loc,
                         int32_t* info, void* ws, size_t ws_bytes, dcStream_t stream);
int dc_block_table_own_base(const int32_t* blk_ptr, const int32_t* blk_ids, int64_t n_rows, int32_t* own_base, dcStream_t stream);
int dc_block_group(const int32_t* order_in, const int32_t* scan_id, const uint8_t* mask, int64_t n, int n_scans, int32_t* order_out,
                   uint16_t* seg_out, uint8_t* blk_skip_out, int32_t* skipped_out, dcStream_t stream);
int dc_table_permute(const int32_t* nbr, int64_t n, int k, const int64_t* order, int32_t* rank_out, int32_t* nbr_out, dcStream_t stream);
int dc_gather_rows(const void* src, int row_bytes, const int64_t* order, int64_t n, void* dst, dcStream_t stream);
int64_t dc_block_table_run_capacity(int64_t n_rows, int64_t n_refs);
int dc_block_table_build_runs(const int32_t* row_ptr, const int32_t* ids, int64_t n_rows, int64_t n_refs, int32_t* run_ptr,
                              int32_t* blk_ptr, int32_t* blk_ids, uint16_t* loc, int32_t* info, void* ws, size_t ws_bytes,
                              dcStream_t stream);

int dc_consistency_fwd(const void* points, int stride, int dtype, int point_fmt, const double* qparams,
                       const int32_t* nbr, const int32_t* centre_idx, const dcBlockTable* table, int64_t n, int k,
                       const uint8_t* mask, const void* offset, int loss_kind, int normalization, int sqrt_, void* rec,
                       void* pointwise, void* eigvals, double* partials_ws, double* sums_out, dcStream_t stream);

int dc_consistency_bwd(const void* points, int stride, int dtype, int point_fmt, const double* qparams, const void* rec,
                       const int32_t* csr_ptr, const int32_t* csr_src, const uint8_t* lane_perm, const dcBlockTable* table,
                       int64_t n, const void* vps, const void* dirs,
                       const void* depth, const void* inc, const uint8_t* lmask, const int32_t* scan_id,
                       const double* poses, int n_scans, int model_kind, int n_terms, const double* w, const double* e,
                       int want_exponent_grad, int want_pose_grad, void* grad_points, double* partials_ws,
                       double* grads_out, dcStream_t stream);

int dc_mask_bounds(const void* num, int num_stride, int num_index, const void* den, int den_stride, int den_index,
                   int dtype, int64_t n, double lo, double hi, uint8_t* mask, dcStream_t stream);
int dc_valid_count(const int32_t* nbr, int64_t n, int k, int32_t* count_out, dcStream_t stream);
int dc_mask_bounds_multi(const void* values, int stride, int dtype, int64_t n, int n_bounds, const int32_t* num_index,
                         const int32_t* den_index, const double* lo, const double* hi, int init, uint8_t* mask, dcStream_t stream);
size_t dc_compact_rows_workspace_bytes(int64_t n);
int dc_compact_rows(const uint8_t* mask, int64_t n, int n_fields, const void* const* src, void* const* dst, const int32_t* row_bytes,
                    int32_t* index_out, int64_t* count_out, void* ws, size_t ws_bytes, dcStream_t stream);
int dc_to_points(const void* vps, int vps_rows, const void* dirs, const void* depth, int dtype, int64_t n, void* points_out,
                 dcStream_t stream);
size_t dc_scan_prefilter_workspace_bytes(int64_t n);
int dc_scan_prefilter(const void* points, int stride, int in_dtype, const void* vps, int64_t n, int out_dtype, double shadow_r,
                      double shadow_lo, double shadow_hi, void* vps_out, void* dirs_out, void* depth_out, void* points_out,
                      int64_t* count_out, void* ws, size_t ws_bytes, dcStream_t stream);
int dc_valid_weights(const int32_t* nbr, int64_t count, float* weights_out, dcStream_t stream);
size_t dc_nn1_corr_workspace_bytes(int64_t n);
int dc_nn1_corr(const double* dist, const int32_t* idx, int64_t n, double ratio, uint8_t* mask_out, int32_t* idx_out, int64_t* count_out,
                double* threshold_out, void* ws, size_t ws_bytes, dcStream_t stream);
int dc_dispersion(const void* vec, int dtype, const int32_t* nbr, const void* weights, int64_t n, int k, void* out,
                  dcStream_t stream);

int dc_pose_correct_fwd(const double* poses, const double* deltas, int n_poses, int n_deltas, double* poses_out,
                        dcStream_t stream);
int dc_pose_correct_bwd(const double* poses, const double* deltas, int n_poses, int n_deltas, const double* grad_poses,
                        double* grad_deltas, dcStream_t stream);
int dc_pose_train_finish(const double* sums, int layout, int n_terms, int n_scans, double* w, double* w_m, double* w_v, const double* poses0,
                         double* deltas, double* d_m, double* d_v, int n_deltas, int zero_first, int64_t* step, double lr_w, double lr_d,
                         double beta1, double beta2, double eps, const double* poses_used, double* record, int ring_rows, double* poses_next,
                         double* poses12_next, const double* totals, const double* record_extra, int n_record_extra, dcStream_t stream);
int dc_pose_train_combine(const double* const* outs, int n_seq, int layout, int n_terms, double* totals, dcStream_t stream);
int dc_pose_train_combine2(const double* const* outs_a, int n_a, const double* const* outs_b, int n_b, int layout, int n_terms,
                           double* totals, dcStream_t stream);

int dc_shadow_mask(const void* points, const void* vps, int vps_rows, int dtype, const int32_t* dir_nbr, int64_t n, int k,
                   double lo, double hi, double fill, uint8_t* mask_out, dcStream_t stream);

int dc_shadow_filter(const void* points, const void* vps, int vps_rows, const void* dirs, int dtype, int64_t n, double r,
                     double lo, double hi, uint8_t* mask_out, void* ws, size_t ws_bytes, dcStream_t stream);

int dc_correct_depth(const void* depth, const void* gamma, const uint8_t* mask, const double* w, const double* exponent,
                     int n_terms, int op, int dtype, int64_t n, void* depth_out, dcStream_t stream);

int64_t dc_p2plane_partial_count(int64_t m);
int dc_p2plane_pair(const void* vpsA, const void* dirsA, const void* depthA, const void* incA, const uint8_t* lmaskA,
                    const void* normalsA, const void* vpsB, const void* dirsB, const void* depthB, const void* incB,
                    const uint8_t* lmaskB, const void* normalsB, int dtype, const double* poseA, const double* poseB,
                    int model_kind, int n_terms, const double* w, const double* e, const int32_t* idxA,
                    const int32_t* idxB, int64_t m, int want_exponent_grad, int want_pose_grad, double* partials_ws,
                    double* out, dcStream_t stream);

typedef struct dcIcpScan {
  const void* vps;
  const void* dirs;
  const void* depth;
// ... 8 lines not shown
  int64_t m;
  double weight;
} dcIcpPair;
int64_t dc_p2plane_sequence_partial_count(const dcIcpPair* pairs, int n_pairs);
int dc_p2plane_sequence(const dcIcpScan* scans, int n_scans, const dcIcpPair* pairs, int n_pairs, int dtype,
                        const double* poses, int model_kind, int n_terms, const double* w, const double* e,
                        double* partials_ws, double* out, dcStream_t stream);
int dc_p2point_pair(const void* vpsA, const void* dirsA, const void* depthA, const void* incA, const uint8_t* lmaskA,
                    const void* vpsB, const void* dirsB, const void* depthB, const void* incB, const uint8_t* lmaskB, int dtype,
                    const double* poseA, const double* poseB, int model_kind, int n_terms, const double* w, const double* e,
                    const int32_t* idxA, const int32_t* idxB, int64_t m, double* partials_ws, double* out, dcStream_t stream);
int dc_p2point_sequence(const dcIcpScan* scans, int n_scans, const dcIcpPair* pairs, int n_pairs, int dtype,
                        const double* poses, int model_kind, int n_terms, const double* w, const double* e,
                        double* partials_ws, double* out, dcStream_t stream);

typedef struct dcPoseTrainStep {
  double *w, *w_m, *w_v;
  const double* poses0;
  double *deltas, *d_m, *d_v;
  int32_t n_deltas, zero_first;
  int64_t* step;
  double lr_w, lr_d, beta1, beta2, eps;
  const double* poses_used;
  double* record;
  int32_t ring_rows, n_record_extra;
  const double* record_extra;
  double* poses_next;
  double* poses12_next;
} dcPoseTrainStep;
int dc_icp_sequence_step(int plane, const dcIcpScan* scans, int n_scans, const dcIcpPair* pairs, int n_pairs, int dtype,
                         const double* poses, int model_kind, int n_terms, const double* w, const double* e, double* partials_ws,
                         double* out, int32_t* ticket, const dcPoseTrainStep* fin, dcStream_t stream);


int dc_consistency_gate(const void* raw_pointwise, int dtype, int point_fmt, const uint8_t* mask, int64_t n,
                        const double* threshold, int sqrt_, void* rec, double* partials_ws, double* sums_out,
                        dcStream_t stream);

typedef struct dcPoseTable {
  const int32_t* blk_ptr;
  const int32_t* ids;
  const uint16_t* loc;
  const uint16_t* own_pos;
  const uint16_t* row_seg;
  const uint8_t* row_scan;
} dcPoseTable;
int dc_pose_table_build(const dcBlockTable* fwd, const int32_t* scan_id, int64_t n, int n_scans, int k, int32_t* ids_out,
                        uint16_t* loc_out, uint16_t* own_pos, uint16_t* row_seg, uint8_t* row_scan, int32_t* info, dcStream_t stream);
int dc_points_local_basis(const void* dirs, const void* depth, const void* inc, const uint8_t* lmask, const int32_t* scan_id,
                          int model_kind, int n_terms, const double* e, int64_t n, int dtype, const dcPoseTable* table, void* rows_out,
                          dcStream_t stream);

typedef struct dcSequenceDesc {
  int64_t n;
  int32_t k, n_scans, dtype, point_fmt;
  double qparams[4];
  const void *vps, *dirs, *depth, *inc;
  const uint8_t* lmask;
  const int32_t* scan_id;
  const int32_t *nbr, *csr_ptr, *csr_src;
  const uint8_t* mask;
  const uint8_t* lane_perm;
  const int32_t* centre_idx;
  int64_t n_centres;
  void *x, *rec;
  double* partials;
  int32_t model_kind, n_terms, loss_kind, normalization, sqrt_, reserved;
  const dcBlockTable* fwd_table;
  const dcBlockTable* bwd_table;
  int32_t* status;
  const void* basis;
  int64_t partials_count;
  const uint16_t* scan_seg;
  const uint8_t* blk_skip;
  int32_t fwd_rows_active;
  int32_t reserved2;
  const dcPoseTable* pose_table;
  const void* local_basis;
  const dcBlockTable* fwd_table_loss;
  int32_t fwd_rows_active_loss;
  int32_t reserved3;
  const void* step_hdr;
  const void* step_rows;
} dcSequenceDesc;

int64_t dc_sequence_partials_count(int64_t n, int n_terms, int n_scans);

int dc_sequence_eval(const dcSequenceDesc* desc, const double* w, const double* e, const double* poses, int want_grad,
                     int want_exponent_grad, int want_pose_grad, double* out, dcStream_t stream);
int dc_sequence_step(const dcSequenceDesc* d, double* w, const double* e, const double* poses, double* exp_avg,
                     double* exp_avg_sq, int64_t step, double grad_scale, double lr, double beta1, double beta2, double eps,
                     double weight_decay, double* out, dcStream_t stream);

int dc_sequence_step_chained(const dcSequenceDesc* d, double* w, const double* e, const double* poses, double* exp_avg,
                             double* exp_avg_sq, int64_t step, int has_prev, double grad_scale, double lr, double beta1, double beta2,
                             double eps, double weight_decay, int32_t* ready, double* out_prev, dcStream_t stream);
int dc_sequence_step_chained_rec(const dcSequenceDesc* d, double* w, const double* e, const double* poses, double* exp_avg,
                                 double* exp_avg_sq, int64_t step, int has_prev, double grad_scale, double lr, double beta1, double beta2,
                                 double eps, double weight_decay, int32_t* ready, double* out_prev, double* w_used_prev,
                                 dcStream_t stream);
int dc_sequence_chain_flush(const dcSequenceDesc* d, double* w, double* exp_avg, double* exp_avg_sq, int64_t step, double grad_scale,
                            double lr, double beta1, double beta2, double eps, double weight_decay, double* out, dcStream_t stream);
int dc_sequence_step_linked(const dcSequenceDesc* d, const dcSequenceDesc* d_prev, int prev_parity, int finish, const double* acc_in,
                            double* w, const double* e, const double* poses, double* exp_avg, double* exp_avg_sq, int64_t step,
                            int64_t stamp, double grad_scale, double lr, double beta1, double beta2, double eps, double weight_decay,
                            int32_t* ready, double* out_prev, double* w_used_prev, dcStream_t stream);
int dc_sequence_chain_flush_linked(const dcSequenceDesc* d_prev, int prev_parity, const double* acc_in, double* w, double* exp_avg,
                                   double* exp_avg_sq, int64_t step, int64_t stamp, double grad_scale, double lr, double beta1, double beta2,
                                   double eps, double weight_decay, int32_t* ready, double* out, dcStream_t stream);
int dc_sequence_eval_after_update(const dcSequenceDesc* d, double* w, const double* e, const double* poses, double* exp_avg,
                                  double* exp_avg_sq, int64_t step, const double* grad_sum, double grad_scale, double lr, double beta1,
                                  double beta2, double eps, double weight_decay, int32_t* ready, double* out, double* w_used,
                                  dcStream_t stream);

int dc_adam_step(double* param, const double* grad, double* exp_avg, double* exp_avg_sq, int64_t n, int64_t step,
                 double grad_scale, double lr, double beta1, double beta2, double eps, double weight_decay,
                 dcStream_t stream);
int dc_adam_step_device(double* param, const double* grad, double* exp_avg, double* exp_avg_sq, int64_t n, int64_t* step,
                        double grad_scale, double lr, double beta1, double beta2, double eps, double weight_decay,
                        dcStream_t stream);

size_t dc_voxel_filter_workspace_bytes(int64_t n);
int dc_voxel_filter(const void* points, int stride, int dtype, int64_t n, double grid_res, const int32_t* seq,
                    int preserve_order, int32_t* out_idx, int32_t* count_out, int32_t* status_out, void* ws, size_t ws_bytes,
                    dcStream_t stream);

size_t dc_cloud_from_points_workspace_bytes(int64_t n);
int dc_cloud_from_points(const void* points, int stride, int in_dtype, const void* vps, int64_t n, double ego_box,
                         double min_depth, double max_depth, int out_dtype, void* dirs_out, void* depth_out, void* vps_out,
                         int32_t* index_out, int64_t* count_out, void* ws, size_t ws_bytes, dcStream_t stream);

int dc_set_option(int option, int value);

int dc_profiler_enable(int every);
int dc_profiler_reset(void);
int dc_profiler_read(int kind, double* total_ms, int64_t* launches);
int dc_profiler_kernel(int kind, char* buf, int len);

int dc_ransac_score(const void* points, int dtype, const int32_t* remaining, int64_t n_rem, int64_t seed, int64_t round, int n_hyp,
                    double thresh, double* hyp, double* anchor, int32_t* valid, int32_t* counts, int32_t* best, dcStream_t stream);
int dc_ransac_refit_partial_count(int64_t n_rem);
int dc_ransac_refit(const void* points, int dtype, const int32_t* remaining, int64_t n_rem, const double* hyp, const double* anchor,
                    const int32_t* best, double thresh, double* partials, int n_partials, double* params, uint8_t* mask,
                    dcStream_t stream);
int dc_dbscan(const int32_t* nbr, int64_t m, int k, int min_pts, uint8_t* core, int32_t* lab, int32_t* label_out, int32_t* sizes,
              int32_t* flag, int32_t* best, dcStream_t stream);
int dc_plane_moments_fwd(const void* vps, const void* dirs, const void* depth, int dtype, const int32_t* idx, const int32_t* plane_ptr,
                         const double* normals, int n_planes, const int32_t* blk_plane, const int32_t* blk_begin, const int32_t* plane_blk,
                         int n_blocks, int chunk, int model_kind, int n_terms, const double* w, const double* e, double* partials,
                         double* cov, double* mean, dcStream_t stream);
int dc_plane_moments_bwd(const void* vps, const void* dirs, const void* depth, int dtype, const int32_t* idx, const int32_t* plane_ptr,
                         const double* normals, int n_planes, const int32_t* blk_plane, const int32_t* blk_begin, int n_blocks, int chunk,
                         int model_kind, int n_terms, const double* w, const double* e, const double* mean, const double* gcov,
                         void* g_vps, void* g_dirs, void* g_depth, double* wpartials, double* g_w, dcStream_t stream);

int64_t dc_sequence_landscape_workspace_count(int64_t n);
int dc_sequence_landscape(const void* rows, int point_fmt, double step, int n_terms, const int32_t* nbr, int64_t n, int k,
                          const uint8_t* mask, const double* weights, int64_t n_w, int loss_kind, int normalization, int sqrt_,
                          int n_bounds, const double* bounds, double* workspace, int64_t workspace_count, double* out,
                          dcStream_t stream);

int dc_plane_landscape_partials_count(int n_blocks, int n_terms);
int dc_plane_landscape(const void* vps, const void* dirs, const void* depth, int dtype, const int32_t* idx, const int32_t* plane_ptr,
                       const double* normals, int n_planes, const int32_t* blk_plane, const int32_t* blk_begin, const int32_t* plane_blk,
                       int n_blocks, int chunk, int model_kind, int n_terms, const double* e, const uint8_t* mask, const double* weights,
                       int64_t n_w, int loss_kind, int normalization, int sqrt_, double* partials, int64_t partials_count,
// ... 276 lines not shown
```

Baseline: 56.47 billion.

## Prebuild per-thread packed neighbour-location words for vectorized loads in q32 step kernel

Adds a one-time build kernel that repacks the block table's 16-bit neighbour location rows into per-thread contiguous 32-bit words. The q32 step kernel can then fetch them with uint4/uint2 vector loads instead of many strided 16-bit loads. It also inserts an empty asm barrier that keeps the fourth row word alive in the gather loops, which may change how the compiler schedules the LDS reads. The cost is an extra device buffer, a cached build step, and a new descriptor field, with an option to turn the path off.

```diff
diff --git a/depth_correction_amd/_native.py b/depth_correction_amd/_native.py
--- a/depth_correction_amd/_native.py
+++ b/depth_correction_amd/_native.py
@@ -68,6 +68,7 @@
     'dc_block_table_build': (_i32, [_vp, _vp, _i64, _i32, _i64, _vp, _i64, _vp, _vp, _vp, _vp, _vp, _sz, _vp]),
     'dc_step_header_build': (_i32, [_vp, _i64, _vp, _vp, _vp, _vp]),
     'dc_step_rows_build': (_i32, [_vp, _i64, _vp, _i32, _vp, _vp]),
+    'dc_step_loc_build': (_i32, [_vp, _i64, _vp, _vp]),
     'dc_block_group': (_i32, [_vp, _vp, _vp, _i64, _i32, _vp, _vp, _vp, _vp, _vp]),
     'dc_pose_table_build': (_i32, [_vp, _vp, _i64, _i32, _i32, _vp, _vp, _vp, _vp, _vp, _vp, _vp]),
     'dc_points_local_basis': (_i32, [_vp, _vp, _vp, _vp, _vp, _i32, _i32, _vp, _i64, _i32, _vp, _vp, _vp]),
@@ -281,7 +282,7 @@
                 ('partials_count', ctypes.c_int64), ('scan_seg', _vp), ('blk_skip', _vp), ('fwd_rows_active', ctypes.c_int32),
                 ('reserved2', ctypes.c_int32), ('pose_table', _vp), ('local_basis', _vp), ('fwd_table_loss', _vp),
                 ('fwd_rows_active_loss', ctypes.c_int32), ('reserved3', ctypes.c_int32), ('step_hdr', _vp),
-                ('step_rows', _vp)]
+                ('step_rows', _vp), ('step_loc', _vp)]
 
 
 def lib_path():
diff --git a/depth_correction_amd/csrc/dc_cons_basis.h b/depth_correction_amd/csrc/dc_cons_basis.h
--- a/depth_correction_amd/csrc/dc_cons_basis.h
+++ b/depth_correction_amd/csrc/dc_cons_basis.h
@@ -173,6 +173,23 @@
   }
 }
 
+__host__ __device__ constexpr int step_loc_piece_words(int nw, int piece) { return nw - 4 * piece < 4 ? nw - 4 * piece : 4; }
+
+__global__ __launch_bounds__(kBlock) void step_loc_kernel(const int32_t* __restrict__ slot_ptr, const uint16_t* __restrict__ loc,
+                                                          uint32_t* __restrict__ out) {
+  const int32_t s0 = slot_ptr[blockIdx.x];
+  const int nw = (slot_ptr[blockIdx.x + 1] - s0) / 2;
+  const uint16_t* lrow = loc + (int64_t)s0 * kBlock;
+  uint32_t* range = out + (int64_t)s0 * (kBlock / 2);
+  const int full = (nw / 4) * 4 * kBlock;
+  for (int j = threadIdx.x; j < nw * kBlock; j += kBlock) {
+    const int g = j < full ? j / (4 * kBlock) : nw / 4;
+    const int gw = step_loc_piece_words(nw, g);
+    const int r = j - 4 * g * kBlock, t = r / gw, w = 4 * g + (r - t * gw);
+    range[j] = (uint32_t)lrow[2 * w * kBlock + t] | ((uint32_t)lrow[(2 * w + 1) * kBlock + t] << 16);
+  }
+}
+
 template <typename PT, bool FULL_EIG, int NS, int P>
 __global__ __launch_bounds__(kBlock) void consistency_fwd_basis_kernel(
     PointBasis pb, BlockTab tab, const int32_t* __restrict__ own_base, int cap, const int32_t* __restrict__ centre_idx, int64_t n,
diff --git a/depth_correction_amd/csrc/dc_cons_pose.h b/depth_correction_amd/csrc/dc_cons_pose.h
--- a/depth_correction_amd/csrc/dc_cons_pose.h
+++ b/depth_correction_amd/csrc/dc_cons_pose.h
@@ -205,8 +205,8 @@
       for (int q = 1; q < NS; ++q) mo |= pre[q];
       const bool any_miss = __any((int)(mo & 1u)) != 0;
       int n_have;
-      if (any_miss) n_have = gather_fixed<q32, NS, true>(tile, CAP, ci, pre, acc);
-      else n_have = gather_fixed<q32, NS, false>(tile, CAP, ci, pre, acc);
+      if (any_miss) n_have = gather_fixed<q32, NS, true, true>(tile, CAP, ci, pre, acc);
+      else n_have = gather_fixed<q32, NS, false, true>(tile, CAP, ci, pre, acc);
       acc.W = (double)n_have;
       double se2;
       step_point2<q32, NS>(acc, n_have, !any_miss, in_mask, lp, qp, acc2, cm, v0, &c1, &c2, &se2);
diff --git a/depth_correction_amd/csrc/dc_cons_step.h b/depth_correction_amd/csrc/dc_cons_step.h
--- a/depth_correction_amd/csrc/dc_cons_step.h
+++ b/depth_correction_amd/csrc/dc_cons_step.h
@@ -474,8 +474,9 @@
       for (int q = 1; q < NS; ++q) mx = max(mx, pre[q]);
       const bool any_miss = __any((int)(mx == kNoLoc)) != 0;
       int n_have;
-      if (any_miss) n_have = gather_fixed<PT, NS, true>(tile, cap, ci, pre, acc);
-      else n_have = gather_fixed<PT, NS, false>(tile, cap, ci, pre, acc);
+      constexpr bool kWide = std::is_same<PT, q32>::value;
+      if (any_miss) n_have = gather_fixed<PT, NS, true, kWide>(tile, cap, ci, pre, acc);
+      else n_have = gather_fixed<PT, NS, false, kWide>(tile, cap, ci, pre, acc);
       acc.W = (double)n_have;
       double cm[3], v0[3], c1, c2;
       if constexpr ((VAR & kVarSlimTail) != 0) step_point2<PT, NS>(acc, n_have, !any_miss, in_mask, lp, qp, acc2, cm, v0, &c1, &c2);
@@ -559,6 +560,24 @@
   return 7 * lds <= 160 * 1024 ? 7 : 6 * lds <= 160 * 1024 ? 6 : 4;
 }
 template <int Q> __device__ __forceinline__ uint32_t pre_at(const uint32_t* pk) { return (Q & 1) ? pk[Q >> 1] >> 16 : pk[Q >> 1] & 0xFFFFu; }
+template <int NW>
+__device__ __forceinline__ void fetch_step_loc(const uint32_t* blk, uint32_t tid, uint32_t* pk) {
+  static_assert(NW % 4 == 0 || NW % 4 == 1 || NW % 4 == 2, "the slot counts the step kernel is built for: 4, 8, 10, 16");
+#pragma unroll
+  for (int g = 0; 4 * g < NW; ++g) {
+    const int gw = step_loc_piece_words(NW, g);
+    const uint32_t* r = blk + (uint32_t)(4 * g * kBlock) + (uint32_t)gw * tid;
+    if (gw == 4) {
+      const uint4 v = *reinterpret_cast<const uint4*>(r);
+      pk[4 * g] = v.x; pk[4 * g + 1] = v.y; pk[4 * g + 2] = v.z; pk[4 * g + 3] = v.w;
+    } else if (gw == 2) {
+      const uint2 v = *reinterpret_cast<const uint2*>(r);
+      pk[4 * g] = v.x; pk[4 * g + 1] = v.y;
+    } else {
+      pk[4 * g] = r[0];
+    }
+  }
+}
 template <int NS, bool MISS, int Q0 = 0>
 __device__ __forceinline__ int gather_fixed_pk(const int4* tile, const Pt<q32>::Raw& ci, const uint32_t* pk, CovAcc& acc) {
   if constexpr (Q0 >= NS) return 0;
@@ -571,6 +590,7 @@
     if constexpr (NQ > 3) off[3] = pre_at<Q0 + (NQ > 3 ? 3 : 0)>(pk);
     Pt<q32>::Raw cj[NQ];
     bool have[NQ];
+    int w4[NQ];
     int n_have = 0;
 #pragma unroll
     for (int u_ = 0; u_ < NQ; ++u_) {
@@ -578,9 +598,11 @@
       int4 piece[1];
       read_row<1>(tile, 0, have[u_] ? off[u_] : 0u, piece);
       cj[u_] = Pt<q32>::from_row(piece);
+      w4[u_] = piece[0].w;
     }
 #pragma unroll
     for (int u_ = 0; u_ < NQ; ++u_) {
+      keep_row_word(w4[u_]);
       double d[3];
       Pt<q32>::delta(have[u_] ? cj[u_] : ci, ci, d);
       cov_add_d(acc, d[0], d[1], d[2]);
@@ -613,8 +635,8 @@
 
 template <int NS, int P, int CAP, int BLOCKS = step_q32_blocks<P, CAP>()>
 __global__ __launch_bounds__(kBlock, BLOCKS) void consistency_step_q32_kernel(
-    PointBasis pb, BlockTab tab, const StepHdr* __restrict__ hdr, const int32_t* __restrict__ step_rows, const int32_t* __restrict__ centre_idx,
-    int64_t n, LossParams lp, QParams qp, double* __restrict__ p_fwd, double* __restrict__ p_bwd, StepChain ch) {
+    PointBasis pb, BlockTab tab, const StepHdr* __restrict__ hdr, const int32_t* __restrict__ step_rows, const uint32_t* __restrict__ step_loc,
+    const int32_t* __restrict__ centre_idx, int64_t n, LossParams lp, QParams qp, double* __restrict__ p_fwd, double* __restrict__ p_bwd, StepChain ch) {
   constexpr int NV = 2 + P, NP2 = NV <= 4 ? 4 : 8;
   constexpr int cap = CAP;
   __shared__ int4 tile[StepRow<q32, P>::kPieces * CAP];
@@ -648,10 +670,16 @@
     const uint16_t* lrow = tab.loc + (int64_t)s0 * kBlock;
     constexpr int NW = (NS + 1) / 2;
     uint32_t pk[NW];
-#pragma unroll
-    for (int j = 0; j < NW; ++j)
-      pk[j] = (uint32_t)lrow[(uint32_t)(2 * j * kBlock) + tid] |
-              (2 * j + 1 < NS ? (uint32_t)lrow[(uint32_t)((2 * j + 1 < NS ? 2 * j + 1 : 0) * kBlock) + tid] << 16 : 0u);
+    if (step_loc) {
+#pragma unroll
+      for (int j = 0; j < NW; ++j) pk[j] = 0u;
+      if (in_word != 0) fetch_step_loc<NW>(step_loc + (int64_t)s0 * (kBlock / 2), tid, pk);
+    } else {
+#pragma unroll
+      for (int j = 0; j < NW; ++j)
+        pk[j] = (uint32_t)lrow[(uint32_t)(2 * j * kBlock) + tid] |
+                (2 * j + 1 < NS ? (uint32_t)lrow[(uint32_t)((2 * j + 1 < NS ? 2 * j + 1 : 0) * kBlock) + tid] << 16 : 0u);
+    }
     const int32_t* ids = tab.blk_ids + base;
     const int32_t* crow = step_rows ? step_rows + (int64_t)base * (6 + P) : nullptr;
     double wq[P];
@@ -816,9 +844,10 @@
 #pragma unroll
     for (int q = 0; q < kPreSlots; ++q) miss |= (q < nslots) && pre[q] == kNoLoc;
     int n_have = 0;
-    if (__any((int)miss)) n_have = gather_slots<PT, true>(tile, cap, ci, pre, nslots, acc);
-    else n_have = gather_slots<PT, false>(tile, cap, ci, pre, nslots, acc);
-    if (nslots > kPreSlots) n_have += gather_tail<PT>(tile, cap, ci, lrow, nslots, packed != 0, acc);
+    constexpr bool kWide = std::is_same<PT, q32>::value;
+    if (__any((int)miss)) n_have = gather_slots<PT, true, kWide>(tile, cap, ci, pre, nslots, acc);
+    else n_have = gather_slots<PT, false, kWide>(tile, cap, ci, pre, nslots, acc);
+    if (nslots > kPreSlots) n_have += gather_tail<PT, kWide>(tile, cap, ci, lrow, nslots, packed != 0, acc);
     acc.W = (double)n_have;
     double cm[3], v0[3], c1, c2;
     const bool full = nslots >= 2 && !__any((int)(n_have != nslots));
@@ -933,8 +962,10 @@
 #pragma unroll
       for (int u_ = 0; u_ < kTrip; ++u_) r[u_] = *reinterpret_cast<const int4*>(tb + (l[u_] == kNoLoc ? own_off : l[u_]));
 #pragma unroll
-      for (int u_ = 0; u_ < kTrip; ++u_)
+      for (int u_ = 0; u_ < kTrip; ++u_) {
+        keep_row_word(r[u_].w);
         cov_add_d(acc, (double)(r[u_].x - ci.v[0]), (double)(r[u_].y - ci.v[1]), (double)(r[u_].z - ci.v[2]));
+      }
     };
     {
       uint32_t la[kTrip], lb[kTrip];
diff --git a/depth_correction_amd/csrc/dc_consistency.hip b/depth_correction_amd/csrc/dc_consistency.hip
--- a/depth_correction_amd/csrc/dc_consistency.hip
+++ b/depth_correction_amd/csrc/dc_consistency.hip
@@ -462,22 +462,25 @@
   for (int a = 0; a < ROW16; ++a) q[a] = *reinterpret_cast<const int4*>(p + (size_t)a * cap * 16);
 }
 
+__device__ __forceinline__ void keep_row_word(int w) { asm volatile("" ::"v"(w)); }
+
 constexpr int kPreSlots = 16;
 
-template <typename PT, bool MISS>
+template <typename PT, bool MISS, bool WIDE = false>
 __device__ __forceinline__ int slot_add(const int4* tile, int cap, const typename Pt<PT>::Raw& ci, uint32_t l, CovAcc& acc) {
   constexpr int XR = Pt<PT>::kRow16;
   const bool have = !MISS || l != kNoLoc;
   int4 piece[XR];
   read_row<XR>(tile, cap, have ? l : 0u, piece);
   const typename Pt<PT>::Raw cj = Pt<PT>::from_row(piece);
+  if constexpr (WIDE) keep_row_word(piece[0].w);
   double d[3];
   Pt<PT>::delta(have ? cj : ci, ci, d);
   cov_add_d(acc, d[0], d[1], d[2]);
   return have ? 1 : 0;
 }
 
-template <typename PT, bool MISS>
+template <typename PT, bool MISS, bool WIDE = false>
 __device__ __forceinline__ int gather_slots(const int4* tile, int cap, const typename Pt<PT>::Raw& ci, const uint32_t* pre,
                                             int nslots, CovAcc& acc) {
   constexpr int XR = Pt<PT>::kRow16;
@@ -487,15 +490,18 @@
     if (4 * t + 4 <= nslots) {
       typename Pt<PT>::Raw cj[4];
       bool have[4];
+      int w4[4];
 #pragma unroll
       for (int u_ = 0; u_ < 4; ++u_) {
         have[u_] = !MISS || pre[4 * t + u_] != kNoLoc;
         int4 piece[XR];
         read_row<XR>(tile, cap, have[u_] ? pre[4 * t + u_] : 0u, piece);
         cj[u_] = Pt<PT>::from_row(piece);
+        w4[u_] = piece[0].w;
       }
 #pragma unroll
       for (int u_ = 0; u_ < 4; ++u_) {
+        if constexpr (WIDE) keep_row_word(w4[u_]);
         double d[3];
         Pt<PT>::delta(have[u_] ? cj[u_] : ci, ci, d);
         cov_add_d(acc, d[0], d[1], d[2]);
@@ -504,14 +510,14 @@
     } else {
 #pragma unroll
       for (int u_ = 0; u_ < 4; ++u_)
-        if (4 * t + u_ < nslots) n_have += slot_add<PT, MISS>(tile, cap, ci, pre[4 * t + u_], acc);
+        if (4 * t + u_ < nslots) n_have += slot_add<PT, MISS, WIDE>(tile, cap, ci, pre[4 * t + u_], acc);
     }
   }
   return n_have;
 }
 
 constexpr int kTrip = 8;
-template <typename PT>
+template <typename PT, bool WIDE = false>
 __device__ __forceinline__ int gather_tail(const int4* tile, int cap, const typename Pt<PT>::Raw& ci, const uint16_t* lrow,
                                            int nslots, bool packed, CovAcc& acc) {
   constexpr int XR = Pt<PT>::kRow16;
@@ -527,14 +533,17 @@
 #pragma unroll
     for (int u_ = 0; u_ < kTrip; ++u_) nxt[u_] = (q0 + kTrip + u_ < nslots) ? (uint32_t)lrow[(q0 + kTrip + u_) * kBlock] : kNoLoc;
     typename Pt<PT>::Raw cj[kTrip];
+    int w4[kTrip];
 #pragma unroll
     for (int u_ = 0; u_ < kTrip; ++u_) {
       int4 piece[XR];
       read_row<XR>(tile, cap, l[u_] != kNoLoc ? l[u_] : 0u, piece);
       cj[u_] = Pt<PT>::from_row(piece);
+      w4[u_] = piece[0].w;
     }
 #pragma unroll
     for (int u_ = 0; u_ < kTrip; ++u_) {
+      if constexpr (WIDE) keep_row_word(w4[u_]);
       const bool have = l[u_] != kNoLoc;
       double d[3];
       Pt<PT>::delta(have ? cj[u_] : ci, ci, d);
@@ -591,15 +600,17 @@
   wave_partials<2>(acc2, partials);
 }
 
-template <typename PT, int NS, bool MISS>
+template <typename PT, int NS, bool MISS, bool WIDE = false>
 __device__ __forceinline__ int gather_fixed(const int4* tile, int cap, const typename Pt<PT>::Raw& ci, const uint32_t* pre,
                                             CovAcc& acc) {
   constexpr int XR = Pt<PT>::kRow16;
+  static_assert(!WIDE || XR == 1, "a row of one 16-byte piece");
   int n_have = 0;
 #pragma unroll
   for (int q0 = 0; q0 < NS; q0 += 4) {
     typename Pt<PT>::Raw cj[4];
     bool have[4];
+    int w4[4];
 #pragma unroll
     for (int u_ = 0; u_ < 4; ++u_) {
       if (q0 + u_ < NS) {
@@ -607,11 +618,13 @@
         int4 piece[XR];
         read_row<XR>(tile, cap, have[u_] ? pre[q0 + u_] : 0u, piece);
         cj[u_] = Pt<PT>::from_row(piece);
+        w4[u_] = piece[0].w;
       }
     }
 #pragma unroll
     for (int u_ = 0; u_ < 4; ++u_) {
       if (q0 + u_ < NS) {
+        if constexpr (WIDE) keep_row_word(w4[u_]);
         double d[3];
         Pt<PT>::delta(have[u_] ? cj[u_] : ci, ci, d);
         cov_add_d(acc, d[0], d[1], d[2]);
@@ -1022,6 +1035,7 @@
 static std::atomic<bool> g_no_reverse{false};
 static std::atomic<bool> g_step_six{false};
 static std::atomic<bool> g_no_step_rows{false};
+static std::atomic<bool> g_no_step_loc{false};
 
 template <int P, int CAP>
 static int ragged_launch(dim3 grid, hipStream_t stream, hipEvent_t ev0, hipEvent_t ev1, const PointBasis& pb, const BlockTab& tab,
@@ -1169,6 +1183,16 @@
   if (!table->blk_ids || !basis || !rows_out || ((uintptr_t)rows_out & 15)) return DC_ERR_ARG;
   hipLaunchKernelGGL(step_rows_kernel, dim3((unsigned)n_blocks(n_rows)), dim3(kBlock), 0, stream, table->blk_ptr, table->blk_ids,
                      static_cast<const int32_t*>(basis), row_words, static_cast<int32_t*>(rows_out));
+  DC_CHECK_LAUNCH();
+  return DC_OK;
+}
+
+int dc_step_loc_build(const dcBlockTable* table, int64_t n_rows, void* loc_out, hipStream_t stream) {
+  if (!table || n_rows < 0 || table->layout != DC_TABLE_SLOTS || !table->slot_ptr) return DC_ERR_ARG;
+  if (n_rows == 0) return DC_OK;
+  if (!table->loc || !loc_out || ((uintptr_t)loc_out & 15)) return DC_ERR_ARG;
+  hipLaunchKernelGGL(step_loc_kernel, dim3((unsigned)n_blocks(n_rows)), dim3(kBlock), 0, stream, table->slot_ptr, table->loc,
+                     static_cast<uint32_t*>(loc_out));
   DC_CHECK_LAUNCH();
   return DC_OK;
 }
@@ -1432,6 +1456,7 @@
   if (option == 8) { g_no_reverse.store(value != 0); return DC_OK; }
   if (option == 9) { g_step_six.store(value != 0); return DC_OK; }
   if (option == 10) { g_no_step_rows.store(value != 0); return DC_OK; }
+  if (option == 11) { g_no_step_loc.store(value != 0); return DC_OK; }
   return DC_ERR_ARG;
 }
 
@@ -1550,11 +1575,12 @@
   ProfScope prof(1);
   const StepHdr* hdr = static_cast<const StepHdr*>(a.d->step_hdr);
   const int32_t* step_rows = g_no_step_rows.load() ? nullptr : static_cast<const int32_t*>(a.d->step_rows);
+  const uint32_t* step_loc = g_no_step_loc.load() ? nullptr : static_cast<const uint32_t*>(a.d->step_loc);
   const dim3 block(kBlock);
   static_assert(kStepQ32Cap == 512, "the profiler names the instantiation by its literal arguments");
   static_assert(step_q32_blocks<1, 512>() == 7 && step_q32_blocks<2, 512>() == 7 && step_q32_blocks<3, 512>() == 6 && step_q32_blocks<2, 768>() == 6,
                 "which instantiations dc_set_option(9, 1) has a six-block build of");
-#define STEPQ_TAIL a.pb, a.tab, hdr, step_rows, a.d->centre_idx, r.n_rows, a.lp, a.qp, a.p_fwd, a.p_bwd, a.ch
+#define STEPQ_TAIL a.pb, a.tab, hdr, step_rows, step_loc, a.d->centre_idx, r.n_rows, a.lp, a.qp, a.p_fwd, a.p_bwd, a.ch
 #define STEPQ(P, NS, CAP) DC_TIMED_LAUNCH((consistency_step_q32_kernel<NS, P, CAP>), a.grid, block, 0, a.stream, STEPQ_TAIL)
 #define STEPQ_SIX(P, NS, X) DC_TIMED_LAUNCH((consistency_step_q32_kernel<NS, P, 512, 6>), a.grid, block, 0, a.stream, STEPQ_TAIL)
 #define STEPQ_P(NS, CAP) DC_SWITCH_P(r.P, STEPQ(3, NS, CAP), STEPQ, NS, CAP)
diff --git a/depth_correction_amd/plan.py b/depth_correction_amd/plan.py
--- a/depth_correction_amd/plan.py
+++ b/depth_correction_amd/plan.py
@@ -23,7 +23,7 @@
                  normalization=True, sqrt=False, spatial_sort=True, point_format='auto', degree_sort=False,
                  active_only=False, block_tables=True, bwd_layout='runs', stages=None, basis=True, lazy_backward=True,
                  scan_group=True, mask_first=False, nan_policy=None, pose_kernel=True, degree_group=False, heavy_first=False,
-                 wave_pack=None, step_rows=True):
+                 wave_pack=None, step_rows=True, step_loc=True):
         mark = stages.mark if stages is not None else (lambda name: None)
         get = (lambda c, f: c[f]) if isinstance(clouds[0], dict) else getattr
         vps = ops.cat_rows([get(c, 'vps') for c in clouds])
@@ -228,6 +228,8 @@
         self._pose_table = self._local_basis = None
         self._basis = None
         self.use_step_rows = bool(step_rows)
+        self._step_loc = None
+        self.use_step_loc = bool(step_loc)
         self._poses_key = self._poses12 = self._poses_ref = None
 
     @on_device
@@ -331,7 +333,7 @@
               and self.fwd_table is not None and self._block_tables and self._bwd_layout == 'runs'
               and d.model_kind != 0)
         if not ok:
-            d.basis = d.step_rows = None
+            d.basis = d.step_rows = d.step_loc = None
             return
         nt = w.numel()
         b = self._basis
@@ -355,6 +357,15 @@
             b[4] = torch.empty((max(self._step_rows_total, 1) * (6 + nt),), dtype=torch.int32, device=self.device)
             check(lib().dc_step_rows_build(ft.ref(), self.nbr.shape[0], ptr(b[1]), 6 + nt, ptr(b[4]), stream_ptr()), 'dc_step_rows_build')
         d.step_rows = None if (b[4] is None or not self.use_step_rows) else b[4].data_ptr()
+        sl = self._step_loc
+        if sl is not None and sl[0] is not ft:
+            self._step_loc = sl = None
+        if (sl is None and b[4] is not None and self.use_step_loc and self.k in (4, 8, 10, 16) and self.nbr.shape[1] == self.k
+                and ft.loc is not None and ft.slot_ptr is not None):
+            words = torch.empty(((ft.loc.numel() + 1) // 2,), dtype=torch.int32, device=self.device)
+            check(lib().dc_step_loc_build(ft.ref(), self.nbr.shape[0], ptr(words), stream_ptr()), 'dc_step_loc_build')
+            self._step_loc = sl = [ft, words]
+        d.step_loc = None if (sl is None or not self.use_step_loc) else sl[1].data_ptr()
 
     @on_device
     def eval_native(self, w, exponent, poses12, out, want_grad=True, want_exponent=False, want_pose=False):
diff --git a/include/dc_hip.h b/include/dc_hip.h
--- a/include/dc_hip.h
+++ b/include/dc_hip.h
@@ -122,6 +122,7 @@
 int dc_step_header_build(const dcBlockTable* table, int64_t n_rows, const uint8_t* mask, const uint8_t* blk_skip, void* hdr_out,
                          dcStream_t stream);
 int dc_step_rows_build(const dcBlockTable* table, int64_t n_rows, const void* basis, int row_words, void* rows_out, dcStream_t stream);
+int dc_step_loc_build(const dcBlockTable* table, int64_t n_rows, void* loc_out, dcStream_t stream);
 size_t dc_block_table_workspace_bytes(int64_t n_refs);
 int dc_block_table_set_lds_build(int on);
 size_t dc_block_table_slots_workspace_bytes(int64_t n_rows, int k);
@@ -296,6 +297,7 @@
   int32_t reserved3;
   const void* step_hdr;
   const void* step_rows;
+  const void* step_loc;
 } dcSequenceDesc;
 
 int64_t dc_sequence_partials_count(int64_t n, int n_terms, int n_scans);
```

Result: faster. 57.81 billion (median of 6 runs) (+2.4%).
